# LeCAR-Lab/dial-mpc

Measured on NVIDIA H100. Metric: sample-steps/s (Nsample*Hsample/wall-s) per MPC reverse_once, Go2, higher is better.
Workload: dtype f32

## Files before the change

__graft_entry__.py:

```python
from __future__ import annotations

import os
import subprocess
import sys

ROOT = os.path.dirname(os.path.abspath(__file__))
CSRC = os.path.join(ROOT, "dial_mpc_b200", "csrc")
LIB = os.path.join(CSRC, "libdial_b200.so")
NVCC_FLAGS = ["-gencode", "arch=compute_90a,code=sm_90a", "-lineinfo", "-O3", "-std=c++17",
              "-use_fast_math", "-Xcompiler", "-fPIC"]
LINK_FLAGS = ["-gencode", "arch=compute_90a,code=sm_90a", "-shared", "-Xcompiler", "-fPIC", "-cudart", "static"]
VARIANTS = (1, 2, 3, 4, 0)
OBJDIR = os.path.join(CSRC, "build")


def _digest(srcs, extra=""):
    import hashlib
    h = hashlib.sha256()
    for s in srcs:
        h.update(open(s, "rb").read())
    h.update((" ".join(NVCC_FLAGS + LINK_FLAGS) + extra).encode())
    return h.hexdigest()


def _stale(target, digest):
    side = target + ".sha256"
    if not (os.path.exists(target) and os.path.exists(side)):
        return True
    return open(side).read().strip() != digest


def _stamp(target, digest):
    with open(target + ".sha256", "w") as f:
        f.write(digest)


def build_library(force: bool = False, extra=(), lib: str = LIB, objdir: str = OBJDIR) -> None:
    extra = list(extra)
    tag = " " + " ".join(extra)
    hdrs = [os.path.join(CSRC, f) for f in ("dial_device.cuh", "dial_host.h")] + [os.path.join(ROOT, "include", "dial_b200.h")]
    var_src = os.path.join(CSRC, "dial_rollout_variant.cu")
    abi_src = os.path.join(CSRC, "dial_kernels.cu")
    lib_digest = _digest(hdrs + [var_src, abi_src], tag)
    if not (force or _stale(lib, lib_digest)):
        return
    nvcc = os.environ.get("NVCC", "/usr/local/cuda/bin/nvcc")
    os.makedirs(objdir, exist_ok=True)
    jobs = []
    for v in VARIANTS:
        obj = os.path.join(objdir, f"rollout_v{v}.o")
        jobs.append((obj, _digest(hdrs + [var_src], f" variant={v}" + tag),
                     [nvcc] + NVCC_FLAGS + extra + [f"-DDIAL_VARIANT={v}", "-c", "-o", obj, var_src]))
    obj = os.path.join(objdir, "dial_kernels.o")
    jobs.append((obj, _digest(hdrs + [abi_src], tag), [nvcc] + NVCC_FLAGS + extra + ["-c", "-o", obj, abi_src]))
    running = [(o, d, subprocess.Popen(cmd)) for o, d, cmd in jobs if force or _stale(o, d)]
    for o, d, p in running:
        if p.wait() != 0:
            for _, _, q in running:
                q.wait()
            raise RuntimeError(f"nvcc failed for {o}")
        _stamp(o, d)
    subprocess.check_call([nvcc] + LINK_FLAGS + ["-o", lib] + [o for o, _, _ in jobs])
    _stamp(lib, lib_digest)


def build(force: bool = False) -> None:
    build_library(force)
    if ROOT not in sys.path:
        sys.path.insert(0, ROOT)
    import dial_mpc_b200
    from dial_mpc_b200 import _capi
    _capi.lib()
    ex = os.path.join(ROOT, "dial_mpc_b200", "examples", "custom_env")
    if ex not in sys.path:
        sys.path.insert(0, ex)
    import quadpod_env
    _ = quadpod_env.QuadpodEnv(quadpod_env.QuadpodEnvConfig()).library_path
    import pincher_env
    _ = pincher_env.PincherEnv(pincher_env.PincherEnvConfig()).library_path
    for mod in ("tests.emul.emul", "oracle.build_oracle"):
        path = os.path.join(ROOT, *mod.split(".")) + ".py"
        if os.path.exists(path):
            subprocess.check_call([sys.executable, "-c", f"import {mod} as m; m.build()"], cwd=ROOT)


def smoke() -> None:
    if ROOT not in sys.path:
        sys.path.insert(0, ROOT)
    import numpy as np
    import torch
    build()
    import dial_mpc_b200.envs as E
    from dial_mpc_b200 import random as drandom
    from dial_mpc_b200.core.dial_config import DialConfig
    from dial_mpc_b200.core.dial_core import MBDPI
    from oracle.envs_oracle import make_env
    from oracle.planner_oracle import PlannerOracle
    torch.cuda.set_device(0)
    cfg = DialConfig(env_name="unitree_go2_walk", Nsample=64, Hsample=8, Hnode=4, temp_sample=0.05)
    env = E.get_environment(cfg.env_name, config=E.UnitreeGo2EnvConfig(default_vx=0.8, ramp_up_time=1.0))
    mb = MBDPI(cfg, env)
    state = env.reset(drandom.PRNGKey(0))
    rng = np.random.default_rng(0)
    eps = rng.standard_normal((cfg.Nsample, cfg.Hnode + 1, mb.nu)).astype(np.float32)
    Y0 = torch.zeros(cfg.Hnode + 1, mb.nu, device=mb.device)
    _, Ybar, info = mb.reverse_once(state, drandom.PRNGKey(1), Y0, mb.sigma_control, eps=eps)
    torch.cuda.synchronize()
    o = make_env(cfg.env_name, dict(default_vx=0.8, ramp_up_time=1.0))
    po = PlannerOracle(o, cfg.Nsample, cfg.Hsample, cfg.Hnode, cfg.temp_sample, cfg.horizon_diffuse_factor,
                       cfg.traj_diffuse_factor)
    Yo, io = po.reverse_once(o.reset(), eps.astype(np.float64), np.zeros((cfg.Hnode + 1, mb.nu)), po.sigma_control)
    rews = info["rews"].cpu().numpy()
    err_r = np.abs(rews - io["rews"]).max()
    err_y = np.abs(Ybar.cpu().numpy() - Yo).max()
    print(f"smoke: max|rews - oracle| = {err_r:.3e}, max|Ybar - oracle| = {err_y:.3e}, launches = {mb.plan.launches}")
    assert np.isfinite(rews).all()
    assert err_r < 2e-3 and err_y < 5e-3, "CUDA reverse_once disagrees with the oracle"


if __name__ == "__main__":
    build()
    if len(sys.argv) > 1 and sys.argv[1] == "smoke":
        smoke()
```

dial_mpc_b200/_capi.py:

```python

from __future__ import annotations

import ctypes as C
import os
import re
from typing import Dict, Optional

import numpy as np

_HERE = os.path.dirname(os.path.abspath(__file__))
_ROOT = os.path.dirname(_HERE)
HEADER = os.path.join(_ROOT, "include", "dial_b200.h")
LIB_PATH = os.path.join(_HERE, "csrc", "libdial_b200.so")

_CT = {"int32_t": C.c_int32, "uint32_t": C.c_uint32, "float": C.c_float, "int64_t": C.c_int64}


def _parse_header(path: str):
    text = open(path).read()
    text = re.sub(r"/\*.*?\*/", "", text, flags=re.S)
    text = re.sub(r"//[^\n]*", "", text)
    defines: Dict[str, int] = {}
    for mm in re.finditer(r"#define\s+(\w+)\s+(\d+)\s*$", text, flags=re.M):
        defines[mm.group(1)] = int(mm.group(2))
# ... 105 lines not shown

def _set(field, value):
    arr = np.ctypeslib.as_array(field)
    value = np.asarray(value)
    if value.size == 0:
        return
    sl = tuple(slice(0, s) for s in value.shape)
    if any(s > d for s, d in zip(value.shape, arr.shape)):
        raise ValueError(f"value of shape {value.shape} exceeds capacity {arr.shape}")
    arr[sl] = value


def fill_model_desc(cm) -> dial_model_desc:
    d = dial_model_desc()
    for k in ("nq", "nv", "nu", "nbody", "njnt", "ngeom", "nsite", "npair", "ncon",
              "iterations", "ls_iterations", "cone"):
        setattr(d, k, int(getattr(cm, k)))
    d.eulerdamp = int(bool(cm.eulerdamp))
    for k in ("timestep", "tolerance", "ls_tolerance", "impratio", "meaninertia"):
        setattr(d, k, float(getattr(cm, k)))
    _set(d.gravity, cm.gravity)
    A = cm.arrays
    for k in ("body_parentid", "body_rootid", "body_depth", "body_jntadr", "body_dofadr", "body_dofnum",
              "body_pos", "body_quat", "body_ipos", "body_iquat", "body_mass", "body_inertia",
              "jnt_type", "jnt_qposadr", "jnt_dofadr", "jnt_limited", "jnt_pos", "jnt_axis", "jnt_range",
              "jnt_margin", "jnt_solref", "jnt_solimp",
              "dof_bodyid", "dof_jntid", "dof_parentid", "dof_armature", "dof_damping", "dof_invweight0",
              "qpos0", "geom_type", "geom_bodyid", "geom_pos", "geom_quat", "geom_size",
              "pair_kind", "pair_geom1", "pair_geom2", "pair_ncon", "pair_condim", "pair_friction", "pair_margin",
              "pair_gap", "pair_solref", "pair_solimp", "site_bodyid", "site_pos",
              "actuator_dofadr", "actuator_qposadr", "actuator_ctrllimited", "actuator_forcelimited",
              "actuator_gear", "actuator_gain", "actuator_bias", "actuator_ctrlrange", "actuator_forcerange"):
        _set(getattr(d, k), A[k])
    _set(d.body_invweight0, A["body_invweight0"][:, 0])
    _set(d.body_invweight0_rot, A["body_invweight0"][:, 1])
    return d


def _bind(path: str) -> C.CDLL:
    if not os.path.exists(path):
        raise RuntimeError(
            f"{path} is missing: build it with `python -c 'import __graft_entry__ as g; g.build()'`."
            " There is no CPU fallback for the DIAL-MPC sampling core.")
    lib = C.CDLL(path)
    lib.dial_abi_version.restype = C.c_int
    lib.dial_last_error.restype = C.c_char_p
    lib.dial_sizeof.restype = C.c_size_t
    lib.dial_sizeof.argtypes = [C.c_int]
    lib.dial_plan_create.restype = C.c_void_p
    lib.dial_plan_create.argtypes = [C.POINTER(dial_model_desc), C.POINTER(dial_plan_desc)]
    lib.dial_plan_destroy.argtypes = [C.c_void_p]
    lib.dial_plan_destroy.restype = None
    P, I, V = C.c_void_p, C.c_int, C.c_void_p
    lib.dial_rollout.argtypes = [V, C.POINTER(dial_state), P, I, I, P, P, P, P, V]
    lib.dial_env_step.argtypes = [V, C.POINTER(dial_state), P, P, P, P, P, P, V]
    lib.dial_env_step_kin.argtypes = [V, C.POINTER(dial_state), P, P, P, P, P, P, P, V]
    lib.dial_plan_set_command.argtypes = [V, C.c_int, C.POINTER(C.c_float), C.POINTER(C.c_float), V]
    F = C.POINTER(C.c_float)
    lib.dial_plan_set_stages.argtypes = [V, C.c_int, F, F, F, F, V]
    lib.dial_pipeline_init.argtypes = [V, P, P, P, P, V]
    U2 = C.POINTER(C.c_uint32)
    lib.dial_reverse_rollout.argtypes = [V, C.POINTER(dial_state), P, U2, P, P, P, V]
    lib.dial_reverse_update.argtypes = [V, P, U2, P, P, P, P, P, V]
    lib.dial_reverse_update_x.argtypes = [V, P, U2, P, P, P, P, P, P, V]
    lib.dial_reverse_update_fused.argtypes = [V, P, P, P, P, P, P, V]
    lib.dial_reverse_trajbar.argtypes = [V, P, I, P, P, P, V]
    lib.dial_exchange_create.argtypes = [V, I, I, P]
    lib.dial_exchange_connect.argtypes = [V, P]
    lib.dial_exchange_status.argtypes = [V, U2]
    lib.dial_reverse_trajectories.argtypes = [V, P, P, P, V]
    lib.dial_key_split.argtypes = [U2, U2, U2]
    lib.dial_key_split.restype = None
    lib.dial_fp32_peak.argtypes = [I, C.POINTER(C.c_float)]
    lib.dial_fp32_peak.restype = C.c_int
    lib.dial_launch_count.argtypes = [V]
    lib.dial_launch_count.restype = C.c_int64
    lib.dial_rollout_wpc.argtypes = [V, I]
    lib.dial_rollout_wpc.restype = C.c_int
    lib.dial_debug_counters.argtypes = [V, C.POINTER(C.c_float)]
    lib.dial_debug_counters.restype = C.c_int
    lib.dial_solver_variant.argtypes = [C.POINTER(dial_model_desc)]
    lib.dial_solver_variant.restype = C.c_int
    lib.dial_custom_reward_id.restype = C.c_char_p
    lib.dial_mpc_bind.argtypes = [V, C.POINTER(dial_mpc_buffers), P]
    lib.dial_mpc_bind.restype = C.c_int
    lib.dial_mpc_step.argtypes = [V, I, I, V]
    lib.dial_mpc_step.restype = C.c_int
    lib.dial_plan_get_task.argtypes = [V, C.POINTER(dial_task)]
    lib.dial_plan_get_task.restype = C.c_int
    for fn in ("dial_rollout", "dial_env_step", "dial_env_step_kin", "dial_plan_set_command", "dial_plan_set_stages", "dial_pipeline_init", "dial_reverse_rollout",
               "dial_reverse_update", "dial_reverse_update_x", "dial_reverse_update_fused", "dial_reverse_trajbar",
               "dial_reverse_trajectories", "dial_exchange_create", "dial_exchange_connect", "dial_exchange_status"):
        getattr(lib, fn).restype = C.c_int
    if lib.dial_abi_version() != DEFINES["DIAL_ABI_VERSION"]:
        raise RuntimeError(f"{os.path.basename(path)} ABI version does not match include/dial_b200.h")
    for i, t in enumerate((dial_model_desc, dial_plan_desc, dial_state, dial_mpc_buffers, dial_task)):
        if lib.dial_sizeof(i) != C.sizeof(t):
            raise RuntimeError(f"struct layout mismatch for {t.__name__}: C {lib.dial_sizeof(i)} vs ctypes {C.sizeof(t)}")
    return lib


_LIBS: Dict[str, C.CDLL] = {}


def lib(path: Optional[str] = None) -> C.CDLL:
    path = os.path.abspath(path or os.environ.get("DIAL_B200_LIB") or LIB_PATH)
    if path not in _LIBS:
        _LIBS[path] = _bind(path)
    return _LIBS[path]


def check(rc: int) -> None:
    if rc != 0:
        raise RuntimeError(f"dial_b200: {lib().dial_last_error().decode()} (rc={rc})")


EXPORTS = ["dial_abi_version", "dial_last_error", "dial_sizeof", "dial_plan_create", "dial_plan_destroy", "dial_rollout",
           "dial_env_step", "dial_env_step_kin", "dial_plan_set_command", "dial_plan_set_stages", "dial_pipeline_init", "dial_reverse_rollout", "dial_reverse_update", "dial_reverse_update_x",
           "dial_reverse_update_fused", "dial_exchange_create", "dial_exchange_connect", "dial_exchange_status",
           "dial_reverse_trajbar", "dial_reverse_trajectories", "dial_key_split", "dial_fp32_peak", "dial_launch_count", "dial_rollout_wpc", "dial_debug_counters",
           "dial_solver_variant", "dial_custom_reward_id", "dial_mpc_bind", "dial_mpc_step", "dial_plan_get_task"]
```

dial_mpc_b200/csrc/dial_device.cuh:

```cuda
#pragma once

#include <stdint.h>
#include <math.h>
#include "../../include/dial_b200.h"

#ifdef DIAL_HOST_EMUL
#include "warp_emul.h"
#define DEV inline
#define HD inline
#else
#define HD __host__ __device__ __forceinline__
#define DEV __device__ __forceinline__
DEV void syncwarp() { __syncwarp(); }
DEV float shfl(float v, int src) { return __shfl_sync(0xffffffffu, v, src); }
DEV float shfl_xor(float v, int m) { return __shfl_xor_sync(0xffffffffu, v, m); }
DEV int shfl_i(int v, int src) { return __shfl_sync(0xffffffffu, v, src); }
DEV void cta_sync() { __syncthreads(); }
DEV bool cta_sync_or(bool p) { return __syncthreads_or(p) != 0; }
DEV void fast_sincos(float x, float& s, float& c) { __sincosf(x, &s, &c); }
DEV float fast_cos(float x) { return __cosf(x); }
#endif

#if defined(DIAL_HOST_EMUL) && defined(DIAL_EMUL_TRACE)
extern "C" void emul_trace(int kind, int val);
// ... 30 lines not shown
  int32_t con_row0[DIAL_MAXC], con_dim[DIAL_MAXC], nrow_c;
  int32_t jd_stride;
  int8_t con_colidx[DIAL_MAXC][DIAL_MAXV];
  int32_t con_lastdof[DIAL_MAXC];
  int32_t dof_nchain[DIAL_MAXV], dof_ndesc[DIAL_MAXV], nlimited;
  int32_t chain_tab[DIAL_MAXV][DIAL_MAXCHAIN];
  int32_t star_nroot, star_nchain, star_maxlen;
  int32_t star_root[8], star_len[4], star_leaf[4], star_att[4];
  int32_t nedge;
  int32_t s_on, s_nrp, s_cs, s_rs, s_npos;
  int32_t s_pos[DIAL_MAXV];
  int32_t s_chain[DIAL_MAXV];
  int32_t s_depth[DIAL_MAXV];
  int32_t s_top[4];
  int32_t s_con_chain[DIAL_MAXC];
  int32_t o_Ms, o_Hs, o_Js, o_xs;
  int32_t sb_on, sb_nroot, sb_root[4], sb_top[4], sb_len[4], sb_att[4];
  int32_t o_xpos, o_xquat, o_xmat, o_xipos, o_cinert, o_cdof, o_cdofdot, o_cvel, o_cacc,
      o_cfrc, o_Mb, o_L, o_J, o_qpos, o_qvel, o_warm, o_ctrl, o_vec, o_frow, o_cpos,
      o_cframe, o_cdist, o_rcom, o_xch, o_crb, o_cfs, o_Md, o_Ld, o_Jd, o_Gd, o_frow2, o_cact, o_hcs, warp_floats;
  int32_t pad_[1];
};

struct alignas(16) DevPlan {
  dial_plan_desc c;
  int32_t pad_[3];
};

#define DIAL_TASK_AT(f) (offsetof(dial_plan_desc, f) - offsetof(dial_plan_desc, vel_cmd) == offsetof(dial_task, f))
static_assert(DIAL_TASK_AT(vel_cmd) && DIAL_TASK_AT(ang_cmd) && DIAL_TASK_AT(pos_tar) && DIAL_TASK_AT(gait_duty) &&
              DIAL_TASK_AT(gait_cadence) && DIAL_TASK_AT(gait_amplitude) && DIAL_TASK_AT(gait_phase) &&
              DIAL_TASK_AT(cmd_step) && DIAL_TASK_AT(cmd_vel) && DIAL_TASK_AT(cmd_ang) && DIAL_TASK_AT(n_stage) &&
              DIAL_TASK_AT(jump_dt) && DIAL_TASK_AT(pose_seq) && DIAL_TASK_AT(yaw_seq) &&
              DIAL_TASK_AT(contact_targets) && DIAL_TASK_AT(contact_radius) && DIAL_TASK_AT(n_user) &&
              DIAL_TASK_AT(user) &&
              offsetof(dial_plan_desc, user) + sizeof(float) * DIAL_MAXUSER - offsetof(dial_plan_desc, vel_cmd) == sizeof(dial_task),
              "dial_plan_desc's task block must have the layout of dial_task");
#undef DIAL_TASK_AT

HD const dial_task& plan_task(const dial_plan_desc& c) { return *reinterpret_cast<const dial_task*>(c.vel_cmd); }

struct RolloutArgs {
  int32_t nrows;
  int32_t H;
  int32_t mode;
  int32_t lockstep;
  int32_t sync_every;
  int32_t step0, stage0;
  int32_t rows_per_inst;
  int32_t us_row;
  int32_t task_rows;
  const dial_task* tasks;
  const float* qpos0;
  const float* qvel0;
  const float* warm0;
  const float* us;
  const float* eps;
  const float* Ybar;
  const float* noise;
  uint32_t key0, key1;
  float* rewss;
  float* rews;
  float* q;
  float* qd;
  float* xpos;
  float* qpos_out;
  float* qvel_out;
  float* warm_out;
  float* ctrl_out;
  float* kin_out;
  const int32_t* counters_in;
  int32_t* counters_out;
  const uint32_t* key_dev;
  const uint32_t* rng_dev;
  unsigned int* row_counter;
  float* dbg;
  int32_t xch_world, xch_rank;
  float* xch_mbox[DIAL_MAXRANK];
  uint32_t* xch_flags[DIAL_MAXRANK];
  const uint32_t* xch_seq;
  unsigned int* xch_done;
};

struct V3 { float x, y, z; };
struct Q4 { float w, x, y, z; };

DEV V3 v3(float x, float y, float z) { V3 r; r.x = x; r.y = y; r.z = z; return r; }
DEV V3 ld3(const float* p) { return v3(p[0], p[1], p[2]); }
DEV void st3(float* p, V3 a) { p[0] = a.x; p[1] = a.y; p[2] = a.z; }
DEV V3 operator+(V3 a, V3 b) { return v3(a.x + b.x, a.y + b.y, a.z + b.z); }
DEV V3 operator-(V3 a, V3 b) { return v3(a.x - b.x, a.y - b.y, a.z - b.z); }
DEV V3 operator*(V3 a, float s) { return v3(a.x * s, a.y * s, a.z * s); }
DEV float dot(V3 a, V3 b) { return a.x * b.x + a.y * b.y + a.z * b.z; }
DEV V3 cross(V3 a, V3 b) { return v3(a.y * b.z - a.z * b.y, a.z * b.x - a.x * b.z, a.x * b.y - a.y * b.x); }
DEV Q4 ldq(const float* p) { Q4 q; q.w = p[0]; q.x = p[1]; q.y = p[2]; q.z = p[3]; return q; }
DEV void stq(float* p, Q4 q) { p[0] = q.w; p[1] = q.x; p[2] = q.y; p[3] = q.z; }
DEV Q4 qmul(Q4 a, Q4 b) {
  Q4 r;
  r.w = a.w * b.w - a.x * b.x - a.y * b.y - a.z * b.z;
  r.x = a.w * b.x + a.x * b.w + a.y * b.z - a.z * b.y;
  r.y = a.w * b.y - a.x * b.z + a.y * b.w + a.z * b.x;
  r.z = a.w * b.z + a.x * b.y - a.y * b.x + a.z * b.w;
  return r;
}
DEV V3 qrot(Q4 q, V3 v) {
  V3 u = v3(q.x, q.y, q.z);
  float s = q.w;
  V3 r = u * (2.f * dot(u, v)) + v * (s * s - dot(u, u));
  return r + cross(u, v) * (2.f * s);
}
DEV Q4 qnormalize(Q4 q) {
  float n = sqrtf(q.w * q.w + q.x * q.x + q.y * q.y + q.z * q.z);
  float inv = 1.f / (n + 1e-6f * (n == 0.f ? 1.f : 0.f));
  Q4 r; r.w = q.w * inv; r.x = q.x * inv; r.y = q.y * inv; r.z = q.z * inv; return r;
}
DEV void qmat(Q4 q, float* m) {
  float w = q.w, x = q.x, y = q.y, z = q.z;
  m[0] = w * w + x * x - y * y - z * z; m[1] = 2.f * (x * y - w * z); m[2] = 2.f * (x * z + w * y);
  m[3] = 2.f * (x * y + w * z); m[4] = w * w - x * x + y * y - z * z; m[5] = 2.f * (y * z - w * x);
  m[6] = 2.f * (x * z - w * y); m[7] = 2.f * (y * z + w * x); m[8] = w * w - x * x - y * y + z * z;
}
DEV Q4 axisangle(V3 axis, float angle) {
  float s, c;
  fast_sincos(0.5f * angle, s, c);
  Q4 q; q.w = c; q.x = axis.x * s; q.y = axis.y * s; q.z = axis.z * s; return q;
}

struct F4 { float x, y, z, w; };
DEV F4 ld4(const float* p) {
#ifdef DIAL_HOST_EMUL
  F4 r; r.x = p[0]; r.y = p[1]; r.z = p[2]; r.w = p[3]; return r;
#else
  const float4 v = *reinterpret_cast<const float4*>(p);
  F4 r; r.x = v.x; r.y = v.y; r.z = v.z; r.w = v.w; return r;
#endif
}
DEV void st4(float* p, float a, float b, float c, float d) {
#ifdef DIAL_HOST_EMUL
  p[0] = a; p[1] = b; p[2] = c; p[3] = d;
#else
  *reinterpret_cast<float4*>(p) = make_float4(a, b, c, d);
#endif
}
DEV void ld2(const float* p, float& a, float& b) {
#ifdef DIAL_HOST_EMUL
  a = p[0]; b = p[1];
#else
  const float2 v = *reinterpret_cast<const float2*>(p);
  a = v.x; b = v.y;
#endif
}
DEV void st2(float* p, float a, float b) {
#ifdef DIAL_HOST_EMUL
  p[0] = a; p[1] = b;
#else
  *reinterpret_cast<float2*>(p) = make_float2(a, b);
#endif
}
#define CDS 8
#define CIS 12
DEV void ld6(const float* p, float* o) {
  F4 a = ld4(p);
  o[0] = a.x; o[1] = a.y; o[2] = a.z; o[3] = a.w;
  ld2(p + 4, o[4], o[5]);
}
DEV void st6(float* p, const float* v) {
// ... 433 lines not shown
  float l_sign, l_D, l_aref, l_Jaref;
  float e_D, e_aref, e_Jaref;
  float gauss, cost, prev_cost, gradnorm2;
  float qfc;
};

DEV void update_constraint(WarpCtx& w, Solver& S) {
  float fl = (S.l_Jaref < 0.f) ? -S.l_D * S.l_Jaref : 0.f;
  float fe = (S.e_Jaref < 0.f) ? -S.e_D * S.e_Jaref : 0.f;
  float qfc = mul_JT(w, fe) + S.l_sign * fl;
  S.grad = S.Ma - S.qfs - qfc;
  float g = (S.Ma - S.qfs) * (S.qacc - S.qas);
  float c = ((S.l_Jaref < 0.f) ? S.l_D * S.l_Jaref * S.l_Jaref : 0.f)
          + ((S.e_Jaref < 0.f) ? S.e_D * S.e_Jaref * S.e_Jaref : 0.f);
  float g2 = S.grad * S.grad;
  warp_sum3(g, c, g2);
  S.gauss = 0.5f * g;
  S.prev_cost = S.cost;
  S.cost = 0.5f * c + S.gauss;
  S.gradnorm2 = g2;
}

template <int MCU>
DEV void build_H(WarpCtx& w, const Solver& S, const float* Mrow, float* R) {
  const DevModel& M = *w.M;
  const int lane = w.lane;
  const float* Jc = SM(J);
  float* frow = SM(frow);
  syncwarp();
  frow[lane] = (S.e_Jaref < 0.f) ? S.e_D : 0.f;
  syncwarp();
#pragma unroll
  for (int c = 0; c < MCU; ++c) R[c] = Mrow[c];
  if (w.nch > 0) {
    R[0] += (S.l_Jaref < 0.f) ? S.l_D : 0.f;
    for (int c_ = 0; c_ < M.m.ncon; ++c_) {
      const int kc = M.con_lastdof[c_];
      if ((M.dof_ancmask[kc] >> lane) & 1u) {
        const int off = M.dof_nchain[kc] - w.nch;
        for (int e = 4 * c_; e < 4 * c_ + 4; ++e) {
          const float de = frow[e];
          if (de != 0.f) {
            const float* Je = Jc + e * MC + off;
            const float a = de * Je[0];
#pragma unroll
            for (int c = 0; c < MCU; ++c)
              if (c < w.nch) R[c] += a * Je[c];
          }
        }
      }
    }
  }
}


template <int NL, int NR>
struct StarDims {
  static constexpr int NRP = (NR + 3) & ~3, CS = (NL + 3) & ~3, RS = NRP + CS;
};

template <int N>
DEV void ldv(const float* p, float* out) {
  F4 a = ld4(p);
  out[0] = a.x; if (N > 1) out[1] = a.y; if (N > 2) out[2] = a.z; if (N > 3) out[3] = a.w;
  if (N > 4) {
    F4 b = ld4(p + 4);
    out[4] = b.x; if (N > 5) out[5] = b.y; if (N > 6) out[6] = b.z; if (N > 7) out[7] = b.w;
  }
}
template <int NL, int NR>
DEV void star_store_row(float* p, const float* Rr, const float* Rc) {
  using SD = StarDims<NL, NR>;
  float t[SD::RS];
#pragma unroll
  for (int i = 0; i < SD::RS; ++i) t[i] = 0.f;
#pragma unroll
  for (int a = 0; a < NR; ++a) t[a] = Rr[a];
#pragma unroll
  for (int q = 0; q < NL; ++q) t[SD::NRP + q] = Rc[q];
#pragma unroll
  for (int i = 0; i < SD::RS; i += 4) st4(p + i, t[i], t[i + 1], t[i + 2], t[i + 3]);
}

template <int NL, int NR, bool WITH_M, bool WITH_J>
DEV void star_mul_MJ(WarpCtx& w, const float* Mr, const float* Mc, float x, float& Mx, float& Jx) {
  using SD = StarDims<NL, NR>;
  const DevModel& M = *w.M;
  float* xs = SM(xs);
  const float* Ms = SM(Ms);
  syncwarp();
  if (w.s_chain >= -1) xs[w.s_pos] = x;
  syncwarp();
  float xr[SD::NRP], xc[SD::CS];
  ldv<NR>(xs, xr);
  ldv<NL>(xs + w.s_cb, xc);
  float y = 0.f;
  if (WITH_M) {
  float y0 = 0.f, y1 = 0.f, y2 = 0.f, y3 = 0.f;
#pragma unroll
  for (int a = 0; a < NR; ++a) { if (a & 1) y1 += Mr[a] * xr[a]; else y0 += Mr[a] * xr[a]; }
  if (w.s_chain >= 0) {
#pragma unroll
    for (int q = 0; q < NL; ++q) { if (q & 1) y3 += Mc[q] * xc[q]; else y2 += Mc[q] * xc[q]; }
  } else if (w.s_chain == -1) {
    const float* col = Ms + SD::NRP * SD::RS + w.s_col;
    const int nslot = M.star_nchain * SD::CS;
    for (int s0 = 0; s0 < nslot; s0 += 4) {
      F4 xv = ld4(xs + SD::NRP + s0);
      y0 += col[(s0 + 0) * SD::RS] * xv.x; y1 += col[(s0 + 1) * SD::RS] * xv.y;
      y2 += col[(s0 + 2) * SD::RS] * xv.z; y3 += col[(s0 + 3) * SD::RS] * xv.w;
    }
  }
  y = (y0 + y1) + (y2 + y3);
  }
  Mx = y;
  if (WITH_J) {
    float j = 0.f;
    if (w.lane < M.nedge) {
      const float* row = SM(Js) + w.lane * SD::RS;
      float jr[SD::NRP], jc[SD::CS], xe[SD::CS];
      ldv<NR>(row, jr);
      ldv<NL>(row + SD::NRP, jc);
      ldv<NL>(xs + w.e_cb, xe);
      float j0 = 0.f, j1 = 0.f, j2 = 0.f;
#pragma unroll
      for (int a = 0; a < NR; ++a) { if (a & 1) j1 += jr[a] * xr[a]; else j0 += jr[a] * xr[a]; }
#pragma unroll
      for (int q = 0; q < NL; ++q) j2 += jc[q] * xe[q];
      j = (j0 + j1) + j2;
    }
    Jx = j;
  }
}

template <int NL, int NR>
DEV float star_mul_JT(WarpCtx& w, float f) {
  using SD = StarDims<NL, NR>;
  const DevModel& M = *w.M;
  const float* Js = SM(Js);
  float* frow = SM(frow);
  syncwarp();
  frow[w.lane] = f;
  syncwarp();
  float y0 = 0.f, y1 = 0.f, y2 = 0.f, y3 = 0.f;
  const float* col = Js + w.s_col;
  for (int c = 0; c < M.m.ncon; ++c) {
    const F4 fv = ld4(frow + 4 * c);
    if ((w.s_conmask >> c) & 1u) {
      const float* jc = col + 4 * c * SD::RS;
      y0 += jc[0] * fv.x; y1 += jc[SD::RS] * fv.y; y2 += jc[2 * SD::RS] * fv.z; y3 += jc[3 * SD::RS] * fv.w;
    }
  }
  return (y0 + y1) + (y2 + y3);
}

template <int NL, int NR>
DEV void star_build_H(WarpCtx& w, const Solver& S, const float* Mr, const float* Mc, float* Rr, float* Rc) {
  using SD = StarDims<NL, NR>;
  const DevModel& M = *w.M;
  const float* Js = SM(Js);
  float* frow = SM(frow);
  syncwarp();
  frow[w.lane] = (S.e_Jaref < 0.f) ? S.e_D : 0.f;
  syncwarp();
#pragma unroll
  for (int a = 0; a < NR; ++a) Rr[a] = Mr[a];
#pragma unroll
  for (int q = 0; q < NL; ++q) Rc[q] = Mc[q];
  const float ld = (S.l_Jaref < 0.f) ? S.l_D : 0.f;
  if (w.s_chain >= 0) {
#pragma unroll
    for (int q = 0; q < NL; ++q) Rc[q] += (q == w.s_depth) ? ld : 0.f;
  } else if (w.s_chain == -1) {
#pragma unroll
    for (int a = 0; a < NR; ++a) Rr[a] += (a == w.s_depth) ? ld : 0.f;
  }
  for (int e = 0; e < M.nedge; ++e) {
    const float de = frow[e];
    if (de == 0.f) continue;
    const float* row = Js + e * SD::RS;
    const float je = ((w.s_conmask >> (e >> 2)) & 1u) ? row[w.s_col] : 0.f;
    const float al = de * je;
    float jr[SD::NRP], jc[SD::CS];
    ldv<NR>(row, jr);
    ldv<NL>(row + SD::NRP, jc);
#pragma unroll
    for (int a = 0; a < NR; ++a) Rr[a] += al * jr[a];
#pragma unroll
    for (int q = 0; q < NL; ++q) Rc[q] += al * jc[q];
  }
}

template <int NL, int NR>
DEV float star_solve2(WarpCtx& w, const float* Rr, const float* Rc, float g) {
  using SD = StarDims<NL, NR>;
  static_assert(NR + 1 <= 8, "root block + rhs must fit the 8 lanes of a group");
  const DevModel& M = *w.M;
  const int lane = w.lane;
  float* Hs = SM(Hs);
  float* xs = SM(xs);
  syncwarp();
  if (w.s_chain >= -1) {
    star_store_row<NL, NR>(Hs + w.s_pos * SD::RS, Rr, Rc);
    xs[w.s_pos] = g;
  }
  syncwarp();
  const int grp = lane >> 3, j = lane & 7, gbase = lane & ~7;
  const bool ischain = grp < M.star_nchain;
  const int len = ischain ? M.star_len[grp] : 0;
  const int cb = SD::NRP + grp * SD::CS;
  float A[NL][NL], wv[NL];
#pragma unroll
  for (int p = 0; p < NL; ++p) {
    const bool on = p < len;
    const float* row = Hs + (cb + p) * SD::RS;
    float rc[SD::CS];
    ldv<NL>(row + SD::NRP, rc);
#pragma unroll
    for (int p2 = p; p2 < NL; ++p2) A[p][p2] = (on && p2 < len) ? rc[p2] : (p2 == p ? 1.f : 0.f);
    float cv = 0.f;
    if (on && j < NR) cv = row[j];
    if (on && j == NR) cv = xs[cb + p];
    wv[p] = cv;
  }
  float rinv[NL];
#pragma unroll
  for (int p = 0; p < NL; ++p) {
    float d = A[p][p];
#pragma unroll
    for (int k = 0; k < p; ++k) d -= A[k][p] * A[k][p];
    const float inv = rsqrtf(fmaxf(d, DIAL_MINVAL));
    rinv[p] = inv;
#pragma unroll
    for (int p2 = p + 1; p2 < NL; ++p2) {
      float v = A[p][p2];
#pragma unroll
      for (int k = 0; k < p; ++k) v -= A[k][p] * A[k][p2];
      A[p][p2] = v * inv;
    }
    float v = wv[p];
#pragma unroll
    for (int k = 0; k < p; ++k) v -= A[k][p] * wv[k];
    wv[p] = v * inv;
  }
  float t[NR + 1];
#pragma unroll
  for (int j2 = 0; j2 <= NR; ++j2) {
    float acc = 0.f;
#pragma unroll
    for (int p = 0; p < NL; ++p) acc += wv[p] * shfl(wv[p], gbase + j2);
    t[j2] = acc;
  }
#pragma unroll
  for (int j2 = 0; j2 <= NR; ++j2) {
    t[j2] += shfl_xor(t[j2], 8);
    t[j2] += shfl_xor(t[j2], 16);
  }
  float srow[NR], rhs = 0.f;
  {
    const int jj = j < NR ? j : 0;
    float br[SD::NRP];
    ldv<NR>(Hs + jj * SD::RS, br);
#pragma unroll
    for (int a2 = 0; a2 < NR; ++a2) srow[a2] = br[a2] - t[a2];
    rhs = xs[jj] - t[NR];
  }
  float S_[NR][NR], xB[NR];
#pragma unroll
  for (int a = 0; a < NR; ++a) {
#pragma unroll
    for (int a2 = a; a2 < NR; ++a2) S_[a][a2] = shfl(srow[a2], gbase + a);
    xB[a] = shfl(rhs, gbase + a);
  }
  float sinv[NR];
#pragma unroll
  for (int a = 0; a < NR; ++a) {
    float d = S_[a][a];
#pragma unroll
    for (int k = 0; k < a; ++k) d -= S_[k][a] * S_[k][a];
    const float inv = rsqrtf(fmaxf(d, DIAL_MINVAL));
    sinv[a] = inv;
#pragma unroll
    for (int a2 = a + 1; a2 < NR; ++a2) {
      float v = S_[a][a2];
#pragma unroll
      for (int k = 0; k < a; ++k) v -= S_[k][a] * S_[k][a2];
      S_[a][a2] = v * inv;
    }
    float v = xB[a];
#pragma unroll
    for (int k = 0; k < a; ++k) v -= S_[k][a] * xB[k];
    xB[a] = v * inv;
  }
#pragma unroll
  for (int a = NR - 1; a >= 0; --a) {
    float v = xB[a];
#pragma unroll
    for (int a2 = a + 1; a2 < NR; ++a2) v -= S_[a][a2] * xB[a2];
    xB[a] = v * sinv[a];
  }
  float xb_j = 0.f;
#pragma unroll
  for (int a = 0; a < NR; ++a) xb_j = (j == a) ? xB[a] : xb_j;
  float xl[NL];
#pragma unroll
  for (int p = 0; p < NL; ++p) {
    float v = (j < NR) ? wv[p] * xb_j : 0.f;
    v += shfl_xor(v, 1); v += shfl_xor(v, 2); v += shfl_xor(v, 4);
    xl[p] = shfl(wv[p], gbase + NR) - v;
  }
#pragma unroll
  for (int p = NL - 1; p >= 0; --p) {
    float v = xl[p];
#pragma unroll
    for (int p2 = p + 1; p2 < NL; ++p2) v -= A[p][p2] * xl[p2];
    xl[p] = v * rinv[p];
  }
  syncwarp();
  if (j == 0 && ischain) {
#pragma unroll
    for (int p = 0; p < NL; ++p)
      if (p < len) xs[cb + p] = xl[p];
  }
  if (lane == 0) {
#pragma unroll
    for (int a = 0; a < NR; ++a) xs[a] = xB[a];
  }
  syncwarp();
  return w.s_chain >= -1 ? xs[w.s_pos] : 0.f;
}

template <int NL, int NR>
DEV void star_update_constraint(WarpCtx& w, Solver& S) {
  float fl = (S.l_Jaref < 0.f) ? -S.l_D * S.l_Jaref : 0.f;
  float fe = (S.e_Jaref < 0.f) ? -S.e_D * S.e_Jaref : 0.f;
  float qfc = star_mul_JT<NL, NR>(w, fe) + S.l_sign * fl;
  S.grad = S.Ma - S.qfs - qfc;
  float g = (S.Ma - S.qfs) * (S.qacc - S.qas);
  float c = ((S.l_Jaref < 0.f) ? S.l_D * S.l_Jaref * S.l_Jaref : 0.f)
          + ((S.e_Jaref < 0.f) ? S.e_D * S.e_Jaref * S.e_Jaref : 0.f);
  float g2 = S.grad * S.grad;
  warp_sum3(g, c, g2);
  S.gauss = 0.5f * g;
  S.prev_cost = S.cost;
  S.cost = 0.5f * c + S.gauss;
  S.gradnorm2 = g2;
}

struct LSPoint { float alpha, cost, d0, d1; };

#ifdef DIAL_ROBUST_LS
#define DIAL_LS_SWAP_LO(lo, nx) (((lo).d0 < (nx).d0) && ((nx).d0 < 0.f))
#define DIAL_LS_SWAP_HI(hi, nx) (((hi).d0 > (nx).d0) && ((nx).d0 > 0.f))
#else
#define DIAL_LS_SWAP_LO(lo, nx) (((lo).d0 > 0.f) || ((lo).d0 < (nx).d0))
#define DIAL_LS_SWAP_HI(hi, nx) (((hi).d0 < 0.f) || ((hi).d0 > (nx).d0))
#endif

DEV void warp_allsum6(int lane, float* v) {
  const bool b16 = (lane & 16) != 0, b8 = (lane & 8) != 0;
  float u0 = b16 ? v[3] : v[0], u1 = b16 ? v[4] : v[1], u2 = b16 ? v[5] : v[2];
  const float s0 = b16 ? v[0] : v[3], s1 = b16 ? v[1] : v[4], s2 = b16 ? v[2] : v[5];
  u0 += shfl_xor(s0, 16); u1 += shfl_xor(s1, 16); u2 += shfl_xor(s2, 16);
  float t = b8 ? u1 : u0;
  const float st = b8 ? u0 : u1;
  t += shfl_xor(st, 8); u2 += shfl_xor(u2, 8);
  t += shfl_xor(t, 4); u2 += shfl_xor(u2, 4);
  t += shfl_xor(t, 2); u2 += shfl_xor(u2, 2);
  t += shfl_xor(t, 1); u2 += shfl_xor(u2, 1);
  v[0] = shfl(t, 0); v[1] = shfl(t, 8); v[3] = shfl(t, 16); v[4] = shfl(t, 24);
  v[2] = shfl(u2, 0); v[5] = shfl(u2, 16);
}

struct LSRow { float lq0, lq1, lq2, eq0, eq1, eq2; };

template <int NA, bool COST>
DEV void ls_points(int lane, const Solver& S, const LSRow& K, float l_jv, float e_jv, const float* qg, const float* al, LSPoint* out) {
  float s[3 * NA];
#pragma unroll
  for (int i = 0; i < 3 * NA; ++i) s[i] = 0.f;
#pragma unroll
  for (int i = 0; i < NA; ++i) {
    if (S.l_Jaref + al[i] * l_jv < 0.f) { if (COST) s[3 * i] += K.lq0; s[3 * i + 1] += K.lq1; s[3 * i + 2] += K.lq2; }
    if (S.e_Jaref + al[i] * e_jv < 0.f) { if (COST) s[3 * i] += K.eq0; s[3 * i + 1] += K.eq1; s[3 * i + 2] += K.eq2; }
  }
  if constexpr ((NA == 3 && !COST) || (NA == 2 && COST)) {
    float v[6];
    if constexpr (NA == 3) { v[0] = s[1]; v[1] = s[2]; v[2] = s[4]; v[3] = s[5]; v[4] = s[7]; v[5] = s[8]; }
    else { v[0] = s[0]; v[1] = s[1]; v[2] = s[2]; v[3] = s[3]; v[4] = s[4]; v[5] = s[5]; }
    warp_allsum6(lane, v);
    if constexpr (NA == 3) { s[1] = v[0]; s[2] = v[1]; s[4] = v[2]; s[5] = v[3]; s[7] = v[4]; s[8] = v[5]; }
    else { s[0] = v[0]; s[1] = v[1]; s[2] = v[2]; s[3] = v[3]; s[4] = v[4]; s[5] = v[5]; }
  } else {
#pragma unroll
    for (int o = 16; o > 0; o >>= 1) {
#pragma unroll
      for (int i = 0; i < 3 * NA; ++i)
        if (COST || (i % 3) != 0) s[i] += shfl_xor(s[i], o);
    }
  }
#pragma unroll
  for (int i = 0; i < NA; ++i) {
    float t0 = qg[0] + s[3 * i], t1 = qg[1] + s[3 * i + 1], t2 = qg[2] + s[3 * i + 2];
    float a = al[i];
    out[i].alpha = a;
    out[i].cost = COST ? a * a * t2 + a * t1 + t0 : 0.f;
    out[i].d0 = 2.f * a * t2 + t1;
    out[i].d1 = 2.f * t2 + (t2 == 0.f ? DIAL_MINVAL : 0.f);
  }
}

DEV void linesearch_core(WarpCtx& w, Solver& S, float mv, float e_jv) {
  const DevModel& M = *w.M;
  const int nv = M.m.nv;
  const float scale = M.m.meaninertia * (float)(nv > 1 ? nv : 1);
  float l_jv = S.l_sign * S.search;
  float ss = S.search * S.search, sMa = S.search * (S.Ma - S.qfs), sMv = S.search * mv;
  warp_sum3(ss, sMa, sMv);
  float gtol = M.m.tolerance * M.m.ls_tolerance * sqrtf(ss) * scale;
  float qg[3] = {S.gauss, sMa, 0.5f * sMv};
  LSRow K;
  K.lq0 = 0.5f * S.l_Jaref * S.l_Jaref * S.l_D; K.lq1 = l_jv * S.l_Jaref * S.l_D; K.lq2 = 0.5f * l_jv * l_jv * S.l_D;
  K.eq0 = 0.5f * S.e_Jaref * S.e_Jaref * S.e_D; K.eq1 = e_jv * S.e_Jaref * S.e_D; K.eq2 = 0.5f * e_jv * e_jv * S.e_D;
  LSPoint p0, lo, hi;
  float a1[1] = {0.f};
  ls_points<1, true>(w.lane, S, K, l_jv, e_jv, qg, a1, &p0);
  a1[0] = p0.alpha - p0.d0 / p0.d1;
  ls_points<1, false>(w.lane, S, K, l_jv, e_jv, qg, a1, &lo);
  if (lo.d0 < p0.d0) { hi = p0; } else { hi = lo; lo = p0; }
  bool swap = true;
  for (int it = 0; it < M.m.ls_iterations; ++it) {
    bool done = !swap;
    done |= (lo.d0 < 0.f) && (lo.d0 > -gtol);
    done |= (hi.d0 > 0.f) && (hi.d0 < gtol);
    if (done) break;
    LSPoint pt[3];
    float a3[3] = {lo.alpha - lo.d0 / lo.d1, hi.alpha - hi.d0 / hi.d1, 0.5f * (lo.alpha + hi.alpha)};
    ls_points<3, false>(w.lane, S, K, l_jv, e_jv, qg, a3, pt);
    const LSPoint lo_next = pt[0], hi_next = pt[1], mid = pt[2];
    bool swap_lo_next = DIAL_LS_SWAP_LO(lo, lo_next);
    if (swap_lo_next) lo = lo_next;
    bool swap_lo_mid = (mid.d0 < 0.f) && (lo.d0 < mid.d0);
    if (swap_lo_mid) lo = mid;
    bool swap_hi_next = DIAL_LS_SWAP_HI(hi, hi_next);
    if (swap_hi_next) hi = hi_next;
    bool swap_hi_mid = (mid.d0 > 0.f) && (hi.d0 > mid.d0);
    if (swap_hi_mid) hi = mid;
    swap = swap_lo_next || swap_lo_mid || swap_hi_next || swap_hi_mid;
  }
  {
    LSPoint fin[2];
    float a2[2] = {lo.alpha, hi.alpha};
    ls_points<2, true>(w.lane, S, K, l_jv, e_jv, qg, a2, fin);
    lo.cost = fin[0].cost; hi.cost = fin[1].cost;
  }
  bool improved = (lo.cost < p0.cost) || (hi.cost < p0.cost);
  float alpha = (lo.cost < hi.cost) ? lo.alpha : hi.alpha;
  if (!improved) alpha = 0.f;
  S.qacc += alpha * S.search;
  S.Ma += alpha * mv;
  S.l_Jaref += alpha * l_jv;
  S.e_Jaref += alpha * e_jv;
}

template <int MCU>
DEV void linesearch(WarpCtx& w, Solver& S, const float* Mrow) {
  float mv = mul_M<MCU>(w, Mrow, S.search);
  float e_jv = mul_J(w, S.search);
  linesearch_core(w, S, mv, e_jv);
}

struct ConeLane {
  float x[6], D[6], aref[6], fri[5];
  float mu, Dm;
  int dim, r0;
  bool inst;
};

DEV void dense_mul_J(WarpCtx& w, const ConeLane& C, float xd, float* out) {
  const DevModel& M = *w.M;
  const int nv = M.m.nv, lane = w.lane;
  const float* Jd = SM(Jd);
  const int* cact = reinterpret_cast<const int*>(SM(cact));
#pragma unroll
  for (int i = 0; i < 6; ++i) out[i] = 0.f;
  const float xv = lane < nv ? xd : 0.f;
  const int col = lane < nv ? lane : 0, js = M.jd_stride;
  for (int c = 0; c < M.m.ncon; ++c) {
    if (!cact[c]) continue;
    const int r0 = M.con_row0[c], dim = M.con_dim[c];
    const int idx = M.con_colidx[c][col];
    float p[6];
#pragma unroll
    for (int i = 0; i < 6; ++i) p[i] = (i < dim && idx >= 0) ? Jd[(r0 + i) * js + idx] * xv : 0.f;
#pragma unroll
    for (int o = 16; o > 0; o >>= 1) {
#pragma unroll
      for (int i = 0; i < 6; ++i)
        if (i < dim) p[i] += shfl_xor(p[i], o);
    }
    if (lane == c) {
#pragma unroll
      for (int i = 0; i < 6; ++i) out[i] = p[i];
    }
  }
  (void)C;
}

DEV float dense_mul_JT(WarpCtx& w, const ConeLane& C, const float* f) {
  const DevModel& M = *w.M;
  const int nv = M.m.nv, lane = w.lane;
  const float* Jd = SM(Jd);
  float* fr = SM(frow2);
  const int* cact = reinterpret_cast<const int*>(SM(cact));
// ... 509 lines not shown
      S.cost = INFINITY;
      S.prev_cost = 0.f;
      mode = 1;
    } else if (!done) {
      S.search = -x;
      dense_linesearch(w, S, C);
      ++it;
    }
    if (!done) {
      dense_update_constraint(w, S, C);
      done = it >= m.iterations;
      if (m.iterations != 1 || it > 0) {
        float improvement = (S.prev_cost - S.cost) / scale;
        float gradient = sqrtf(S.gradnorm2) / scale;
        if (m.iterations != 1) done = done || (improvement < m.tolerance) || (gradient < m.tolerance);
      }
      if (!(fabsf(S.cost) <= 3.0e38f)) done = true;
    }
    const bool any = w.itersync ? cta_sync_or(!done) : !done;
    if (!any) {
      if (!m.eulerdamp) { qacc_int = S.qacc; break; }
      mode = 2;
#pragma unroll
      for (int j = 0; j < NVD; ++j) Hrow[j] = (isdof && j <= d) ? Md[d * nv + j] : 0.f;
#pragma unroll
      for (int j = 0; j < NVD; ++j)
        if (j == d) Hrow[j] += isdof ? m.timestep * m.dof_damping[d] : 1.f;
      g = S.qfs + S.qfc;
      continue;
    }
    if (done) continue;
    dense_build_H<NVD>(w, S, C, Hrow);
    g = S.grad;
  }
#ifndef DIAL_HOST_EMUL
  if (w.dbg && lane == 0) { atomicAdd(w.dbg, 1.f); atomicAdd(w.dbg + 1, (float)it); }
#endif
  DIAL_TRACE(lane, 0, it);
  return S.qacc;
}

DEV V3 mat_z(const float* X, const float* q) {
  float Rg[9];
  qmat(ldq(q), Rg);
  return v3(X[0] * Rg[2] + X[1] * Rg[5] + X[2] * Rg[8], X[3] * Rg[2] + X[4] * Rg[5] + X[5] * Rg[8],
            X[6] * Rg[2] + X[7] * Rg[5] + X[8] * Rg[8]);
}
DEV V3 mat_apply(const float* X, const float* p) {
  return v3(X[0] * p[0] + X[1] * p[1] + X[2] * p[2], X[3] * p[0] + X[4] * p[1] + X[5] * p[2],
            X[6] * p[0] + X[7] * p[1] + X[8] * p[2]);
}
DEV V3 vnormalize(V3 a, float& n) {
  n = sqrtf(dot(a, a));
  return a * (1.f / (n + 1e-6f * (n == 0.f ? 1.f : 0.f)));
}
DEV V3 closest_segment_point(V3 a, V3 b, V3 pt) {
  V3 ab = b - a;
  float t = dot(pt - a, ab) / (dot(ab, ab) + 1e-6f);
  return a + ab * fminf(fmaxf(t, 0.f), 1.f);
}
DEV void closest_segment_to_segment(V3 a0, V3 a1, V3 b0, V3 b1, V3& pa, V3& pb) {
  float len_a, len_b;
  V3 dir_a = vnormalize(a1 - a0, len_a), dir_b = vnormalize(b1 - b0, len_b);
  float ha = 0.5f * len_a, hb = 0.5f * len_b;
  V3 a_mid = a0 + dir_a * ha, b_mid = b0 + dir_b * hb;
  V3 trans = a_mid - b_mid;
  float dd = dot(dir_a, dir_b), dat = dot(dir_a, trans), dbt = dot(dir_b, trans);
  float denom = 1.f - dd * dd;
  float ta = (-dat + dd * dbt) / (denom + 1e-6f);
  float tb = dbt + ta * dd;
  ta = fminf(fmaxf(ta, -ha), ha);
  tb = fminf(fmaxf(tb, -hb), hb);
  V3 best_a = a_mid + dir_a * ta, best_b = b_mid + dir_b * tb;
  V3 new_a = closest_segment_point(a0, a1, best_b), new_b = closest_segment_point(b0, b1, best_a);
  V3 e1 = new_a - best_b, e2 = new_b - best_a;
  if (dot(e1, e1) < dot(e2, e2)) { pa = new_a; pb = best_b; } else { pa = best_a; pb = new_b; }
}
DEV V3 frame_tangent(V3 n) {
  V3 alt = (n.y > -0.5f && n.y < 0.5f) ? v3(0, 1, 0) : v3(0, 0, 1);
  float bn;
  return vnormalize(alt - n * dot(n, alt), bn);
}

DEV void collide(WarpCtx& w) {
  const DevModel& M = *w.M;
  const dial_model_desc& m = M.m;
  const int lane = w.lane;
  if (lane >= m.ncon) return;
  const float* xpos = SM(xpos);
  const float* xmat = SM(xmat);
  const int k = M.con_pair[lane];
  const int g1 = m.pair_geom1[k], g2 = m.pair_geom2[k];
  const int b1 = m.geom_bodyid[g1], b2 = m.geom_bodyid[g2];
  const float* X1 = xmat + 9 * b1;
  const float* X2 = xmat + 9 * b2;
  const V3 gp1 = mat_apply(X1, m.geom_pos[g1]) + ld3(xpos + 3 * b1);
  const V3 gp2 = mat_apply(X2, m.geom_pos[g2]) + ld3(xpos + 3 * b2);
  const int kind = m.pair_kind[k];
  V3 n, t1, p;
  float dist;
  if (kind == PAIR_PLANE_SPHERE || kind == PAIR_PLANE_CAPSULE) {
    n = mat_z(X1, m.geom_quat[g1]);
    const float radius = m.geom_size[g2][0];
    V3 center = gp2;
    if (kind == PAIR_PLANE_CAPSULE) {
      V3 ax = mat_z(X2, m.geom_quat[g2]);
      float bn;
      V3 bd = vnormalize(ax - n * dot(n, ax), bn);
      V3 alt = (n.y > -0.5f && n.y < 0.5f) ? v3(0, 1, 0) : v3(0, 0, 1);
      t1 = bn < 0.5f ? alt : bd;
      center = gp2 + ax * ((M.con_sub[lane] == 0 ? 1.f : -1.f) * m.geom_size[g2][1]);
    } else {
      t1 = frame_tangent(n);
    }
    dist = dot(center - gp1, n) - radius;
    p = center - n * (radius + 0.5f * dist);
  } else {
    V3 q1 = gp1, q2 = gp2;
    if (kind == PAIR_SPHERE_CAPSULE) {
      V3 seg = mat_z(X2, m.geom_quat[g2]) * m.geom_size[g2][1];
      q2 = closest_segment_point(gp2 - seg, gp2 + seg, gp1);
    } else if (kind == PAIR_CAPSULE_CAPSULE) {
      V3 s1 = mat_z(X1, m.geom_quat[g1]) * m.geom_size[g1][1];
      V3 s2 = mat_z(X2, m.geom_quat[g2]) * m.geom_size[g2][1];
      closest_segment_to_segment(gp1 - s1, gp1 + s1, gp2 - s2, gp2 + s2, q1, q2);
    }
    float dn;
    n = vnormalize(q2 - q1, dn);
    if (dn == 0.f) n = v3(1, 0, 0);
    const float r1 = m.geom_size[g1][0], r2 = m.geom_size[g2][0];
    dist = dn - (r1 + r2);
    p = q1 + n * (r1 + 0.5f * dist);
    float nn;
    n = vnormalize(n, nn);
    t1 = frame_tangent(n);
  }
  SM(cdist)[lane] = dist;
  st3(SM(cpos) + 3 * lane, p);
  st3(SM(cframe) + 9 * lane, n);
  st3(SM(cframe) + 9 * lane + 3, t1);
  st3(SM(cframe) + 9 * lane + 6, cross(n, t1));
}

template <int NL, int NR>
DEV void physics_step(WarpCtx& w, bool integrate) {
  constexpr int MCU = (NL == 3 && NR == 6) ? 9 : DIAL_MAXCHAIN;
  const DevModel& M = *w.M;
  const dial_model_desc& m = M.m;
  const int lane = w.lane, nb = m.nbody, nv = m.nv;
  float* xpos = SM(xpos); float* xquat = SM(xquat); float* xmat = SM(xmat); float* xipos = SM(xipos);
  float* cinert = SM(cinert); float* cdof = SM(cdof); float* cdofdot = SM(cdofdot);
  float* cvel = SM(cvel); float* cacc = SM(cacc); float* cfrc = SM(cfrc);
  float* J = SM(J);
  float* qpos = SM(qpos); float* qvel = SM(qvel); float* warm = SM(warm); float* ctrl = SM(ctrl);
  float* cpos = SM(cpos); float* cframe = SM(cframe); float* cdist = SM(cdist); float* rcom = SM(rcom);

  const int b = lane;
  const bool isbody = b > 0 && b < nb;
  const int depth = isbody ? m.body_depth[b] : -1;
  const int jid = isbody ? m.body_jntadr[b] : -1;
  const int jtype = jid >= 0 ? m.jnt_type[jid] : -1;
  V3 anchor = v3(0, 0, 0), axis = v3(0, 0, 1), xip = v3(0, 0, 0);
  float ximat[9];
#pragma unroll
  for (int i = 0; i < 9; ++i) ximat[i] = 0.f;
  Q4 qL; qL.w = 1.f; qL.x = qL.y = qL.z = 0.f;
  V3 pL = v3(0, 0, 0), aL = v3(0, 0, 0), axL = v3(0, 0, 1);
  if (isbody) {
    const Q4 bq = ldq(m.body_quat[b]);
    const V3 bp = ld3(m.body_pos[b]);
    qL = bq; pL = bp;
    if (jtype == JNT_HINGE || jtype == JNT_SLIDE) {
      const int qa = m.jnt_qposadr[jid];
      const V3 jp = ld3(m.jnt_pos[jid]), ja = ld3(m.jnt_axis[jid]);
      aL = bp + qrot(bq, jp);
      axL = qrot(bq, ja);
      const float dq = qpos[qa] - m.qpos0[qa];
      if (jtype == JNT_HINGE) {
        qL = qmul(bq, axisangle(ja, dq));
        pL = aL - qrot(qL, jp);
      } else {
        pL = bp + axL * dq;
      }
    }
  }
  V3 pos = v3(0, 0, 0);
  Q4 quat; quat.w = 1.f; quat.x = quat.y = quat.z = 0.f;
  for (int lv = 1; lv <= M.maxdepth; ++lv) {
    if (depth == lv) {
      if (jtype == JNT_FREE) {
        const int qa = m.jnt_qposadr[jid];
        pos = ld3(qpos + qa);
        quat = qnormalize(ldq(qpos + qa + 3));
        stq(qpos + qa + 3, quat);
        anchor = pos;
        axis = v3(0, 0, 1);
      } else {
        const int p = m.body_parentid[b];
        const Q4 pq = ldq(xquat + 4 * p);
        const V3 pp = ld3(xpos + 3 * p);
        quat = qmul(pq, qL);
        pos = pp + qrot(pq, pL);
        anchor = pp + qrot(pq, aL);
        axis = qrot(pq, axL);
      }
      quat = qnormalize(quat);
      st3(xpos + 3 * b, pos);
      stq(xquat + 4 * b, quat);
    }
    syncwarp();
  }
  if (isbody) {
    float R[9];
    qmat(quat, R);
#pragma unroll
    for (int i = 0; i < 9; ++i) xmat[9 * b + i] = R[i];
    xip = pos + qrot(quat, ld3(m.body_ipos[b]));
    st3(xipos + 3 * b, xip);
    qmat(qmul(quat, ldq(m.body_iquat[b])), ximat);
  }

  const int myroot = isbody ? M.body_rootidx[b] : -1;
  V3 com = v3(0, 0, 0);
  for (int r = 0; r < M.nroot; ++r) {
    float mass = (myroot == r) ? m.body_mass[b] : 0.f;
    float sx = mass * xip.x, sy = mass * xip.y, sz = mass * xip.z;
    warp_sum3(sx, sy, sz);
    V3 c = v3(sx, sy, sz) * M.root_invmass[r];
    if (lane == 0) st3(rcom + 3 * r, c);
    if (myroot == r) com = c;
  }

  if (isbody) {
    V3 off = xip - com;
    float mass = m.body_mass[b];
    const float* di = m.body_inertia[b];
    float I[6];
    I[0] = ximat[0] * ximat[0] * di[0] + ximat[1] * ximat[1] * di[1] + ximat[2] * ximat[2] * di[2];
    I[1] = ximat[3] * ximat[3] * di[0] + ximat[4] * ximat[4] * di[1] + ximat[5] * ximat[5] * di[2];
    I[2] = ximat[6] * ximat[6] * di[0] + ximat[7] * ximat[7] * di[1] + ximat[8] * ximat[8] * di[2];
    I[3] = ximat[0] * ximat[3] * di[0] + ximat[1] * ximat[4] * di[1] + ximat[2] * ximat[5] * di[2];
    I[4] = ximat[0] * ximat[6] * di[0] + ximat[1] * ximat[7] * di[1] + ximat[2] * ximat[8] * di[2];
    I[5] = ximat[3] * ximat[6] * di[0] + ximat[4] * ximat[7] * di[1] + ximat[5] * ximat[8] * di[2];
    float o2 = dot(off, off);
    float* ci = cinert + CIS * b;
    st4(ci, I[0] + mass * (o2 - off.x * off.x), I[1] + mass * (o2 - off.y * off.y), I[2] + mass * (o2 - off.z * off.z),
        I[3] - mass * off.x * off.y);
    st4(ci + 4, I[4] - mass * off.x * off.z, I[5] - mass * off.y * off.z, mass * off.x, mass * off.y);
    st2(ci + 8, mass * off.z, mass);
    if (jid >= 0) {
      int d = m.jnt_dofadr[jid];
      V3 offset = com - anchor;
      if (jtype == JNT_FREE) {
        for (int i = 0; i < 3; ++i) {
          float* c0 = cdof + CDS * (d + i);
          st4(c0, 0.f, 0.f, 0.f, i == 0 ? 1.f : 0.f);
          st2(c0 + 4, i == 1 ? 1.f : 0.f, i == 2 ? 1.f : 0.f);
          V3 ax = v3(xmat[9 * b + i], xmat[9 * b + 3 + i], xmat[9 * b + 6 + i]);
          V3 cx = cross(ax, offset);
          float* c1 = cdof + CDS * (d + 3 + i);
          st4(c1, ax.x, ax.y, ax.z, cx.x);
          st2(c1 + 4, cx.y, cx.z);
        }
      } else if (jtype == JNT_HINGE) {
        V3 cx = cross(axis, offset);
        st4(cdof + CDS * d, axis.x, axis.y, axis.z, cx.x);
        st2(cdof + CDS * d + 4, cx.y, cx.z);
      } else {
        st4(cdof + CDS * d, 0.f, 0.f, 0.f, axis.x);
        st2(cdof + CDS * d + 4, axis.y, axis.z);
      }
    }
  }
  syncwarp();

  float mycv[6] = {0.f, 0.f, 0.f, 0.f, 0.f, 0.f}, myca[6] = {0.f, 0.f, 0.f, 0.f, 0.f, 0.f};
  for (int lv = 1; lv <= M.maxdepth; ++lv) {
    if (depth == lv) {
      int p = m.body_parentid[b];
      float cv[6], ca[6];
#pragma unroll
      for (int i = 0; i < 6; ++i) { cv[i] = cvel[6 * p + i]; ca[i] = cacc[6 * p + i]; }
      if (jtype == JNT_FREE) {
        int d = m.jnt_dofadr[jid];
        for (int k = 0; k < 3; ++k) {
          float qd = qvel[d + k], cd[6];
          ld6(cdof + CDS * (d + k), cd);
#pragma unroll
          for (int i = 0; i < 6; ++i) cv[i] += cd[i] * qd;
          st4(cdofdot + CDS * (d + k), 0.f, 0.f, 0.f, 0.f);
          st2(cdofdot + CDS * (d + k) + 4, 0.f, 0.f);
        }
        float cvt[6];
#pragma unroll
        for (int i = 0; i < 6; ++i) cvt[i] = cv[i];
        for (int k = 3; k < 6; ++k) {
          float dd[6], cd[6];
          ld6(cdof + CDS * (d + k), cd);
          mcross(cvt, cd, dd);
          float qd = qvel[d + k];
          st6(cdofdot + CDS * (d + k), dd);
#pragma unroll
          for (int i = 0; i < 6; ++i) {
            cv[i] += cd[i] * qd;
            ca[i] += dd[i] * qd;
          }
        }
      } else if (jid >= 0) {
        int d = m.jnt_dofadr[jid];
        float dd[6], cd[6];
        ld6(cdof + CDS * d, cd);
        mcross(cv, cd, dd);
        float qd = qvel[d];
        st6(cdofdot + CDS * d, dd);
#pragma unroll
        for (int i = 0; i < 6; ++i) {
          cv[i] += cd[i] * qd;
          ca[i] += dd[i] * qd;
        }
      }
#pragma unroll
      for (int i = 0; i < 6; ++i) {
        cvel[6 * b + i] = cv[i];
        cacc[6 * b + i] = ca[i];
        mycv[i] = cv[i]; myca[i] = ca[i];
      }
    }
    syncwarp();
  }
  if (isbody) {
    float f1[6], f2[6], f3[6], cib[10];
    ld10(cinert + CIS * b, cib);
    inert_mul(cib, myca, f1);
    inert_mul(cib, mycv, f2);
    mcross_force(mycv, f2, f3);
#pragma unroll
    for (int i = 0; i < 6; ++i) cfrc[6 * b + i] = f1[i] + f3[i];
  }
  syncwarp();

  {
    float* crb = SM(crb);
    float* cfs = SM(cfs);
    const int comp = lane & 15, half = lane >> 4;
    const float* src = comp < 10 ? cinert + comp : cfrc + (comp - 10);
    const int stride = comp < 10 ? CIS : 6;
    float* dst = comp < 10 ? crb + comp : cfs + (comp - 10);
    if (NL > 0 && M.sb_on) {
      for (int l = half; l < M.star_nchain; l += 2) {
        const int top = M.sb_top[l];
        float acc = 0.f;
        for (int k = M.sb_len[l] - 1; k >= 0; --k) { acc += src[(top + k) * stride]; dst[(top + k) * stride] = acc; }
      }
      syncwarp();
      if (half == 0) {
        float below = 0.f;
        for (int r = 0; r < M.sb_nroot; ++r) {
          float acc = src[M.sb_root[r] * stride] + below;
          for (int l = 0; l < M.star_nchain; ++l)
            if (M.sb_att[l] == r) acc += dst[M.sb_top[l] * stride];
          dst[M.sb_root[r] * stride] = acc;
          below = acc;
        }
      }
    } else {
      for (int b0 = 1; b0 < nb; b0 += 2) {
        const int bb = b0 + half;
        if (bb < nb) {
          float acc = 0.f;
          const int last = bb + M.body_ndesc[bb];
          for (int jb = bb; jb <= last; ++jb) acc += src[jb * stride];
          dst[bb * stride] = acc;
        }
      }
    }
  }
  syncwarp();

  collide(w);
  syncwarp();

  Solver S;
  S.qfs = 0.f; S.qas = 0.f;
  S.l_sign = 0.f; S.l_D = 0.f; S.l_aref = 0.f; S.l_Jaref = 0.f;
  S.e_D = 0.f; S.e_aref = 0.f; S.e_Jaref = 0.f;
  S.qacc = S.Ma = S.grad = S.search = 0.f;
  S.gauss = S.cost = S.prev_cost = S.gradnorm2 = 0.f;
  S.qfc = 0.f;
  const int d = lane;
  const bool isdof = d < nv;
  float myqvel = isdof ? qvel[d] : 0.f;
  float mycdof[6] = {0.f, 0.f, 0.f, 0.f, 0.f, 0.f};
  constexpr bool STAR = NL > 0;
  constexpr int SNR = STAR ? NR : 1, SNL = STAR ? NL : 1;
  float Mrow[STAR ? 1 : MC], R[STAR ? 1 : MC];
  float Mr[SNR], Mc[SNL], Rr[SNR], Rc[SNL];
#pragma unroll
  for (int a = 0; a < SNR; ++a) { Mr[a] = 0.f; Rr[a] = 0.f; }
#pragma unroll
  for (int q = 0; q < SNL; ++q) { Mc[q] = 0.f; Rc[q] = 0.f; }
  if constexpr (!STAR) {
#pragma unroll
    for (int c = 0; c < MCU; ++c) { Mrow[c] = 0.f; R[c] = 0.f; }
  }
  if (isdof) {
    int bi = m.dof_bodyid[d];
    float f[6];
    {
      float crbb[10];
      ld10(SM(crb) + CIS * bi, crbb);
      ld6(cdof + CDS * d, mycdof);
      inert_mul(crbb, mycdof, f);
    }
    if constexpr (STAR) {
      using SD = StarDims<NL, NR>;
      const float arm = m.dof_armature[d];
      if (w.s_chain >= 0) {
        const int att = M.star_att[w.s_chain];
#pragma unroll
        for (int q = 0; q < NL; ++q)
          if (q <= w.s_depth) { float cd[6]; ld6(cdof + CDS * (w.s_top + q), cd); Mc[q] = dot6(f, cd) + (q == w.s_depth ? arm : 0.f); }
#pragma unroll
        for (int a = 0; a < NR; ++a)
          if (a >= att) { float cd[6]; ld6(cdof + CDS * M.star_root[a], cd); Mr[a] = dot6(f, cd); }
      } else {
#pragma unroll
        for (int a = 0; a < NR; ++a)
          if (a >= w.s_depth) { float cd[6]; ld6(cdof + CDS * M.star_root[a], cd); Mr[a] = dot6(f, cd) + (a == w.s_depth ? arm : 0.f); }
      }
      star_store_row<NL, NR>(SM(Ms) + w.s_pos * SD::RS, Mr, Mc);
    } else {
#pragma unroll
      for (int c = 0; c < MCU; ++c)
        if (c < w.nch) { float cd[6]; ld6(cdof + CDS * w.chain[c], cd); Mrow[c] = dot6(f, cd); }
      Mrow[0] += m.dof_armature[d];
      if constexpr (NL >= 0) {
        float* Mb = SM(Mb);
#pragma unroll
        for (int c = 0; c < MCU; ++c)
          if (c < w.nch) Mb[d * MC + c] = Mrow[c];
      }
    }
    float bias = dot6(mycdof, SM(cfs) + 6 * bi);
    float act = 0.f;
    int a = M.dof_actuator[d];
    if (a >= 0) {
      float c = ctrl[a];
      if (m.actuator_ctrllimited[a]) c = fminf(fmaxf(c, m.actuator_ctrlrange[a][0]), m.actuator_ctrlrange[a][1]);
      float force = m.actuator_gain[a] * c + m.actuator_bias[a][0]
                  + m.actuator_bias[a][1] * qpos[m.actuator_qposadr[a]] + m.actuator_bias[a][2] * myqvel;
      if (m.actuator_forcelimited[a]) force = fminf(fmaxf(force, m.actuator_forcerange[a][0]), m.actuator_forcerange[a][1]);
      act = force * m.actuator_gear[a];
    }
    S.qfs = -m.dof_damping[d] * myqvel - bias + act;
  }
  if constexpr (NL >= 0) {
    if (M.s_on && M.o_crb == M.o_Hs) {
      syncwarp();
      float* z = SM(crb);
      for (int i = lane; i < (CIS + 6) * nb; i += 32) z[i] = 0.f;
      syncwarp();
    }
  }
  if constexpr (STAR) {
    using SD = StarDims<NL, NR>;
    float* Ms = SM(Ms);
    syncwarp();
    if (w.s_chain >= 0) {
#pragma unroll
      for (int q = 0; q < NL; ++q)
        if (q > w.s_depth) { Mc[q] = Ms[(w.s_cb + q) * SD::RS + SD::NRP + w.s_depth]; Ms[w.s_pos * SD::RS + SD::NRP + q] = Mc[q]; }
    } else if (w.s_chain == -1) {
#pragma unroll
      for (int a = 0; a < NR; ++a)
        if (a < w.s_depth) { Mr[a] = Ms[a * SD::RS + w.s_depth]; Ms[w.s_pos * SD::RS + a] = Mr[a]; }
    }
  }

  float qacc, qacc_int;
  if constexpr (NL < 0) {
    if (w.midsync) cta_sync();
    else syncwarp();
    qacc = dense_constraint_solve<NR>(w, S, Mrow, myqvel, qacc_int);
  } else if constexpr (STAR) {
  using SD = StarDims<NL, NR>;
  float* Js = SM(Js);
  if (isdof) {
    V3 ca_ = v3(mycdof[0], mycdof[1], mycdof[2]), cl_ = v3(mycdof[3], mycdof[4], mycdof[5]);
    V3 rc = ld3(rcom + 3 * M.body_rootidx[m.dof_bodyid[d]]);
    for (int c = 0; c < m.ncon; ++c) {
      if (!((w.s_conmask >> c) & 1u)) continue;
      const int k = M.con_pair[c];
      float e0 = 0.f, e1 = 0.f, e2 = 0.f, e3 = 0.f;
      const bool moves = (M.body_dofmask[m.geom_bodyid[m.pair_geom2[k]]] >> d) & 1u;
      if (moves && cdist[c] - (m.pair_margin[k] - m.pair_gap[k]) < 0.f) {
        V3 p = ld3(cpos + 3 * c);
        V3 jp = cl_ + cross(ca_, p - rc);
        float jn = dot(ld3(cframe + 9 * c), jp), j1 = dot(ld3(cframe + 9 * c + 3), jp), j2 = dot(ld3(cframe + 9 * c + 6), jp);
        float mu0 = m.pair_friction[k][0], mu1 = m.pair_friction[k][1];
        e0 = jn + mu0 * j1; e1 = jn - mu0 * j1; e2 = jn + mu1 * j2; e3 = jn - mu1 * j2;
      }
      float* col = Js + 4 * c * SD::RS + w.s_col;
      col[0] = e0; col[SD::RS] = e1; col[2 * SD::RS] = e2; col[3 * SD::RS] = e3;
    }
    int lj = M.dof_limited[d];
    if (lj >= 0) {
      float qv = qpos[m.jnt_qposadr[lj]];
      float dmin = qv - m.jnt_range[lj][0], dmax = m.jnt_range[lj][1] - qv;
      float pos = fminf(dmin, dmax) - m.jnt_margin[lj];
      if (pos < 0.f) {
        float sign = dmin < dmax ? 1.f : -1.f;
        float k_, b_, imp;
        kbi(m.timestep, m.jnt_solref[lj], m.jnt_solimp[lj], pos, k_, b_, imp);
        float Rr_ = fmaxf(m.dof_invweight0[d] * (1.f - imp) / imp, DIAL_MINVAL);
        S.l_sign = sign;
        S.l_D = 1.f / Rr_;
        S.l_aref = -b_ * (sign * myqvel) - k_ * imp * pos;
      }
    }
  }
  float ejv, dummy;
  star_mul_MJ<NL, NR, false, true>(w, Mr, Mc, myqvel, dummy, ejv);
  if (lane < M.nedge) {
    int c = lane >> 2;
    int k = M.con_pair[c];
    float pos = cdist[c] - (m.pair_margin[k] - m.pair_gap[k]);
    if (pos < 0.f) {
      int b1 = m.geom_bodyid[m.pair_geom1[k]], b2 = m.geom_bodyid[m.pair_geom2[k]];
      float mu = m.pair_friction[k][0];
      float t = m.body_invweight0[b1] + m.body_invweight0[b2];
      float iw = (t + mu * mu * t) * 2.f * mu * mu / m.impratio;
      float k_, b_, imp;
      kbi(m.timestep, m.pair_solref[k], m.pair_solimp[k], pos, k_, b_, imp);
      float Rr_ = fmaxf(iw * (1.f - imp) / imp, DIAL_MINVAL);
      S.e_D = 1.f / Rr_;
      S.e_aref = -b_ * ejv - k_ * imp * pos;
    }
  }
  if (w.midsync) cta_sync();
  const float scale = m.meaninertia * (float)(nv > 1 ? nv : 1);
  const float mywarm = isdof ? warm[d] : 0.f;
  float g = S.qfs;
#pragma unroll
  for (int a = 0; a < NR; ++a) Rr[a] = Mr[a];
#pragma unroll
  for (int q = 0; q < NL; ++q) Rc[q] = Mc[q];
  int it = 0;
  bool done;
  {
    float x = star_solve2<NL, NR>(w, Rr, Rc, g);
    S.qas = x;
    if (M.nedge == 0 && M.nlimited == 0) { S.qacc = x; done = true; }
    else {
      float Maw, eJw, eJs;
      star_mul_MJ<NL, NR, true, true>(w, Mr, Mc, mywarm, Maw, eJw);
      star_mul_MJ<NL, NR, false, true>(w, Mr, Mc, S.qas, dummy, eJs);
      eJw -= S.e_aref; eJs -= S.e_aref;
      float lJw = S.l_sign * mywarm - S.l_aref;
      float gw = (Maw - S.qfs) * (mywarm - S.qas);
      float cw = ((lJw < 0.f) ? S.l_D * lJw * lJw : 0.f) + ((eJw < 0.f) ? S.e_D * eJw * eJw : 0.f);
      float Mas = S.qfs;
      float lJs = S.l_sign * S.qas - S.l_aref;
      float cs = ((lJs < 0.f) ? S.l_D * lJs * lJs : 0.f) + ((eJs < 0.f) ? S.e_D * eJs * eJs : 0.f);
      warp_sum3(gw, cw, cs);
      const bool usewarm = (0.5f * cw + 0.5f * gw) < (0.5f * cs);
      S.qacc = usewarm ? mywarm : S.qas;
      S.Ma = usewarm ? Maw : Mas;
      S.e_Jaref = usewarm ? eJw : eJs;
      S.l_Jaref = usewarm ? lJw : lJs;
      S.cost = INFINITY;
      S.prev_cost = 0.f;
      star_update_constraint<NL, NR>(w, S);
      done = false;
      if (m.iterations != 1) {
        float improvement = (S.prev_cost - S.cost) / scale;
        float gradient = sqrtf(S.gradnorm2) / scale;
        done = (improvement < m.tolerance) || (gradient < m.tolerance);
      }
    }
  }
  while (!done) {
    star_build_H<NL, NR>(w, S, Mr, Mc, Rr, Rc);
    float x = star_solve2<NL, NR>(w, Rr, Rc, S.grad);
    S.search = -x;
    float mv, e_jv;
    star_mul_MJ<NL, NR, true, true>(w, Mr, Mc, S.search, mv, e_jv);
    linesearch_core(w, S, mv, e_jv);
    ++it;
    star_update_constraint<NL, NR>(w, S);
    done = it >= m.iterations;
    float improvement = (S.prev_cost - S.cost) / scale;
    float gradient = sqrtf(S.gradnorm2) / scale;
    if (m.iterations != 1) done = done || (improvement < m.tolerance) || (gradient < m.tolerance);
  }
  qacc = S.qacc;
  qacc_int = qacc;
  } else {
  if (isdof) {
    V3 ca_ = v3(mycdof[0], mycdof[1], mycdof[2]), cl_ = v3(mycdof[3], mycdof[4], mycdof[5]);
    int rootb = M.body_rootidx[m.dof_bodyid[d]];
    V3 rc = ld3(rcom + 3 * rootb);
    for (int c = 0; c < m.ncon; ++c) {
      const int kc = M.con_lastdof[c];
      if (!((M.dof_ancmask[kc] >> d) & 1u)) continue;
      const int k = M.con_pair[c];
      const int p_ = M.dof_nchain[kc] - w.nch;
      float e0 = 0.f, e1 = 0.f, e2 = 0.f, e3 = 0.f;
      if (cdist[c] - (m.pair_margin[k] - m.pair_gap[k]) < 0.f) {
        V3 p = ld3(cpos + 3 * c);
        V3 jp = cl_ + cross(ca_, p - rc);
        float jn = dot(ld3(cframe + 9 * c), jp), j1 = dot(ld3(cframe + 9 * c + 3), jp), j2 = dot(ld3(cframe + 9 * c + 6), jp);
        float mu0 = m.pair_friction[k][0], mu1 = m.pair_friction[k][1];
        e0 = jn + mu0 * j1; e1 = jn - mu0 * j1; e2 = jn + mu1 * j2; e3 = jn - mu1 * j2;
      }
      J[(4 * c + 0) * MC + p_] = e0; J[(4 * c + 1) * MC + p_] = e1;
      J[(4 * c + 2) * MC + p_] = e2; J[(4 * c + 3) * MC + p_] = e3;
    }
    int lj = M.dof_limited[d];
    if (lj >= 0) {
      float qv = qpos[m.jnt_qposadr[lj]];
      float dmin = qv - m.jnt_range[lj][0], dmax = m.jnt_range[lj][1] - qv;
      float pos = fminf(dmin, dmax) - m.jnt_margin[lj];
      if (pos < 0.f) {
        float sign = dmin < dmax ? 1.f : -1.f;
        float k_, b_, imp;
        kbi(m.timestep, m.jnt_solref[lj], m.jnt_solimp[lj], pos, k_, b_, imp);
        float Rr = fmaxf(m.dof_invweight0[d] * (1.f - imp) / imp, DIAL_MINVAL);
        S.l_sign = sign;
        S.l_D = 1.f / Rr;
        S.l_aref = -b_ * (sign * myqvel) - k_ * imp * pos;
      }
    }
  }
  float ejv = mul_J(w, myqvel);
  if (lane < M.nedge) {
    int c = lane >> 2;
    int k = M.con_pair[c];
    float pos = cdist[c] - (m.pair_margin[k] - m.pair_gap[k]);
    if (pos < 0.f) {
      int b1 = m.geom_bodyid[m.pair_geom1[k]], b2 = m.geom_bodyid[m.pair_geom2[k]];
      float mu = m.pair_friction[k][0];
      float t = m.body_invweight0[b1] + m.body_invweight0[b2];
      float iw = (t + mu * mu * t) * 2.f * mu * mu / m.impratio;
      float k_, b_, imp;
      kbi(m.timestep, m.pair_solref[k], m.pair_solimp[k], pos, k_, b_, imp);
      float Rr = fmaxf(iw * (1.f - imp) / imp, DIAL_MINVAL);
      S.e_D = 1.f / Rr;
      S.e_aref = -b_ * ejv - k_ * imp * pos;
    }
  }

  if (w.midsync) cta_sync();
  const float scale = m.meaninertia * (float)(nv > 1 ? nv : 1);
  const float mywarm = isdof ? warm[d] : 0.f;
  float g = S.qfs;
#pragma unroll
  for (int c = 0; c < MCU; ++c) R[c] = Mrow[c];
  int phase = 0, it = 0;
  while (true) {
    float x = tree_solve<NL, NR, MCU>(w, R, g);
    if (phase == 0) {
      S.qas = x;
      if (M.nedge == 0 && M.nlimited == 0) { S.qacc = x; break; }
      float Maw = mul_M<MCU>(w, Mrow, mywarm);
      float eJw = mul_J(w, mywarm) - S.e_aref;
      float lJw = S.l_sign * mywarm - S.l_aref;
      float gw = (Maw - S.qfs) * (mywarm - S.qas);
      float cw = ((lJw < 0.f) ? S.l_D * lJw * lJw : 0.f) + ((eJw < 0.f) ? S.e_D * eJw * eJw : 0.f);
      float Mas = S.qfs;
      float eJs = mul_J(w, S.qas) - S.e_aref;
      float lJs = S.l_sign * S.qas - S.l_aref;
      float cs = ((lJs < 0.f) ? S.l_D * lJs * lJs : 0.f) + ((eJs < 0.f) ? S.e_D * eJs * eJs : 0.f);
      warp_sum3(gw, cw, cs);
      const bool usewarm = (0.5f * cw + 0.5f * gw) < (0.5f * cs);
      S.qacc = usewarm ? mywarm : S.qas;
      S.Ma = usewarm ? Maw : Mas;
// ... 2 lines not shown
      S.cost = INFINITY;
      S.prev_cost = 0.f;
    } else {
      S.search = -x;
      linesearch<MCU>(w, S, Mrow);
      ++it;
    }
    update_constraint(w, S);
    bool done = (phase == 1) && (it >= m.iterations);
    if (m.iterations != 1 || phase == 1) {
      float improvement = (S.prev_cost - S.cost) / scale;
      float gradient = sqrtf(S.gradnorm2) / scale;
      if (m.iterations != 1) done = done || (improvement < m.tolerance) || (gradient < m.tolerance);
    }
    if (done) break;
    phase = 1;
    build_H<MCU>(w, S, Mrow, R);
    g = S.grad;
  }
  qacc = S.qacc;
  qacc_int = qacc;

  }

  syncwarp();
  if (isdof) {
    warm[d] = qacc;
    if (integrate) qvel[d] = myqvel + m.timestep * qacc_int;
  }
  syncwarp();
  if (integrate && isbody && jid >= 0) {
    int qa = m.jnt_qposadr[jid], dd = m.jnt_dofadr[jid];
    if (jtype == JNT_FREE) {
      for (int i = 0; i < 3; ++i) qpos[qa + i] += m.timestep * qvel[dd + i];
      V3 wv = ld3(qvel + dd + 3);
      float nrm = sqrtf(dot(wv, wv));
      V3 ax = wv * (1.f / (nrm + 1e-6f * (nrm == 0.f ? 1.f : 0.f)));
      Q4 qn = qnormalize(qmul(ldq(qpos + qa + 3), axisangle(ax, m.timestep * nrm)));
      stq(qpos + qa + 3, qn);
    } else {
      qpos[qa] += m.timestep * qvel[dd];
    }
  }
  syncwarp();
}

DEV float foot_step(float duty, float cadence, float amplitude, float phase, float time) {
  const float PI = 3.14159265358979f, TWO_PI = 6.28318530717959f;
  float t = time * TWO_PI * cadence + PI;
  float a = t + PI - TWO_PI * phase;
  float angle = a - floorf(a / TWO_PI) * TWO_PI - PI;
  if (duty < 1.f) angle *= 0.5f / (1.f - duty);
  float cl = fminf(fmaxf(angle, -0.5f * PI), 0.5f * PI);
  float value = duty < 1.f ? fast_cos(cl) : 0.f;
  float fin = fabsf(value) >= 1e-6f ? fabsf(value) : 0.f;
  return amplitude * fin;
}

DEV float quat_yaw(Q4 q) {
  return atan2f(-2.f * q.x * q.y + 2.f * q.w * q.z, q.x * q.x + q.w * q.w - q.z * q.z - q.y * q.y);
}

struct BaseKin { V3 pos, vb, ab; Q4 rot; };

DEV BaseKin base_kin(WarpCtx& w, int bid) {
  const DevModel& M = *w.M;
  BaseKin r;
  r.pos = ld3(SM(xpos) + 3 * bid);
  r.rot = ldq(SM(xquat) + 4 * bid);
  V3 ang = ld3(SM(cvel) + 6 * bid), lin = ld3(SM(cvel) + 6 * bid + 3);
  V3 off = r.pos - ld3(SM(rcom) + 3 * M.body_rootidx[bid]);
  V3 vel = lin - cross(off, ang);
  Q4 qc; qc.w = r.rot.w; qc.x = -r.rot.x; qc.y = -r.rot.y; qc.z = -r.rot.z;
  r.vb = qrot(qc, vel);
  r.ab = qrot(qc, ang * (3.14159265358979f / 180.f));
  return r;
}

#ifdef DIAL_CUSTOM_REWARD_FILE
#include "../../include/dial_custom_reward.h"
#include DIAL_CUSTOM_REWARD_FILE
#endif

DEV void reward_partials(WarpCtx& w, const dial_task& T, int step, int stage, float& p0, float& p1) {
  const DevModel& M = *w.M;
  const dial_plan_desc& c = w.P->c;
  const dial_model_desc& m = M.m;
  const float stepf = (float)step;
  const int f = w.lane;
  p0 = 0.f; p1 = 0.f;
  if (c.env_id == DIAL_ENV_GO2_WALK || c.env_id == DIAL_ENV_H1_WALK || c.env_id == DIAL_ENV_H1_LOCO) {
    if (f < c.nfeet) {
      float zt = foot_step(T.gait_duty, T.gait_cadence, T.gait_amplitude, T.gait_phase[f], stepf * c.dt);
      float z;
      if (c.env_id == DIAL_ENV_GO2_WALK) {
        int sid = c.feet_site[f], sb = m.site_bodyid[sid];
        const float* X = SM(xmat) + 9 * sb;
        z = SM(xpos)[3 * sb + 2] + X[6] * m.site_pos[sid][0] + X[7] * m.site_pos[sid][1] + X[8] * m.site_pos[sid][2];
        float e = (zt - z) / 0.05f;
        p0 = -e * e;
      } else if (c.env_id == DIAL_ENV_H1_WALK) {
        z = fminf(SM(cdist)[2 * f], SM(cdist)[2 * f + 1]);
        p0 = -(zt - z) * (zt - z);
      } else {
        z = fminf(fminf(SM(cdist)[4 * f], SM(cdist)[4 * f + 1]), fminf(SM(cdist)[4 * f + 2], SM(cdist)[4 * f + 3]));
        p0 = -(zt - z) * (zt - z);
      }
    }
  } else if (c.env_id == DIAL_ENV_GO2_SEQJUMP) {
    if (f < 4) {
      const int i = f;
      float dist = SM(cdist)[i];
      bool penal = dist <= 0.001f;
      float px = SM(cpos)[3 * i], py = SM(cpos)[3 * i + 1];
      for (int j = 0; j < T.n_stage; ++j) {
        float dx = px - T.contact_targets[j][i][0], dyy = py - T.contact_targets[j][i][1];
        bool cond = dx * dx + dyy * dyy <= T.contact_radius[j][i] * T.contact_radius[j][i];
        if (cond && j == stage) p0 += fminf(fmaxf(1.f - dist, 0.f), 1.f);
        penal = penal && !cond;
      }
      p1 = penal ? 1.f : 0.f;
    }
  } else {
    return;
  }
  p0 += shfl_xor(p0, 1); p1 += shfl_xor(p1, 1);
  p0 += shfl_xor(p0, 2); p1 += shfl_xor(p1, 2);
}

DEV float reward_lane0(WarpCtx& w, const dial_task& T, int step, int& stage, float part0, float part1) {
  const DevModel& M = *w.M;
  const dial_plan_desc& c = w.P->c;
  const dial_model_desc& m = M.m;
  const float stepf = (float)step;
  float rew = 0.f;
#ifdef DIAL_CUSTOM_REWARD_FILE
  if (c.env_id == DIAL_ENV_CUSTOM) {
    dial_reward_ctx x;
    x.step = step; x.dt = c.dt;
    x.nq = m.nq; x.nv = m.nv; x.nu = m.nu; x.nbody = m.nbody; x.ncon = m.ncon; x.nsite = m.nsite; x.n_user = T.n_user;
    x.qpos = SM(qpos); x.qvel = SM(qvel); x.ctrl = SM(ctrl);
    x.xpos = SM(xpos); x.xquat = SM(xquat); x.xmat = SM(xmat); x.cvel = SM(cvel);
    x.subtree_com = SM(rcom); x.body_rootidx = M.body_rootidx;
    x.contact_dist = SM(cdist); x.contact_pos = SM(cpos);
    x.site_bodyid = m.site_bodyid; x.site_pos = &m.site_pos[0][0];
    x.user = T.user;
    return dial_custom_reward(&x);
  }
#endif
  Q4 rot0 = ldq(SM(xquat) + 4);
  V3 up = qrot(rot0, v3(0, 0, 1));
  float r_upright = -(up.x * up.x + up.y * up.y + (up.z - 1.f) * (up.z - 1.f));
  BaseKin bk = base_kin(w, c.torso_body);
  if (c.env_id == DIAL_ENV_ALLEGRO) {
    const int ob = c.torso_body;
    V3 wv = ld3(SM(cvel) + 6 * ob) * (3.14159265358979f / 180.f);
    V3 dw = wv - ld3(T.ang_cmd);
    V3 dp = ld3(SM(xpos) + 3 * ob) - ld3(T.pos_tar);
    float rj = 0.f;
    for (int a = 0; a < m.nu; ++a) { float e = SM(qpos)[7 + a] - c.joint_offset[a]; rj -= e * e; }
    return -dot(dw, dw) - 5.f * dot(dp, dp) + 0.1f * rj;
  }
  if (c.env_id == DIAL_ENV_GO2_WALK || c.env_id == DIAL_ENV_H1_WALK || c.env_id == DIAL_ENV_H1_LOCO) {
    float ramp = stepf * c.dt / c.ramp_up_time;
    const float* vel_cmd = step == T.cmd_step ? T.cmd_vel : T.vel_cmd;
    const float* ang_cmd = step == T.cmd_step ? T.cmd_ang : T.ang_cmd;
    float vtx = fminf(vel_cmd[0] * ramp, vel_cmd[0]), vty = fminf(vel_cmd[1] * ramp, vel_cmd[1]);
    float atz = fminf(ang_cmd[2] * ramp, ang_cmd[2]);
    const float r_gaits = part0;
    float yaw_tar = 0.f + atz * c.dt * stepf;
    float dyaw = quat_yaw(bk.rot) - yaw_tar;
    float wy = dyaw - 6.28318530717959f * rintf(dyaw * 0.159154943091895f);
    float r_yaw = -wy * wy;
    float r_vel = -((bk.vb.x - vtx) * (bk.vb.x - vtx) + (bk.vb.y - vty) * (bk.vb.y - vty));
    float r_ang = -(bk.ab.z - atz) * (bk.ab.z - atz);
    float r_h = -(bk.pos.z - T.pos_tar[2]) * (bk.pos.z - T.pos_tar[2]);
    if (c.env_id == DIAL_ENV_GO2_WALK) {
      rew = 0.1f * r_gaits + 0.5f * r_upright + 0.3f * r_yaw + r_vel + r_ang + r_h;
    } else if (c.env_id == DIAL_ENV_H1_LOCO) {
      float atx = fminf(ang_cmd[0] * ramp, ang_cmd[0]), aty = fminf(ang_cmd[1] * ramp, ang_cmd[1]);
      float r_ang3 = -((bk.ab.x - atx) * (bk.ab.x - atx) + (bk.ab.y - aty) * (bk.ab.y - aty) + (bk.ab.z - atz) * (bk.ab.z - atz));
      float r_level = 0.f;
      for (int f = 0; f < c.nfeet; ++f) {
        const float* X = SM(xmat) + 9 * m.site_bodyid[c.feet_site[f]];
        r_level -= X[2] * X[2] + X[5] * X[5] + (X[8] - 1.f) * (X[8] - 1.f);
      }
      float r_energy = 0.f;
      for (int a = 0; a < m.nu; ++a) { float e = SM(ctrl)[a] / c.joint_torque_range[a][1] * SM(qvel)[6 + a] / 160.f; r_energy -= e * e; }
      rew = 10.f * r_gaits + 0.5f * r_upright + 0.5f * r_yaw + r_vel + r_ang3 + 0.5f * r_h + 0.02f * r_level + 0.01f * r_energy;
    } else {
      float r_energy = 0.f;
      for (int a = 0; a < m.nu; ++a) { float e = SM(ctrl)[a] / c.joint_torque_range[a][1]; r_energy -= e * e; }
      rew = 5.f * r_gaits + 0.5f * r_upright + 0.1f * r_yaw + r_vel + r_ang + 0.5f * r_h + 0.01f * r_energy;
    }
  } else {
    V3 dp = bk.pos - ld3(T.pose_seq[stage]);
    float r_pos = -dot(dp, dp);
    float dy = quat_yaw(bk.rot) - T.yaw_seq[stage];
    float r_yaw = -dy * dy;
    const float r_contact = part0, pen = part1;
    rew = r_pos + r_upright + 0.3f * r_yaw + 0.1f * r_contact - 0.1f * pen + 10.f;
    int ns = (int)floorf((float)(step + 1) * c.dt / T.jump_dt);
    stage = ns < T.n_stage - 1 ? ns : T.n_stage - 1;
  }
  return rew;
}

template <int NL, int NR>
DEV void rollout_warp(const DevModel* Mp, const DevPlan* Pp, float* slab, const RolloutArgs& A,
                      int row, int lane) {
  WarpCtx w;
  w.M = Mp; w.P = Pp; w.s = slab; w.lane = lane;
  w.midsync = A.lockstep >= 2;
  w.itersync = A.lockstep >= 3;
  w.dbg = A.dbg;
  const DevModel& M = *Mp;
  const dial_model_desc& m = M.m;
  const dial_plan_desc& c = Pp->c;
  const int nq = m.nq, nv = m.nv, nu = m.nu, nb = m.nbody;
  const int inst = A.rows_per_inst > 0 ? row / A.rows_per_inst : 0;
  const int lrow = row - inst * A.rows_per_inst;
  w.nch = 0; w.ndesc = 0; w.mylevel = -1; w.parent = -1;
#pragma unroll
  for (int i = 0; i < DIAL_MAXCHAIN; ++i) w.chain[i] = 0;
  if (lane < nv) {
    w.nch = M.dof_nchain[lane];
    w.ndesc = M.dof_ndesc[lane];
    w.mylevel = M.dof_level[lane];
    w.parent = m.dof_parentid[lane];
#pragma unroll
    for (int i = 0; i < DIAL_MAXCHAIN; ++i)
      if (i < w.nch) w.chain[i] = M.chain_tab[lane][i];
  }
  w.s_pos = 0; w.s_col = 0; w.s_cb = 0; w.s_chain = -2; w.s_depth = 0; w.s_top = 0; w.s_conmask = 0u; w.e_cb = 0;
  if constexpr (NL > 0) {
    using SD = StarDims<NL, NR>;
    w.s_cb = SD::NRP; w.e_cb = SD::NRP;
    if (lane < nv) {
      w.s_pos = M.s_pos[lane]; w.s_chain = M.s_chain[lane]; w.s_depth = M.s_depth[lane];
      if (w.s_chain >= 0) { w.s_cb = SD::NRP + w.s_chain * SD::CS; w.s_col = SD::NRP + w.s_depth; w.s_top = M.s_top[w.s_chain]; }
      else w.s_col = w.s_depth;
      for (int c = 0; c < m.ncon; ++c)
        if (w.s_chain < 0 || M.s_con_chain[c] == w.s_chain) w.s_conmask |= 1u << c;
    }
    if (lane < M.nedge) { const int cc = M.s_con_chain[lane >> 2]; if (cc >= 0) w.e_cb = SD::NRP + cc * SD::CS; }
    const int nz = 2 * M.s_npos * SD::RS + M.nedge * SD::RS + M.s_npos + 8;
    for (int i = lane; i < nz; i += 32) SM(Ms)[i] = 0.f;
    for (int i = lane; i < 32; i += 32) SM(frow)[i] = 0.f;
  }
  for (int i = lane; i < nq; i += 32) SM(qpos)[i] = A.qpos0[(size_t)inst * nq + i];
  for (int i = lane; i < nv; i += 32) { SM(qvel)[i] = A.qvel0[(size_t)inst * nv + i]; SM(warm)[i] = A.warm0[(size_t)inst * nv + i]; }
  if (lane == 0) {
    SM(xpos)[0] = SM(xpos)[1] = SM(xpos)[2] = 0.f;
    SM(xquat)[0] = 1.f; SM(xquat)[1] = SM(xquat)[2] = SM(xquat)[3] = 0.f;
    for (int i = 0; i < 9; ++i) SM(xmat)[i] = (i % 4 == 0) ? 1.f : 0.f;
    for (int i = 0; i < 3; ++i) SM(xipos)[i] = 0.f;
    for (int i = 0; i < 10; ++i) SM(cinert)[i] = 0.f;
    for (int i = 0; i < 6; ++i) { SM(cvel)[i] = 0.f; SM(cfrc)[i] = 0.f; }
    SM(cacc)[0] = SM(cacc)[1] = SM(cacc)[2] = 0.f;
    SM(cacc)[3] = -m.gravity[0]; SM(cacc)[4] = -m.gravity[1]; SM(cacc)[5] = -m.gravity[2];
  }
  syncwarp();

  const int Hn1 = c.Hnode + 1;
  float Y[DIAL_MAXNODE];
#pragma unroll
  for (int k = 0; k < DIAL_MAXNODE; ++k) Y[k] = 0.f;
  if (A.mode == 1 && lane < nu) {
    const bool is_mean = lrow == c.Nsample;
    const uint32_t gidx = (uint32_t)(c.shard_offset + lrow);
    const uint32_t ntot = (uint32_t)c.Ntotal * (uint32_t)Hn1 * (uint32_t)nu;
    uint32_t key0 = A.key_dev ? A.key_dev[2 * inst] : A.key0, key1 = A.key_dev ? A.key_dev[2 * inst + 1] : A.key1;
    if (A.rng_dev) split_key(A.rng_dev[2 * inst], A.rng_dev[2 * inst + 1], key0, key1);
#pragma unroll
    for (int k = 0; k < DIAL_MAXNODE; ++k) {
      if (k < Hn1) {
        float yb = A.Ybar[(inst * Hn1 + k) * nu + lane];
        float y = yb;
        if (!is_mean && k > 0) {
          uint32_t idx = (gidx * (uint32_t)Hn1 + (uint32_t)k) * (uint32_t)nu + (uint32_t)lane;
          float e = A.eps ? A.eps[idx] : jax_normal_legacy(key0, key1, idx, ntot);
          y = e * A.noise[k] + yb;
        }
        Y[k] = fminf(fmaxf(y, -1.f), 1.f);
      }
    }
  }

  int step = A.counters_in ? A.counters_in[2 * inst] : A.step0, stage = A.counters_in ? A.counters_in[2 * inst + 1] : A.stage0;
  float rsum = 0.f;
  const bool fwd_only = A.mode == 2;
  const int H = fwd_only ? 1 : A.H;
  const int nfr = fwd_only ? 1 : c.n_frames;
  for (int t = 0; t < H; ++t) {
    if (A.lockstep && (A.sync_every <= 1 || t % A.sync_every == 0)) cta_sync();
    if (lane < nu && fwd_only) SM(ctrl)[lane] = 0.f;
    if (lane < nu && !fwd_only) {
      float u;
      if (A.mode == 0) {
        u = A.us[(size_t)row * (A.us_row ? A.us_row : A.H * nu) + t * nu + lane];
      } else {
        u = 0.f;
#pragma unroll
        for (int k = 0; k < DIAL_MAXNODE; ++k)
          if (k < Hn1) u += c.M_n2u[t][k] * Y[k];
      }
      float an = (u * c.action_scale + 1.f) * 0.5f;
      float jt = c.joint_range[lane][0] + c.joint_offset[lane] + an * (c.joint_range[lane][1] - c.joint_range[lane][0]);
      jt = fminf(fmaxf(jt, c.physical_joint_range[lane][0]), c.physical_joint_range[lane][1]);
      float ctrl = jt;
      if (c.leg_control_torque) {
        float tau = c.kp[lane] * (jt - SM(qpos)[7 + lane]) - c.kd[lane] * SM(qvel)[6 + lane];
        ctrl = fminf(fmaxf(tau, c.joint_torque_range[lane][0]), c.joint_torque_range[lane][1]);
      }
      SM(ctrl)[lane] = ctrl;
    }
    syncwarp();
    for (int f = 0; f < nfr; ++f) physics_step<NL, NR>(w, !fwd_only);
    if (fwd_only) break;
    float rew = 0.f, part0, part1;
    const dial_task& T = A.tasks ? A.tasks[A.task_rows > 0 ? row / A.task_rows : 0] : plan_task(c);
    reward_partials(w, T, step, stage, part0, part1);
    if (lane == 0) rew = reward_lane0(w, T, step, stage, part0, part1);
    stage = shfl_i(stage, 0);
    step += 1;
    rsum += rew;
    size_t rt = (size_t)row * A.H + t;
    if (A.rewss && lane == 0) A.rewss[rt] = rew;
    if (A.q) for (int i = lane; i < nq; i += 32) A.q[rt * nq + i] = SM(qpos)[i];
    if (A.qd) for (int i = lane; i < nv; i += 32) A.qd[rt * nv + i] = SM(qvel)[i];
    if (A.xpos) for (int i = lane; i < 3 * (nb - 1); i += 32) A.xpos[rt * 3 * (nb - 1) + i] = SM(xpos)[3 + i];
  }
  if (A.rews && lane == 0 && !fwd_only) A.rews[row] = rsum / (float)A.H;
#ifndef DIAL_NO_XCH
  if (A.xch_world > 1 && lane == 0 && !fwd_only && A.mode == 1) {
    const float val = rsum / (float)A.H;
    const uint32_t buf = (*A.xch_seq) & 1u;
    const size_t base = (size_t)buf * (size_t)(c.Ntotal + 1);
    const bool sample = row < c.Nsample;
    const size_t slot = base + (size_t)(sample ? c.shard_offset + row : c.Ntotal);
    for (int p = 0; p < A.xch_world; ++p)
      if (sample || p == A.xch_rank) A.xch_mbox[p][slot] = val;
  }
#endif
  const int erow = shfl_i(row, 0), einst = A.rows_per_inst > 0 ? erow / A.rows_per_inst : 0;
  if (erow == einst * A.rows_per_inst) {
    const int inst = einst;
    if (A.qpos_out) for (int i = lane; i < nq; i += 32) A.qpos_out[(size_t)inst * nq + i] = SM(qpos)[i];
    if (A.qvel_out) for (int i = lane; i < nv; i += 32) A.qvel_out[(size_t)inst * nv + i] = SM(qvel)[i];
    if (A.warm_out) for (int i = lane; i < nv; i += 32) A.warm_out[(size_t)inst * nv + i] = SM(warm)[i];
    if (A.ctrl_out) for (int i = lane; i < nu; i += 32) A.ctrl_out[(size_t)inst * nu + i] = SM(ctrl)[i];
    if (A.kin_out && lane == 0) {
      const BaseKin bk = base_kin(w, c.torso_body);
      float* ko = A.kin_out + 13 * inst;
      ko[0] = bk.pos.x; ko[1] = bk.pos.y; ko[2] = bk.pos.z;
      ko[3] = bk.rot.w; ko[4] = bk.rot.x; ko[5] = bk.rot.y; ko[6] = bk.rot.z;
      ko[7] = bk.vb.x; ko[8] = bk.vb.y; ko[9] = bk.vb.z;
      ko[10] = bk.ab.x; ko[11] = bk.ab.y; ko[12] = bk.ab.z;
    }
    if (A.counters_out && lane == 0) { A.counters_out[2 * inst] = step; A.counters_out[2 * inst + 1] = stage; }
  }
}
```

dial_mpc_b200/csrc/dial_kernels.cu:

```cuda
#include <cuda_runtime.h>
#include <stdio.h>
#include <stdlib.h>
#include <string>
#include <vector>
#include <new>
#include "dial_host.h"
#define DIAL_STR2(x) #x
#define DIAL_STR(x) DIAL_STR2(x)

static thread_local std::string g_err;
static int fail(const std::string& s) { g_err = s; return -1; }
#define CUDA_OK(x) do { cudaError_t e_ = (x); if (e_ != cudaSuccess) return fail(std::string(#x) + ": " + cudaGetErrorString(e_)); } while (0)

#ifdef DIAL_ONLY_VARIANT
#define DIAL_HAS_VARIANT(v) ((v) == DIAL_ONLY_VARIANT)
#define DIAL_VARIANT DIAL_ONLY_VARIANT
#include "dial_rollout_variant.cu"
#else
#define DIAL_HAS_VARIANT(v) 1
#endif
#define DIAL_DECL_LAUNCH(v) cudaError_t dial_launch_rollout_v##v(const DevModel*, const DevPlan*, const RolloutArgs&, int, int, size_t, cudaStream_t);
#if DIAL_HAS_VARIANT(0)
DIAL_DECL_LAUNCH(0)
#endif
#if DIAL_HAS_VARIANT(1)
DIAL_DECL_LAUNCH(1)
#endif
#if DIAL_HAS_VARIANT(2)
DIAL_DECL_LAUNCH(2)
#endif
#if DIAL_HAS_VARIANT(3)
DIAL_DECL_LAUNCH(3)
#endif
#if DIAL_HAS_VARIANT(4)
DIAL_DECL_LAUNCH(4)
#endif

template <typename T, int K>
__device__ __forceinline__ void block_reduce(T (&v)[K], T* mx, T* red) {
  const int lane = threadIdx.x & 31, wid = threadIdx.x >> 5, nw = blockDim.x >> 5;
#pragma unroll
  for (int o = 16; o > 0; o >>= 1) {
#pragma unroll
    for (int k = 0; k < K; ++k) v[k] += __shfl_xor_sync(0xffffffffu, v[k], o);
    if (mx) *mx = fmax(*mx, __shfl_xor_sync(0xffffffffu, *mx, o));
  }
  __syncthreads();
  if (lane == 0) {
#pragma unroll
    for (int k = 0; k < K; ++k) red[k * 32 + wid] = v[k];
    if (mx) red[K * 32 + wid] = *mx;
  }
  __syncthreads();
#pragma unroll
  for (int k = 0; k < K; ++k) v[k] = lane < nw ? red[k * 32 + lane] : T(0);
  if (mx) *mx = lane < nw ? red[K * 32 + lane] : T(-INFINITY);
#pragma unroll
  for (int o = 16; o > 0; o >>= 1) {
#pragma unroll
    for (int k = 0; k < K; ++k) v[k] += __shfl_xor_sync(0xffffffffu, v[k], o);
    if (mx) *mx = fmax(*mx, __shfl_xor_sync(0xffffffffu, *mx, o));
  }
}

struct SoftmaxParams {
  float shift, inv, mx;
  bool none;
};
__device__ __noinline__ SoftmaxParams reward_softmax_params_fp64(const float* __restrict__ rews, int n, float temp,
                                                                 float rbar, float mean, float cnt, float* red_f) {
  double* red = reinterpret_cast<double*>(red_f);
  SoftmaxParams s;
  s.none = false;
  const double c = isfinite(mean) ? (double)rbar + (double)mean : 0.0;
  double s1[1] = {0.0}, s2[1] = {0.0}, rmax = -INFINITY;
  for (int i = threadIdx.x; i < n; i += blockDim.x) {
    const float r = __ldcg(rews + i);
    if (isfinite(r)) { const double d = (double)r - c; s1[0] += d; s2[0] += d * d; rmax = fmax(rmax, (double)r); }
  }
  block_reduce<double, 1>(s1, &rmax, red);
  block_reduce<double, 1>(s2, nullptr, red);
  const double m = s1[0] / (double)cnt, var64 = s2[0] / (double)cnt - m * m;
  s.shift = (float)rmax;
  s.mx = 0.f;
  s.inv = var64 > 0.0 ? (float)fmin(1.0 / (sqrt(var64) * (double)temp), 3.4028234663852886e38) : 0.f;
  return s;
}
__device__ __forceinline__ SoftmaxParams reward_softmax_params(const float* __restrict__ rews, int n, float temp,
                                                               float* red) {
  float rbar = __ldcg(rews + n - 1);
  const bool rbar_finite = isfinite(rbar);
  if (!rbar_finite) rbar = 0.f;
  float st[3] = {0.f, 0.f, 0.f}, dmax = -INFINITY;
  for (int i = threadIdx.x; i < n; i += blockDim.x) {
    const float r = __ldcg(rews + i);
    if (isfinite(r)) { const float d = r - rbar; st[0] += 1.f; st[1] += d; st[2] += d * d; dmax = fmaxf(dmax, d); }
  }
  block_reduce<float, 3>(st, &dmax, red);
  SoftmaxParams s;
  const float cnt = st[0];
  s.none = cnt == 0.f;
  const float mean = st[1] / fmaxf(cnt, 1.f);
  const float var = st[2] / fmaxf(cnt, 1.f) - mean * mean;
  const float sd = sqrtf(fmaxf(var, 0.f));
  if (s.none || (rbar_finite && isfinite(st[2]) && fabsf(mean) <= 8.f * sd)) {
    s.shift = rbar;
    s.inv = (sd > 0.f) ? 1.f / sd / temp : 0.f;
    s.mx = dmax * s.inv;
    return s;
  }
  return reward_softmax_params_fp64(rews, n, temp, rbar, mean, cnt, red);
}

struct XchWait {
  const float* mbox;
  const uint32_t* flags;
  uint32_t* seq;
  uint32_t* err;
// ... 246 lines not shown

__global__ void mpc_shift_kernel(const float* __restrict__ Msh, const float* __restrict__ Yin,
                                 float* __restrict__ Yout, int n1, int nu) {
  const int i = threadIdx.x;
  Yin += (size_t)blockIdx.x * n1 * nu; Yout += (size_t)blockIdx.x * n1 * nu;
  if (i < n1 * nu) {
    const int k = i / nu, a = i - k * nu;
    float s = 0.f;
    for (int j = 0; j < n1; ++j) s += Msh[k * n1 + j] * Yin[j * nu + a];
    Yout[i] = s;
  }
}

#define TB_CHUNKS 32
struct TrajArgs {
  const float* traj[3];
  float* out[3];
  int ncol[3], coloff[3];
  int coltot, nrows, H;
  const float* weights;
  int w_offset, mean_row, mean_weight_index, include_mean;
  float* partial;
};

template <bool BATCH>
__global__ void __launch_bounds__(256, 8) trajbar_partial_kernel(const TrajArgs T) {
  const int chunk = blockIdx.y, arr = BATCH ? blockIdx.z % 3 : blockIdx.z, inst = BATCH ? blockIdx.z / 3 : 0;
  const int ncol = arr == 0 ? T.ncol[0] : (arr == 1 ? T.ncol[1] : T.ncol[2]), len = T.H * ncol;
  const int coloff = arr == 0 ? T.coloff[0] : (arr == 1 ? T.coloff[1] : T.coloff[2]);
  const int j = blockIdx.x * 256 + threadIdx.x;
  if (blockIdx.x * 256 >= len) return;
  const float* __restrict__ traj = (arr == 0 ? T.traj[0] : (arr == 1 ? T.traj[1] : T.traj[2])) + (size_t)inst * T.nrows * len;
  const float* wts = BATCH ? T.weights + (size_t)inst * (T.mean_weight_index + 1) : T.weights;
  const int per = (T.nrows + TB_CHUNKS - 1) / TB_CHUNKS;
  const int r0 = chunk * per, r1 = min(T.nrows, r0 + per);
  const int jj = j < len ? j : len - 1;
  float a = 0.f;
  for (int r = r0; r < r1; r += 8) {
    float wv[8], xv[8];
#pragma unroll
    for (int k = 0; k < 8; ++k) {
      const int rr = r + k;
      float wgt = 0.f;
      if (rr < r1) {
        if (rr == T.mean_row) wgt = T.include_mean ? wts[T.mean_weight_index] : 0.f;
        else wgt = wts[T.w_offset + rr];
      }
      wv[k] = wgt;
    }
#pragma unroll
    for (int k = 0; k < 8; ++k)
      xv[k] = (wv[k] != 0.f) ? traj[(size_t)(r + k) * len + jj] : 0.f;
#pragma unroll
    for (int k = 0; k < 8; ++k) a += wv[k] * xv[k];
  }
  if (j < len) {
    const int t = j / ncol, c = j - t * ncol;
    T.partial[(((size_t)inst * TB_CHUNKS + chunk) * T.H + t) * T.coltot + coloff + c] = a;
  }
}

template <bool BATCH>
__global__ void __launch_bounds__(128, 8) trajbar_final_kernel(const TrajArgs T) {
  const int t = blockIdx.x, inst = BATCH ? blockIdx.y : 0;
  const float* partial = T.partial + (size_t)inst * TB_CHUNKS * T.H * T.coltot;
  for (int col = threadIdx.x; col < T.coltot; col += blockDim.x) {
    float s = 0.f;
#pragma unroll 8
    for (int ch = 0; ch < TB_CHUNKS; ++ch) s += partial[((size_t)ch * T.H + t) * T.coltot + col];
    float* out; int ncol, off;
    if (col >= T.coloff[2]) { out = T.out[2]; ncol = T.ncol[2]; off = T.coloff[2]; }
    else if (col >= T.coloff[1]) { out = T.out[1]; ncol = T.ncol[1]; off = T.coloff[1]; }
    else { out = T.out[0]; ncol = T.ncol[0]; off = T.coloff[0]; }
    if (out) out[((size_t)inst * T.H + t) * ncol + (col - off)] = s;
  }
}

struct dial_plan {
  DevModel hM;
  DevPlan hP;
  DevModel* dM = nullptr;
  DevPlan* dP = nullptr;
  int variant = 0;
  int n_inst = 1;
  int num_sms = 132;
  size_t smem_bytes = 0;
  float *traj_q[2] = {nullptr, nullptr}, *traj_qd[2] = {nullptr, nullptr}, *traj_x[2] = {nullptr, nullptr};
  int cur = 0;
  float* weights = nullptr;
  float* weights2 = nullptr;
  cudaStream_t side = nullptr;
  cudaEvent_t ev_main[2] = {nullptr, nullptr}, ev_side[2] = {nullptr, nullptr};
  float* partial = nullptr;
  float* tb_partial = nullptr;
  unsigned int* counter = nullptr;
  unsigned int* row_counter = nullptr;
  float* zeros = nullptr;
  int ybar_grid = 0;
  int upd_grid = 0;
  int64_t launches = 0;
  float* dbg = nullptr;
  dial_mpc_buffers mpc{};
  bool mpc_bound = false;
  float* mpc_Msh = nullptr;
  float* mpc_Y1 = nullptr;
  uint32_t* mpc_key = nullptr;
  struct MpcGraph { int n_diffuse, env_step, seen; cudaGraphExec_t exec; int64_t launches; };
  std::vector<MpcGraph> mpc_graphs;
  struct Exchange {
    bool on = false;
    int rank = 0, world = 1, nbar = 0;
    uint32_t* base[DIAL_MAXRANK] = {nullptr};
    size_t words = 0, o_mbox = 0, o_bars = 0, o_flags = 0, o_bflags = 0, o_local = 0;
    float* bars_partial = nullptr;
    float* mbox(int p) const { return reinterpret_cast<float*>(base[p] + o_mbox); }
    float* bars(int p) const { return reinterpret_cast<float*>(base[p] + o_bars); }
    uint32_t* flags(int p) const { return base[p] + o_flags; }
    uint32_t* bflags(int p) const { return base[p] + o_bflags; }
    uint32_t* seq() const { return base[rank] + o_local; }
    unsigned int* done() const { return base[rank] + o_local + 1; }
    uint32_t* err() const { return base[rank] + o_local + 2; }
    uint32_t* bseq() const { return base[rank] + o_local + 3; }
  } xch;
};

static void fill_xch(const dial_plan* p, RolloutArgs& A) {
  if (!p->xch.on) return;
  A.xch_world = p->xch.world; A.xch_rank = p->xch.rank;
  for (int r = 0; r < p->xch.world; ++r) { A.xch_mbox[r] = p->xch.mbox(r); A.xch_flags[r] = p->xch.flags(r); }
  A.xch_seq = p->xch.seq(); A.xch_done = p->xch.done();
}
static XchWait xch_wait_args(const dial_plan* p, float* rews_copy) {
  XchWait X; memset(&X, 0, sizeof(X));
  if (p->xch.on) {
    X.mbox = p->xch.mbox(p->xch.rank); X.flags = p->xch.flags(p->xch.rank); X.seq = p->xch.seq(); X.err = p->xch.err();
    X.rews_copy = rews_copy; X.world = p->xch.world;
  }
  return X;
}

extern "C" int dial_abi_version(void) { return DIAL_ABI_VERSION; }
extern "C" const char* dial_last_error(void) { return g_err.c_str(); }
extern "C" size_t dial_sizeof(int which) {
  return which == 0 ? sizeof(dial_model_desc) : which == 1 ? sizeof(dial_plan_desc) : which == 2 ? sizeof(dial_state)
       : which == 3 ? sizeof(dial_mpc_buffers) : which == 4 ? sizeof(dial_task) : 0;
}

static cudaError_t launch_rollout(dial_plan* p, const RolloutArgs& A, int wpc, cudaStream_t st) {
  const size_t smem = sizeof(DevModel) + sizeof(DevPlan) + (size_t)wpc * p->hM.warp_floats * sizeof(float);
  int grid = (A.nrows + wpc - 1) / wpc;
  if (A.row_counter) {
    const int resident = p->num_sms * (wpc > 8 ? 1 : 16 / wpc);
    grid = grid < resident ? grid : resident;
    cudaError_t e = cudaMemsetAsync(A.row_counter, 0, sizeof(unsigned int), st);
    if (e != cudaSuccess) return e;
  }
  p->launches++;
  switch (p->variant) {
#if DIAL_HAS_VARIANT(1)
    case 1: return dial_launch_rollout_v1(p->dM, p->dP, A, grid, wpc, smem, st);
#endif
#if DIAL_HAS_VARIANT(2)
    case 2: return dial_launch_rollout_v2(p->dM, p->dP, A, grid, wpc, smem, st);
#endif
#if DIAL_HAS_VARIANT(3)
    case 3: return dial_launch_rollout_v3(p->dM, p->dP, A, grid, wpc, smem, st);
#endif
#if DIAL_HAS_VARIANT(4)
    case 4: return dial_launch_rollout_v4(p->dM, p->dP, A, grid, wpc, smem, st);
#endif
#if DIAL_HAS_VARIANT(0)
    case 0: return dial_launch_rollout_v0(p->dM, p->dP, A, grid, wpc, smem, st);
#endif
    default: return cudaErrorInvalidDeviceFunction;
  }
}

static int default_wpc(const dial_plan* p, int nrows) {
  const int per_sm = (nrows + p->num_sms - 1) / p->num_sms;
  const size_t fixed = sizeof(DevModel) + sizeof(DevPlan), slab = (size_t)p->hM.warp_floats * sizeof(float);
  int maxw = DIAL_MAXTHREADS / 32;
  while (maxw > 1 && fixed + maxw * slab > 227 * 1024) --maxw;
  if (per_sm <= maxw) return per_sm;
  const int waves = (per_sm + maxw - 1) / maxw;
  return (per_sm + waves - 1) / waves;
}

static cudaError_t launch_rollout_any(dial_plan* p, const RolloutArgs& A0, cudaStream_t st) {
  RolloutArgs A = A0;
  const char* f = getenv("DIAL_WPC");
  int wpc = f ? atoi(f) : 0;
  if (wpc == 0) wpc = default_wpc(p, A.nrows);
  if (wpc < 1 || wpc > DIAL_MAXTHREADS / 32) return cudaErrorInvalidValue;
  A.lockstep = (wpc >= 2 && !getenv("DIAL_NO_LOCKSTEP")) ? 1 : 0;
  if (p->hM.dense && !A.lockstep && A.nrows > wpc * p->num_sms && !getenv("DIAL_NO_DYNAMIC_ROWS")) A.row_counter = p->row_counter;
  const bool mid = getenv("DIAL_MIDSYNC") ? true : (getenv("DIAL_NO_MIDSYNC") ? false : (p->hM.dense || !p->hM.s_on));
  if (A.lockstep && mid) A.lockstep = 2;
  { const char* se = getenv("DIAL_SYNC_EVERY"); A.sync_every = se ? atoi(se) : 1; if (A.sync_every < 1) A.sync_every = 1; }
  const char* dl = getenv("DIAL_DENSE_LOCKSTEP");
  if (A.lockstep == 2 && p->hM.dense && !(dl && atoi(dl) == 2)) A.lockstep = 3;
  return launch_rollout(p, A, wpc, st);
}

extern "C" dial_plan* dial_plan_create(const dial_model_desc* model, const dial_plan_desc* cfg) {
  if (!model || !cfg) { g_err = "null descriptor"; return nullptr; }
  dial_plan* p = new (std::nothrow) dial_plan();
  if (!p) { g_err = "out of memory"; return nullptr; }
  std::string err;
  if (!derive_model(*model, p->hM, err)) { g_err = err; delete p; return nullptr; }
  {
    int dev = 0, sms = 0;
    if (cudaGetDevice(&dev) == cudaSuccess && cudaDeviceGetAttribute(&sms, cudaDevAttrMultiProcessorCount, dev) == cudaSuccess && sms > 0)
      p->num_sms = sms;
  }
  p->variant = (getenv("DIAL_FORCE_GENERIC_TREE") && !p->hM.dense) ? 0 : star_variant(p->hM);
  if (p->variant < 0) { g_err = "this build instantiates the dense (elliptic) solver path for nv = " DIAL_STR(DIAL_DENSE_NV) " only (custom builds: dial_mpc_b200.custom compiles it for the model's nv)"; delete p; return nullptr; }
  memset(&p->hP, 0, sizeof(DevPlan));
  p->hP.c = *cfg;
  p->hP.c.cmd_step = -1;
  const dial_plan_desc& c = *cfg;
  if (c.Hsample + 1 > DIAL_MAXH || c.Hnode + 1 > DIAL_MAXNODE || c.Hnode < 1 || c.Nsample < 1 || c.Ntotal < c.Nsample ||
      c.n_frames < 1 || (c.Hnode + 1) * model->nu > YBAR_THREADS || c.n_stage > DIAL_MAXSTAGE) {
    g_err = "invalid plan configuration (Hsample/Hnode/Nsample/n_frames out of range)";
    delete p;
    return nullptr;
  }
  if (c.env_id < DIAL_ENV_GO2_WALK || c.env_id > DIAL_ENV_CUSTOM) { g_err = "unknown env_id"; delete p; return nullptr; }
#ifndef DIAL_CUSTOM_REWARD_FILE
  if (c.env_id == DIAL_ENV_CUSTOM) {
    g_err = "env_id DIAL_ENV_CUSTOM needs a library built with a reward source (dial_mpc_b200.custom.build_library); this is the stock build";
    delete p; return nullptr;
  }
#endif
#ifdef DIAL_ONLY_VARIANT
  if (p->variant != DIAL_ONLY_VARIANT) {
    g_err = "this custom build holds solver variant " + std::to_string(DIAL_ONLY_VARIANT) + " only, the model needs " + std::to_string(p->variant);
    delete p; return nullptr;
  }
#endif
  if (c.n_user < 0 || c.n_user > DIAL_MAXUSER) { g_err = "n_user out of range"; delete p; return nullptr; }
  if (c.n_inst < 0) { g_err = "n_inst must be >= 0 (0 or 1: a single instance)"; delete p; return nullptr; }
  if (c.n_inst > 1) {
    if (c.Ntotal != c.Nsample) { g_err = "a batched plan (n_inst > 1) cannot be sharded (Ntotal must equal Nsample)"; delete p; return nullptr; }
    if (c.Nsample + 1 > (1 << 17)) { g_err = "a batched plan (n_inst > 1) needs Nsample + 1 <= 131072 (the fused update)"; delete p; return nullptr; }
    if (c.n_inst > 65535 / 3 || (int64_t)c.n_inst * (c.Nsample + 1) > 0x7fffffff) {
      g_err = "n_inst too large: at most 21845 instances and 2^31 - 1 rows per rollout launch"; delete p; return nullptr;
    }
  }
  p->n_inst = c.n_inst > 1 ? c.n_inst : 1;
  auto bad = [&](cudaError_t e, const char* what) {
    g_err = std::string(what) + ": " + cudaGetErrorString(e);
    dial_plan_destroy(p);
    return (dial_plan*)nullptr;
  };
  cudaError_t e;
  if ((e = cudaMalloc(&p->dM, sizeof(DevModel))) != cudaSuccess) return bad(e, "cudaMalloc(model)");
  if ((e = cudaMalloc(&p->dP, sizeof(DevPlan))) != cudaSuccess) return bad(e, "cudaMalloc(plan)");
  if ((e = cudaMemcpy(p->dM, &p->hM, sizeof(DevModel), cudaMemcpyHostToDevice)) != cudaSuccess) return bad(e, "cudaMemcpy(model)");
  if ((e = cudaMemcpy(p->dP, &p->hP, sizeof(DevPlan), cudaMemcpyHostToDevice)) != cudaSuccess) return bad(e, "cudaMemcpy(plan)");
  const size_t B = (size_t)p->n_inst, rows = B * ((size_t)c.Nsample + 1), H = (size_t)c.Hsample + 1;
  const dial_model_desc& m = *model;
  for (int b = 0; b < 2; ++b) {
    if ((e = cudaMalloc(&p->traj_q[b], rows * H * m.nq * sizeof(float))) != cudaSuccess) return bad(e, "cudaMalloc(traj_q)");
    if ((e = cudaMalloc(&p->traj_qd[b], rows * H * m.nv * sizeof(float))) != cudaSuccess) return bad(e, "cudaMalloc(traj_qd)");
    if ((e = cudaMalloc(&p->traj_x[b], rows * H * 3 * (m.nbody - 1) * sizeof(float))) != cudaSuccess) return bad(e, "cudaMalloc(traj_x)");
  }
  if ((e = cudaMalloc(&p->weights, B * ((size_t)c.Ntotal + 1) * sizeof(float))) != cudaSuccess) return bad(e, "cudaMalloc(weights)");
  if ((e = cudaMalloc(&p->weights2, B * ((size_t)c.Ntotal + 1) * sizeof(float))) != cudaSuccess) return bad(e, "cudaMalloc(weights2)");
  if ((e = cudaStreamCreateWithFlags(&p->side, cudaStreamNonBlocking)) != cudaSuccess) return bad(e, "cudaStreamCreate(side)");
  for (int i = 0; i < 2; ++i) {
    if ((e = cudaEventCreateWithFlags(&p->ev_main[i], cudaEventDisableTiming)) != cudaSuccess) return bad(e, "cudaEventCreate");
    if ((e = cudaEventCreateWithFlags(&p->ev_side[i], cudaEventDisableTiming)) != cudaSuccess) return bad(e, "cudaEventCreate");
  }
  const int ne = (c.Hnode + 1) * m.nu, slots = YBAR_THREADS / ne;
  int g = (c.Ntotal + 1 + slots - 1) / slots;
  p->ybar_grid = g < 1 ? 1 : (g > 2 * p->num_sms ? 2 * p->num_sms : g);
  {
    int gu = (c.Ntotal + 1 + slots * 8 - 1) / (slots * 8);
    p->upd_grid = gu < 1 ? 1 : (gu > p->ybar_grid ? p->ybar_grid : gu);
  }
  if ((e = cudaMalloc(&p->partial, B * p->ybar_grid * (ne + 1) * sizeof(float))) != cudaSuccess) return bad(e, "cudaMalloc(partial)");
  if ((e = cudaMalloc(&p->tb_partial, B * TB_CHUNKS * H * (m.nq + m.nv + 3 * (m.nbody - 1)) * sizeof(float))) != cudaSuccess) return bad(e, "cudaMalloc(tb_partial)");
  if ((e = cudaMalloc(&p->counter, B * sizeof(unsigned int))) != cudaSuccess) return bad(e, "cudaMalloc(counter)");
  if ((e = cudaMemset(p->counter, 0, B * sizeof(unsigned int))) != cudaSuccess) return bad(e, "cudaMemset(counter)");
  if ((e = cudaMalloc(&p->row_counter, sizeof(unsigned int))) != cudaSuccess) return bad(e, "cudaMalloc(row_counter)");
  if (getenv("DIAL_DEBUG_COUNTERS")) {
    if ((e = cudaMalloc(&p->dbg, 8 * sizeof(float))) != cudaSuccess) return bad(e, "cudaMalloc(dbg)");
    cudaMemset(p->dbg, 0, 8 * sizeof(float));
  }
  if ((e = cudaMalloc(&p->zeros, DIAL_MAXV * sizeof(float))) != cudaSuccess) return bad(e, "cudaMalloc(zeros)");
  if ((e = cudaMemset(p->zeros, 0, DIAL_MAXV * sizeof(float))) != cudaSuccess) return bad(e, "cudaMemset(zeros)");
  return p;
}

extern "C" void dial_plan_destroy(dial_plan* p) {
  if (!p) return;
  cudaFree(p->dM); cudaFree(p->dP);
  for (int b = 0; b < 2; ++b) { cudaFree(p->traj_q[b]); cudaFree(p->traj_qd[b]); cudaFree(p->traj_x[b]); }
  for (auto& g : p->mpc_graphs) if (g.exec) cudaGraphExecDestroy(g.exec);
  for (int r = 0; r < DIAL_MAXRANK; ++r) {
    if (!p->xch.base[r]) continue;
    if (r == p->xch.rank) cudaFree(p->xch.base[r]); else cudaIpcCloseMemHandle(p->xch.base[r]);
  }
  cudaFree(p->xch.bars_partial);
  cudaFree(p->mpc_Msh); cudaFree(p->mpc_Y1); cudaFree(p->mpc_key);
  for (int i = 0; i < 2; ++i) { if (p->ev_main[i]) cudaEventDestroy(p->ev_main[i]); if (p->ev_side[i]) cudaEventDestroy(p->ev_side[i]); }
  if (p->side) cudaStreamDestroy(p->side);
  cudaFree(p->weights2);
  cudaFree(p->weights); cudaFree(p->partial); cudaFree(p->tb_partial); cudaFree(p->counter); cudaFree(p->row_counter); cudaFree(p->zeros); cudaFree(p->dbg);
  delete p;
}

static void fill_state(RolloutArgs& A, const dial_state* s) {
  A.qpos0 = s->qpos; A.qvel0 = s->qvel; A.warm0 = s->qacc_warmstart; A.step0 = s->step; A.stage0 = s->stage;
}

extern "C" int dial_rollout(dial_plan* p, const dial_state* s, const float* us, int B, int H, float* rewss,
                            float* q, float* qd, float* xpos, void* stream) {
  if (!p || !s || !us || !rewss) return fail("dial_rollout: null argument");
  if (B < 1 || H < 1) return fail("dial_rollout: B and H must be positive");
  RolloutArgs A; memset(&A, 0, sizeof(A));
  fill_state(A, s);
  A.nrows = B; A.H = H; A.mode = 0; A.us = us; A.rewss = rewss; A.q = q; A.qd = qd; A.xpos = xpos;
  CUDA_OK(launch_rollout_any(p, A, (cudaStream_t)stream));
  return 0;
}

extern "C" int dial_plan_set_command(dial_plan* p, int cmd_step, const float* vel, const float* ang, void* stream) {
  if (!p) return fail("dial_plan_set_command: null plan");
  if (cmd_step >= 0 && (!vel || !ang)) return fail("dial_plan_set_command: null command");
  dial_plan_desc& c = p->hP.c;
  c.cmd_step = cmd_step;
// ... 322 lines not shown
      weights_kernel<<<1, 1024, 0, st>>>(B.rews, c.Ntotal + 1, c.temp_sample, w, X);
      p->launches++;
      CUDA_OK(cudaGetLastError());
      ybar_kernel<<<p->ybar_grid, YBAR_THREADS, 0, st>>>(w, nullptr, 0u, 0u, Y[cur], noise, c.Ntotal, n1, nu,
                                                         p->partial, p->counter, Y[cur ^ 1], p->mpc_key);
      p->launches++;
      CUDA_OK(cudaGetLastError());
    }
    cur ^= 1;
    if (bars) {
      CUDA_OK(cudaEventRecord(p->ev_main[i & 1], st));
      CUDA_OK(cudaStreamWaitEvent(p->side, p->ev_main[i & 1], 0));
      int rc = enqueue_trajbar(p, w, p->xch.on ? p->xch.rank : 0, B.qbar, B.qdbar, B.xbar, p->side);
      if (rc) return rc;
      CUDA_OK(cudaEventRecord(p->ev_side[i & 1], p->side));
    }
  }
  if (cur != 0) CUDA_OK(cudaMemcpyAsync(Y[0], Y[1], (size_t)ni * n1 * nu * sizeof(float), cudaMemcpyDeviceToDevice, st));
  if (bars && n_diffuse > 0) {
    if (n_diffuse >= 2) CUDA_OK(cudaStreamWaitEvent(st, p->ev_side[(n_diffuse - 2) & 1], 0));
    CUDA_OK(cudaStreamWaitEvent(st, p->ev_side[(n_diffuse - 1) & 1], 0));
  }
  if (n_diffuse > 0 && wts[(n_diffuse - 1) & 1] != p->weights)
    CUDA_OK(cudaMemcpyAsync(p->weights, p->weights2, nw * sizeof(float), cudaMemcpyDeviceToDevice, st));
  return 0;
}

extern "C" int dial_mpc_step(dial_plan* p, int n_diffuse, int env_step, void* stream) {
  if (!p) return fail("dial_mpc_step: null plan");
  if (!p->mpc_bound) return fail("dial_mpc_step: call dial_mpc_bind first");
  if (n_diffuse < 0 || n_diffuse > 64) return fail("dial_mpc_step: n_diffuse out of range");
  if (env_step < 0 || env_step > 2) return fail("dial_mpc_step: env_step must be 0 (plan only), 1 (env step + shift) or 2 (shift only)");
  if (p->n_inst > 1 && getenv("DIAL_NO_FUSED_UPDATE")) return fail("dial_mpc_step: batched plans need the fused update (unset DIAL_NO_FUSED_UPDATE)");
  cudaStream_t st = (cudaStream_t)stream;
  dial_plan::MpcGraph* g = nullptr;
  for (auto& e : p->mpc_graphs) if (e.n_diffuse == n_diffuse && e.env_step == env_step) g = &e;
  if (!g) {
    p->mpc_graphs.push_back({n_diffuse, env_step, 1, nullptr, 0});
    return mpc_enqueue(p, n_diffuse, env_step, st);
  }
  if (!g->exec) {
    if (getenv("DIAL_NO_GRAPH")) return mpc_enqueue(p, n_diffuse, env_step, st);
    cudaStream_t cs;
    CUDA_OK(cudaStreamCreateWithFlags(&cs, cudaStreamNonBlocking));
    const int64_t l0 = p->launches;
    cudaError_t e = cudaStreamBeginCapture(cs, cudaStreamCaptureModeThreadLocal);
    if (e != cudaSuccess) { cudaStreamDestroy(cs); CUDA_OK(e); }
    int rc = mpc_enqueue(p, n_diffuse, env_step, cs);
    cudaGraph_t graph = nullptr;
    e = cudaStreamEndCapture(cs, &graph);
    cudaStreamDestroy(cs);
    g->launches = p->launches - l0;
    p->launches = l0;
    if (rc) { if (graph) cudaGraphDestroy(graph); return rc; }
    CUDA_OK(e);
    e = cudaGraphInstantiate(&g->exec, graph, 0);
    cudaGraphDestroy(graph);
    CUDA_OK(e);
  }
  CUDA_OK(cudaGraphLaunch(g->exec, st));
  p->launches += g->launches;
  return 0;
}

extern "C" void dial_key_split(const uint32_t key[2], uint32_t out0[2], uint32_t out1[2]) {
  uint32_t a0 = 0, b0 = 2, a1 = 1, b1 = 3;
  threefry2x32(key[0], key[1], a0, b0);
  threefry2x32(key[0], key[1], a1, b1);
  out0[0] = a0; out0[1] = a1; out1[0] = b0; out1[1] = b1;
}

extern "C" int dial_solver_variant(const dial_model_desc* model) {
  if (!model) return fail("null descriptor");
  DevModel* D = new (std::nothrow) DevModel();
  if (!D) return fail("out of memory");
  std::string err;
  int v = -1;
  if (!derive_model(*model, *D, err)) g_err = err;
  else if ((v = star_variant(*D)) < 0) g_err = "this build instantiates the dense (elliptic) solver path for nv = " DIAL_STR(DIAL_DENSE_NV) " only (custom builds: dial_mpc_b200.custom compiles it for the model's nv)";
  delete D;
  return v;
}

extern "C" const char* dial_custom_reward_id(void) {
#if defined(DIAL_CUSTOM_REWARD_FILE) && defined(DIAL_CUSTOM_REWARD_ID)
  return DIAL_STR(DIAL_CUSTOM_REWARD_ID);
#elif defined(DIAL_CUSTOM_REWARD_FILE)
  return "custom";
#else
  return "";
#endif
}

__global__ void __launch_bounds__(1024) fp32_peak_kernel(float* out, int iters, float a, float b) {
  float x[8];
#pragma unroll
  for (int i = 0; i < 8; ++i) x[i] = (float)(threadIdx.x + i) * 1e-3f;
  for (int it = 0; it < iters; ++it) {
#pragma unroll
    for (int r = 0; r < 16; ++r) {
#pragma unroll
      for (int i = 0; i < 8; ++i) x[i] = fmaf(x[i], a, b);
    }
  }
  float s = 0.f;
#pragma unroll
  for (int i = 0; i < 8; ++i) s += x[i];
  if (s == 123.456f) out[0] = s;
}

extern "C" int dial_fp32_peak(int iters, float* tflops_out) {
  if (!tflops_out || iters < 1) return fail("dial_fp32_peak: bad argument");
  int dev = 0, sms = 0;
  CUDA_OK(cudaGetDevice(&dev));
  CUDA_OK(cudaDeviceGetAttribute(&sms, cudaDevAttrMultiProcessorCount, dev));
  float* d = nullptr;
  CUDA_OK(cudaMalloc(&d, sizeof(float)));
  cudaEvent_t e0, e1;
  CUDA_OK(cudaEventCreate(&e0));
  CUDA_OK(cudaEventCreate(&e1));
  const int grid = sms * 2;
  fp32_peak_kernel<<<grid, 1024>>>(d, 64, 0.999f, 1e-3f);
  float best = 0.f;
  for (int rep = 0; rep < 3; ++rep) {
    cudaEventRecord(e0);
    fp32_peak_kernel<<<grid, 1024>>>(d, iters, 0.999f, 1e-3f);
    cudaEventRecord(e1);
    cudaError_t e = cudaEventSynchronize(e1);
    if (e != cudaSuccess) { cudaFree(d); return fail(std::string("fp32 peak kernel: ") + cudaGetErrorString(e)); }
    float ms = 0.f;
    cudaEventElapsedTime(&ms, e0, e1);
    const double flop = 2.0 * 8 * 16 * (double)iters * 1024.0 * grid;
    const float tf = (float)(flop / (ms * 1e-3) / 1e12);
    best = tf > best ? tf : best;
  }
  cudaEventDestroy(e0); cudaEventDestroy(e1); cudaFree(d);
  *tflops_out = best;
  return 0;
}

extern "C" int64_t dial_launch_count(const dial_plan* p) { return p ? p->launches : 0; }
extern "C" int dial_rollout_wpc(const dial_plan* p, int nrows) { return (p && nrows > 0) ? default_wpc(p, nrows) : 0; }

extern "C" int dial_debug_counters(dial_plan* p, float out[8]) {
  if (!p || !p->dbg) return fail("debug counters are off (set DIAL_DEBUG_COUNTERS=1 before dial_plan_create)");
  CUDA_OK(cudaMemcpy(out, p->dbg, 8 * sizeof(float), cudaMemcpyDeviceToHost));
  CUDA_OK(cudaMemset(p->dbg, 0, 8 * sizeof(float)));
  return 0;
}
```

dial_mpc_b200/csrc/dial_rollout_variant.cu:

```cuda
#include <cuda_runtime.h>
#include "dial_host.h"

#ifndef DIAL_VARIANT
#error "compile with -DDIAL_VARIANT=<0..4>"
#endif
#if DIAL_VARIANT == 1
#define DIAL_V_NL 3
#define DIAL_V_NR 6
#elif DIAL_VARIANT == 2
#define DIAL_V_NL 5
#define DIAL_V_NR 7
#elif DIAL_VARIANT == 3
#define DIAL_V_NL -1
#define DIAL_V_NR DIAL_DENSE_NV
#elif DIAL_VARIANT == 4
#define DIAL_V_NL 5
#define DIAL_V_NR 6
#else
#define DIAL_V_NL 0
#define DIAL_V_NR 0
#endif

__device__ __forceinline__ uint32_t smem_u32(const void* p) { return (uint32_t)__cvta_generic_to_shared(p); }
__device__ __forceinline__ void mbar_init(uint64_t* bar, int count) {
  asm volatile("mbarrier.init.shared::cta.b64 [%0], %1;" ::"r"(smem_u32(bar)), "r"(count));
  asm volatile("fence.mbarrier_init.release.cluster;" ::: "memory");
}
__device__ __forceinline__ void mbar_expect_tx(uint64_t* bar, uint32_t bytes) {
  asm volatile("mbarrier.arrive.expect_tx.shared::cta.b64 _, [%0], %1;" ::"r"(smem_u32(bar)), "r"(bytes) : "memory");
}
__device__ __forceinline__ void tma_bulk_g2s(void* dst, const void* src, uint32_t bytes, uint64_t* bar) {
  asm volatile("cp.async.bulk.shared::cluster.global.mbarrier::complete_tx::bytes [%0], [%1], %2, [%3];"
               ::"r"(smem_u32(dst)), "l"(src), "r"(bytes), "r"(smem_u32(bar)) : "memory");
}
__device__ __forceinline__ void mbar_wait(uint64_t* bar, uint32_t parity) {
  asm volatile(
      "{\n .reg .pred p;\n WAIT_%=:\n"
      " mbarrier.try_wait.parity.shared::cta.b64 p, [%0], %1;\n"
      " @p bra DONE_%=;\n bra WAIT_%=;\n DONE_%=:\n}\n" ::"r"(smem_u32(bar)), "r"(parity) : "memory");
}

static_assert(sizeof(DevModel) % 16 == 0, "DevModel must be a multiple of 16 bytes for cp.async.bulk");
static_assert(sizeof(DevPlan) % 16 == 0, "DevPlan must be a multiple of 16 bytes for cp.async.bulk");

template <int NL, int NR>
__global__ void __launch_bounds__(DIAL_MAXTHREADS, 1) rollout_kernel(const DevModel* __restrict__ gM,
                                                         const DevPlan* __restrict__ gP,
                                                         const RolloutArgs A) {
  extern __shared__ __align__(128) unsigned char smem[];
  __shared__ __align__(8) uint64_t bar;
  DevModel* sM = reinterpret_cast<DevModel*>(smem);
  DevPlan* sP = reinterpret_cast<DevPlan*>(smem + sizeof(DevModel));
  float* slabs = reinterpret_cast<float*>(smem + sizeof(DevModel) + sizeof(DevPlan));
  if (threadIdx.x == 0) {
    mbar_init(&bar, 1);
    mbar_expect_tx(&bar, (uint32_t)(sizeof(DevModel) + sizeof(DevPlan)));
    tma_bulk_g2s(sM, gM, (uint32_t)sizeof(DevModel), &bar);
    tma_bulk_g2s(sP, gP, (uint32_t)sizeof(DevPlan), &bar);
  }
  __syncthreads();
  mbar_wait(&bar, 0);
  const int warp = threadIdx.x >> 5, lane = threadIdx.x & 31, wpc = blockDim.x >> 5;
  float* slab = slabs + (size_t)warp * sM->warp_floats;
  if constexpr (NL < 0) {
    if (A.row_counter) {
      for (;;) {
        int row = 0;
        if (lane == 0) row = (int)atomicAdd(A.row_counter, 1u);
        row = __shfl_sync(0xffffffffu, row, 0);
        if (row >= A.nrows) return;
        rollout_warp<NL, NR>(sM, sP, slab, A, row, lane);
        __syncwarp();
      }
    }
  }
  int row = blockIdx.x * wpc + warp;
  bool active = true;
  if (row >= A.nrows) {
    active = A.lockstep != 0;
    row = A.nrows - 1;
  }
  if (active) rollout_warp<NL, NR>(sM, sP, slab, A, row, lane);
#ifndef DIAL_NO_XCH
  if (A.xch_world > 1) {
    __syncthreads();
    if (threadIdx.x == 0) {
      __threadfence_system();
      const unsigned int old = atomicAdd(A.xch_done, 1u);
      if (old == gridDim.x - 1) {
        __threadfence_system();
        const uint32_t seq = *A.xch_seq, buf = seq & 1u;
        for (int p = 0; p < A.xch_world; ++p)
          *reinterpret_cast<volatile uint32_t*>(A.xch_flags[p] + buf * DIAL_MAXRANK + A.xch_rank) = seq + 1u;
        *A.xch_done = 0u;
        __threadfence_system();
      }
    }
  }
#endif
}

#define DIAL_CAT2(a, b) a##b
#define DIAL_CAT(a, b) DIAL_CAT2(a, b)

cudaError_t DIAL_CAT(dial_launch_rollout_v, DIAL_VARIANT)(const DevModel* dM, const DevPlan* dP, const RolloutArgs& A,
                                                          int grid, int wpc, size_t smem, cudaStream_t st) {
  static size_t configured[64] = {0};
  int dev = 0;
  cudaError_t e = cudaGetDevice(&dev);
  if (e != cudaSuccess) return e;
  if (dev < 0 || dev >= 64 || smem > configured[dev]) {
    e = cudaFuncSetAttribute(rollout_kernel<DIAL_V_NL, DIAL_V_NR>, cudaFuncAttributeMaxDynamicSharedMemorySize, (int)smem);
    if (e != cudaSuccess) return e;
    if (dev >= 0 && dev < 64) configured[dev] = smem;
  }
  rollout_kernel<DIAL_V_NL, DIAL_V_NR><<<grid, wpc * 32, smem, st>>>(dM, dP, A);
  return cudaGetLastError();
}
```

include/dial_b200.h:

```cpp
#ifndef DIAL_B200_H_
#define DIAL_B200_H_

#include <stddef.h>
#include <stdint.h>

#ifdef __cplusplus
extern "C" {
#endif

#define DIAL_ABI_VERSION 11

#define DIAL_MAXB 24
#define DIAL_MAXV 28
#define DIAL_MAXQ 29
#define DIAL_MAXU 20
#define DIAL_MAXG 8
#define DIAL_MAXP 16
#define DIAL_MAXC 20
#define DIAL_MAXS 8
#define DIAL_MAXNODE 8
#define DIAL_MAXH 64
#define DIAL_MAXSTAGE 12
#define DIAL_MAXUSER 64
#define DIAL_MAXRANK 8
#define DIAL_IPC_HANDLE_BYTES 64

enum {
  DIAL_ENV_GO2_WALK = 0,
  DIAL_ENV_GO2_SEQJUMP = 1,
  DIAL_ENV_H1_WALK = 2,
  DIAL_ENV_ALLEGRO = 3,
  DIAL_ENV_H1_LOCO = 4,
  DIAL_ENV_CUSTOM = 5,
};

typedef struct dial_model_desc {
  int32_t nq, nv, nu, nbody, njnt, ngeom, nsite, npair, ncon;
  int32_t iterations, ls_iterations, eulerdamp, cone;
  float timestep, gravity[3], tolerance, ls_tolerance, impratio, meaninertia;
  int32_t body_parentid[DIAL_MAXB], body_rootid[DIAL_MAXB], body_depth[DIAL_MAXB];
  int32_t body_jntadr[DIAL_MAXB], body_dofadr[DIAL_MAXB], body_dofnum[DIAL_MAXB];
  float body_pos[DIAL_MAXB][3], body_quat[DIAL_MAXB][4];
  float body_ipos[DIAL_MAXB][3], body_iquat[DIAL_MAXB][4];
  float body_mass[DIAL_MAXB], body_inertia[DIAL_MAXB][3], body_invweight0[DIAL_MAXB];
  float body_invweight0_rot[DIAL_MAXB];
  int32_t jnt_type[DIAL_MAXB], jnt_qposadr[DIAL_MAXB], jnt_dofadr[DIAL_MAXB], jnt_limited[DIAL_MAXB];
  float jnt_pos[DIAL_MAXB][3], jnt_axis[DIAL_MAXB][3], jnt_range[DIAL_MAXB][2], jnt_margin[DIAL_MAXB];
  float jnt_solref[DIAL_MAXB][2], jnt_solimp[DIAL_MAXB][5];
  int32_t dof_bodyid[DIAL_MAXV], dof_jntid[DIAL_MAXV], dof_parentid[DIAL_MAXV];
  float dof_armature[DIAL_MAXV], dof_damping[DIAL_MAXV], dof_invweight0[DIAL_MAXV];
  float qpos0[DIAL_MAXQ];
  int32_t geom_type[DIAL_MAXG], geom_bodyid[DIAL_MAXG];
  float geom_pos[DIAL_MAXG][3], geom_quat[DIAL_MAXG][4], geom_size[DIAL_MAXG][3];
  int32_t pair_kind[DIAL_MAXP], pair_geom1[DIAL_MAXP], pair_geom2[DIAL_MAXP], pair_ncon[DIAL_MAXP];
  int32_t pair_condim[DIAL_MAXP];
  float pair_friction[DIAL_MAXP][5], pair_margin[DIAL_MAXP], pair_gap[DIAL_MAXP];
  float pair_solref[DIAL_MAXP][2], pair_solimp[DIAL_MAXP][5];
  int32_t site_bodyid[DIAL_MAXS];
  float site_pos[DIAL_MAXS][3];
  int32_t actuator_dofadr[DIAL_MAXU], actuator_qposadr[DIAL_MAXU];
  int32_t actuator_ctrllimited[DIAL_MAXU], actuator_forcelimited[DIAL_MAXU];
  float actuator_gear[DIAL_MAXU], actuator_gain[DIAL_MAXU], actuator_bias[DIAL_MAXU][3];
  float actuator_ctrlrange[DIAL_MAXU][2], actuator_forcerange[DIAL_MAXU][2];
} dial_model_desc;

typedef struct dial_plan_desc {
  int32_t env_id;
  int32_t Nsample;
  int32_t Ntotal;
  int32_t shard_offset;
  int32_t Hsample, Hnode;
  int32_t n_frames;
  int32_t leg_control_torque;
  float temp_sample;
  float dt, action_scale;
  float kp[DIAL_MAXU], kd[DIAL_MAXU];
  float joint_range[DIAL_MAXU][2];
  float physical_joint_range[DIAL_MAXU][2];
  float joint_torque_range[DIAL_MAXU][2];
  float joint_offset[DIAL_MAXU];
  float M_n2u[DIAL_MAXH][DIAL_MAXNODE];
  int32_t torso_body;
  int32_t nfeet;
  int32_t feet_site[4];
  float ramp_up_time;
  float vel_cmd[3], ang_cmd[3], pos_tar[3];
  float gait_duty, gait_cadence, gait_amplitude, gait_phase[4];
  int32_t cmd_step;
  float cmd_vel[3], cmd_ang[3];
  int32_t n_stage;
  float jump_dt;
  float pose_seq[DIAL_MAXSTAGE][3], yaw_seq[DIAL_MAXSTAGE];
  float contact_targets[DIAL_MAXSTAGE][4][3], contact_radius[DIAL_MAXSTAGE][4];
// ... 26 lines not shown
typedef struct dial_plan dial_plan;

int dial_abi_version(void);
const char* dial_last_error(void);
size_t dial_sizeof(int which);

dial_plan* dial_plan_create(const dial_model_desc* model, const dial_plan_desc* cfg);
void dial_plan_destroy(dial_plan* plan);

int dial_rollout(dial_plan* plan, const dial_state* s, const float* us, int B, int H,
                 float* rewss, float* q, float* qd, float* xpos, void* stream);

int dial_env_step(dial_plan* plan, const dial_state* s, const float* action,
                  float* qpos_out, float* qvel_out, float* warm_out, float* reward,
                  float* ctrl_out, void* stream);

int dial_plan_set_command(dial_plan* plan, int cmd_step, const float vel[3], const float ang[3], void* stream);

int dial_plan_set_stages(dial_plan* plan, int n_stage, const float* pose_seq, const float* yaw_seq,
                         const float* contact_targets, const float* contact_radius, void* stream);

int dial_plan_get_task(const dial_plan* plan, dial_task* out);

int dial_env_step_kin(dial_plan* plan, const dial_state* s, const float* action,
                      float* qpos_out, float* qvel_out, float* warm_out, float* reward,
                      float* ctrl_out, float* kin_out, void* stream);

int dial_pipeline_init(dial_plan* plan, const float* qpos, const float* qvel,
                       float* qpos_out, float* warm_out, void* stream);

int dial_reverse_rollout(dial_plan* plan, const dial_state* s, const float* eps,
                         const uint32_t key[2], const float* Ybar ,
                         const float* noise_scale , float* rews_local,
                         void* stream);

int dial_reverse_update(dial_plan* plan, const float* eps, const uint32_t key[2],
                        const float* Ybar, const float* noise_scale, const float* rews_all,
                        float* Ybar_out, float* weights, void* stream);

int dial_reverse_update_x(dial_plan* plan, const float* eps, const uint32_t key[2],
                          const float* Ybar, const float* noise_scale, const float* rews_all,
                          float* Ybar_out, float* weights, float* rews_gathered, void* stream);

int dial_reverse_update_fused(dial_plan* plan, const float* rews, uint32_t* rng, const float* Ybar,
                              const float* noise_scale, float* Ybar_out, float* weights, void* stream);

int dial_reverse_trajbar(dial_plan* plan, const float* weights, int rank,
                         float* qbar, float* qdbar, float* xbar, void* stream);

int dial_reverse_trajectories(dial_plan* plan, float* q, float* qd, float* xpos, void* stream);

int dial_exchange_create(dial_plan* plan, int rank, int world, unsigned char handle_out[DIAL_IPC_HANDLE_BYTES]);
int dial_exchange_connect(dial_plan* plan, const unsigned char* handles);
int dial_exchange_status(dial_plan* plan, uint32_t out[6]);

typedef struct dial_mpc_buffers {
  float* qpos;
  float* qvel;
  float* qacc_warmstart;
  int32_t* counters;
  uint32_t* rng;
  float* Y;
  float* ctrl;
  float* reward;
  float* rews;
  float* rews_all;
  float* qbar;
  float* qdbar;
  float* xbar;
  const float* noise;
  const dial_task* tasks;
} dial_mpc_buffers;

int dial_mpc_bind(dial_plan* plan, const dial_mpc_buffers* buffers, const float* M_shift);

int dial_mpc_step(dial_plan* plan, int n_diffuse, int env_step, void* stream);

void dial_key_split(const uint32_t key[2], uint32_t out0[2], uint32_t out1[2]);

int dial_debug_counters(dial_plan* plan, float out[8]);

int dial_solver_variant(const dial_model_desc* model);

const char* dial_custom_reward_id(void);

int dial_fp32_peak(int iters, float* tflops_out);

int64_t dial_launch_count(const dial_plan* plan);
int dial_rollout_wpc(const dial_plan* plan, int nrows);

#ifdef __cplusplus
}
#endif
#endif
```

Baseline: 67.41 million.

## Compile a shape-specialised Go2 rollout kernel with model dimensions as constants

Adds a ShapeFixed traits class whose model dimensions (bodies, dofs, chains, contact count, pair kind, solver iteration counts) come from compile-time defines derived from the Go2 model. The rollout, physics step, collision and solver routines are templated on it, and the plan selects the specialised kernel at runtime when the loaded model matches. The aim is to let the compiler unroll loops and fold branches that currently depend on runtime model fields. It adds an extra build object and a runtime structural match check, and falls back to the generic kernel when the model does not match.

```diff
diff --git a/__graft_entry__.py b/__graft_entry__.py
--- a/__graft_entry__.py
+++ b/__graft_entry__.py
@@ -35,13 +35,22 @@
         f.write(digest)
 
 
+def _shape_defines():
+    if ROOT not in sys.path:
+        sys.path.insert(0, ROOT)
+    from dial_mpc_b200.modelc.shape import SHAPES, env_structure_defines
+    return [(name, env_structure_defines(env)) for name, env in SHAPES]
+
+
 def build_library(force: bool = False, extra=(), lib: str = LIB, objdir: str = OBJDIR) -> None:
     extra = list(extra)
     tag = " " + " ".join(extra)
     hdrs = [os.path.join(CSRC, f) for f in ("dial_device.cuh", "dial_host.h")] + [os.path.join(ROOT, "include", "dial_b200.h")]
     var_src = os.path.join(CSRC, "dial_rollout_variant.cu")
     abi_src = os.path.join(CSRC, "dial_kernels.cu")
-    lib_digest = _digest(hdrs + [var_src, abi_src], tag)
+    shapes = _shape_defines()
+    shape_tag = "".join(f" {name}:" + ",".join(d) for name, d in shapes)
+    lib_digest = _digest(hdrs + [var_src, abi_src], tag + shape_tag)
     if not (force or _stale(lib, lib_digest)):
         return
     nvcc = os.environ.get("NVCC", "/usr/local/cuda/bin/nvcc")
@@ -51,6 +60,11 @@
         obj = os.path.join(objdir, f"rollout_v{v}.o")
         jobs.append((obj, _digest(hdrs + [var_src], f" variant={v}" + tag),
                      [nvcc] + NVCC_FLAGS + extra + [f"-DDIAL_VARIANT={v}", "-c", "-o", obj, var_src]))
+    for name, defs in shapes:
+        obj = os.path.join(objdir, f"rollout_{name}.o")
+        flags = ["-DDIAL_VARIANT=1", f"-DDIAL_SHAPE_NAME={name}"] + [f"-D{d}" for d in defs]
+        jobs.append((obj, _digest(hdrs + [var_src], " " + " ".join(flags) + tag),
+                     [nvcc] + NVCC_FLAGS + extra + flags + ["-c", "-o", obj, var_src]))
     obj = os.path.join(objdir, "dial_kernels.o")
     jobs.append((obj, _digest(hdrs + [abi_src], tag), [nvcc] + NVCC_FLAGS + extra + ["-c", "-o", obj, abi_src]))
     running = [(o, d, subprocess.Popen(cmd)) for o, d, cmd in jobs if force or _stale(o, d)]
diff --git a/dial_mpc_b200/_capi.py b/dial_mpc_b200/_capi.py
--- a/dial_mpc_b200/_capi.py
+++ b/dial_mpc_b200/_capi.py
@@ -211,6 +211,8 @@
     lib.dial_solver_variant.argtypes = [C.POINTER(dial_model_desc)]
     lib.dial_solver_variant.restype = C.c_int
     lib.dial_custom_reward_id.restype = C.c_char_p
+    lib.dial_plan_rollout_kernel.argtypes = [V]
+    lib.dial_plan_rollout_kernel.restype = C.c_char_p
     lib.dial_mpc_bind.argtypes = [V, C.POINTER(dial_mpc_buffers), P]
     lib.dial_mpc_bind.restype = C.c_int
     lib.dial_mpc_step.argtypes = [V, I, I, V]
@@ -248,4 +250,5 @@
            "dial_env_step", "dial_env_step_kin", "dial_plan_set_command", "dial_plan_set_stages", "dial_pipeline_init", "dial_reverse_rollout", "dial_reverse_update", "dial_reverse_update_x",
            "dial_reverse_update_fused", "dial_exchange_create", "dial_exchange_connect", "dial_exchange_status",
            "dial_reverse_trajbar", "dial_reverse_trajectories", "dial_key_split", "dial_fp32_peak", "dial_launch_count", "dial_rollout_wpc", "dial_debug_counters",
-           "dial_solver_variant", "dial_custom_reward_id", "dial_mpc_bind", "dial_mpc_step", "dial_plan_get_task"]
+           "dial_solver_variant", "dial_custom_reward_id", "dial_mpc_bind", "dial_mpc_step", "dial_plan_get_task",
+           "dial_plan_rollout_kernel"]
diff --git a/dial_mpc_b200/csrc/dial_device.cuh b/dial_mpc_b200/csrc/dial_device.cuh
--- a/dial_mpc_b200/csrc/dial_device.cuh
+++ b/dial_mpc_b200/csrc/dial_device.cuh
@@ -136,6 +136,65 @@
   unsigned int* xch_done;
 };
 
+struct ShapeRT {
+  static HD int nbody(const DevModel& M) { return M.m.nbody; }
+  static HD int nq(const DevModel& M) { return M.m.nq; }
+  static HD int nv(const DevModel& M) { return M.m.nv; }
+  static HD int nu(const DevModel& M) { return M.m.nu; }
+  static HD int maxdepth(const DevModel& M) { return M.maxdepth; }
+  static HD int nroot(const DevModel& M) { return M.nroot; }
+  static HD int ncon(const DevModel& M) { return M.m.ncon; }
+  static HD int nedge(const DevModel& M) { return M.nedge; }
+  static HD int nchain(const DevModel& M) { return M.star_nchain; }
+  static HD int sb_on(const DevModel& M) { return M.sb_on; }
+  static HD int sb_nroot(const DevModel& M) { return M.sb_nroot; }
+  static HD int sb_len(const DevModel& M, int l) { return M.sb_len[l]; }
+  static HD int pair_kind(const DevModel& M, int k) { return M.m.pair_kind[k]; }
+  static HD int iterations(const DevModel& M) { return M.m.iterations; }
+  static HD int ls_iterations(const DevModel& M) { return M.m.ls_iterations; }
+  static HD int n_frames(const dial_plan_desc& c) { return c.n_frames; }
+  static HD int env_id(const dial_plan_desc& c) { return c.env_id; }
+  static HD int nfeet(const dial_plan_desc& c) { return c.nfeet; }
+};
+
+#ifdef DIAL_SHAPE_NBODY
+namespace {
+struct ShapeFixed : ShapeRT {
+  static HD constexpr int nbody(const DevModel&) { return DIAL_SHAPE_NBODY; }
+  static HD constexpr int nq(const DevModel&) { return DIAL_SHAPE_NQ; }
+  static HD constexpr int nv(const DevModel&) { return DIAL_SHAPE_NV; }
+  static HD constexpr int nu(const DevModel&) { return DIAL_SHAPE_NU; }
+  static HD constexpr int maxdepth(const DevModel&) { return DIAL_SHAPE_MAXDEPTH; }
+  static HD constexpr int nroot(const DevModel&) { return DIAL_SHAPE_NROOT; }
+  static HD constexpr int nchain(const DevModel&) { return DIAL_SHAPE_NCHAIN; }
+  static HD constexpr int sb_on(const DevModel&) { return 1; }
+  static HD constexpr int sb_nroot(const DevModel&) { return DIAL_SHAPE_SB_NROOT; }
+  static HD constexpr int sb_len(const DevModel&, int) { return DIAL_SHAPE_CHAINLEN; }
+  static HD constexpr int pair_kind(const DevModel&, int) { return DIAL_SHAPE_PAIR_KIND; }
+  static HD constexpr int iterations(const DevModel&) { return DIAL_SHAPE_ITERATIONS; }
+  static HD constexpr int ls_iterations(const DevModel&) { return DIAL_SHAPE_LS_ITERATIONS; }
+};
+}
+#endif
+
+template <class SH>
+static inline bool shape_matches(const DevModel& M, const dial_plan_desc& c) {
+  using R = ShapeRT;
+  if (!M.s_on || !R::sb_on(M) || SH::sb_on(M) != R::sb_on(M)) return false;
+  if (SH::nbody(M) != R::nbody(M) || SH::nq(M) != R::nq(M) || SH::nv(M) != R::nv(M) || SH::nu(M) != R::nu(M) ||
+      SH::maxdepth(M) != R::maxdepth(M) || SH::nroot(M) != R::nroot(M) || SH::ncon(M) != R::ncon(M) ||
+      SH::nedge(M) != R::nedge(M) || SH::nchain(M) != R::nchain(M) || SH::sb_nroot(M) != R::sb_nroot(M) ||
+      SH::iterations(M) != R::iterations(M) || SH::ls_iterations(M) != R::ls_iterations(M) ||
+      SH::n_frames(c) != R::n_frames(c) || SH::env_id(c) != R::env_id(c) || SH::nfeet(c) != R::nfeet(c))
+    return false;
+  for (int l = 0; l < R::nchain(M); ++l) if (SH::sb_len(M, l) != R::sb_len(M, l)) return false;
+  for (int k = 0; k < R::ncon(M); ++k) {
+    const int p = M.con_pair[k];
+    if (SH::pair_kind(M, p) != R::pair_kind(M, p)) return false;
+  }
+  return true;
+}
+
 struct V3 { float x, y, z; };
 struct Q4 { float w, x, y, z; };
 
@@ -735,7 +794,7 @@
   for (int i = 0; i < SD::RS; i += 4) st4(p + i, t[i], t[i + 1], t[i + 2], t[i + 3]);
 }
 
-template <int NL, int NR, bool WITH_M, bool WITH_J>
+template <int NL, int NR, bool WITH_M, bool WITH_J, class SH = ShapeRT>
 DEV void star_mul_MJ(WarpCtx& w, const float* Mr, const float* Mc, float x, float& Mx, float& Jx) {
   using SD = StarDims<NL, NR>;
   const DevModel& M = *w.M;
@@ -757,7 +816,7 @@
     for (int q = 0; q < NL; ++q) { if (q & 1) y3 += Mc[q] * xc[q]; else y2 += Mc[q] * xc[q]; }
   } else if (w.s_chain == -1) {
     const float* col = Ms + SD::NRP * SD::RS + w.s_col;
-    const int nslot = M.star_nchain * SD::CS;
+    const int nslot = SH::nchain(M) * SD::CS;
     for (int s0 = 0; s0 < nslot; s0 += 4) {
       F4 xv = ld4(xs + SD::NRP + s0);
       y0 += col[(s0 + 0) * SD::RS] * xv.x; y1 += col[(s0 + 1) * SD::RS] * xv.y;
@@ -769,7 +828,7 @@
   Mx = y;
   if (WITH_J) {
     float j = 0.f;
-    if (w.lane < M.nedge) {
+    if (w.lane < SH::nedge(M)) {
       const float* row = SM(Js) + w.lane * SD::RS;
       float jr[SD::NRP], jc[SD::CS], xe[SD::CS];
       ldv<NR>(row, jr);
@@ -786,7 +845,7 @@
   }
 }
 
-template <int NL, int NR>
+template <int NL, int NR, class SH = ShapeRT>
 DEV float star_mul_JT(WarpCtx& w, float f) {
   using SD = StarDims<NL, NR>;
   const DevModel& M = *w.M;
@@ -797,7 +856,7 @@
   syncwarp();
   float y0 = 0.f, y1 = 0.f, y2 = 0.f, y3 = 0.f;
   const float* col = Js + w.s_col;
-  for (int c = 0; c < M.m.ncon; ++c) {
+  for (int c = 0; c < SH::ncon(M); ++c) {
     const F4 fv = ld4(frow + 4 * c);
     if ((w.s_conmask >> c) & 1u) {
       const float* jc = col + 4 * c * SD::RS;
@@ -807,7 +866,7 @@
   return (y0 + y1) + (y2 + y3);
 }
 
-template <int NL, int NR>
+template <int NL, int NR, class SH = ShapeRT>
 DEV void star_build_H(WarpCtx& w, const Solver& S, const float* Mr, const float* Mc, float* Rr, float* Rc) {
   using SD = StarDims<NL, NR>;
   const DevModel& M = *w.M;
@@ -828,7 +887,7 @@
 #pragma unroll
     for (int a = 0; a < NR; ++a) Rr[a] += (a == w.s_depth) ? ld : 0.f;
   }
-  for (int e = 0; e < M.nedge; ++e) {
+  for (int e = 0; e < SH::nedge(M); ++e) {
     const float de = frow[e];
     if (de == 0.f) continue;
     const float* row = Js + e * SD::RS;
@@ -844,7 +903,7 @@
   }
 }
 
-template <int NL, int NR>
+template <int NL, int NR, class SH = ShapeRT>
 DEV float star_solve2(WarpCtx& w, const float* Rr, const float* Rc, float g) {
   using SD = StarDims<NL, NR>;
   static_assert(NR + 1 <= 8, "root block + rhs must fit the 8 lanes of a group");
@@ -859,7 +918,7 @@
   }
   syncwarp();
   const int grp = lane >> 3, j = lane & 7, gbase = lane & ~7;
-  const bool ischain = grp < M.star_nchain;
+  const bool ischain = grp < SH::nchain(M);
   const int len = ischain ? M.star_len[grp] : 0;
   const int cb = SD::NRP + grp * SD::CS;
   float A[NL][NL], wv[NL];
@@ -983,11 +1042,11 @@
   return w.s_chain >= -1 ? xs[w.s_pos] : 0.f;
 }
 
-template <int NL, int NR>
+template <int NL, int NR, class SH = ShapeRT>
 DEV void star_update_constraint(WarpCtx& w, Solver& S) {
   float fl = (S.l_Jaref < 0.f) ? -S.l_D * S.l_Jaref : 0.f;
   float fe = (S.e_Jaref < 0.f) ? -S.e_D * S.e_Jaref : 0.f;
-  float qfc = star_mul_JT<NL, NR>(w, fe) + S.l_sign * fl;
+  float qfc = star_mul_JT<NL, NR, SH>(w, fe) + S.l_sign * fl;
   S.grad = S.Ma - S.qfs - qfc;
   float g = (S.Ma - S.qfs) * (S.qacc - S.qas);
   float c = ((S.l_Jaref < 0.f) ? S.l_D * S.l_Jaref * S.l_Jaref : 0.f)
@@ -1063,9 +1122,10 @@
   }
 }
 
+template <class SH = ShapeRT>
 DEV void linesearch_core(WarpCtx& w, Solver& S, float mv, float e_jv) {
   const DevModel& M = *w.M;
-  const int nv = M.m.nv;
+  const int nv = SH::nv(M);
   const float scale = M.m.meaninertia * (float)(nv > 1 ? nv : 1);
   float l_jv = S.l_sign * S.search;
   float ss = S.search * S.search, sMa = S.search * (S.Ma - S.qfs), sMv = S.search * mv;
@@ -1082,7 +1142,8 @@
   ls_points<1, false>(w.lane, S, K, l_jv, e_jv, qg, a1, &lo);
   if (lo.d0 < p0.d0) { hi = p0; } else { hi = lo; lo = p0; }
   bool swap = true;
-  for (int it = 0; it < M.m.ls_iterations; ++it) {
+#pragma unroll 1
+  for (int it = 0; it < SH::ls_iterations(M); ++it) {
     bool done = !swap;
     done |= (lo.d0 < 0.f) && (lo.d0 > -gtol);
     done |= (hi.d0 > 0.f) && (hi.d0 < gtol);
@@ -1758,11 +1819,12 @@
   return vnormalize(alt - n * dot(n, alt), bn);
 }
 
+template <class SH = ShapeRT>
 DEV void collide(WarpCtx& w) {
   const DevModel& M = *w.M;
   const dial_model_desc& m = M.m;
   const int lane = w.lane;
-  if (lane >= m.ncon) return;
+  if (lane >= SH::ncon(M)) return;
   const float* xpos = SM(xpos);
   const float* xmat = SM(xmat);
   const int k = M.con_pair[lane];
@@ -1772,7 +1834,7 @@
   const float* X2 = xmat + 9 * b2;
   const V3 gp1 = mat_apply(X1, m.geom_pos[g1]) + ld3(xpos + 3 * b1);
   const V3 gp2 = mat_apply(X2, m.geom_pos[g2]) + ld3(xpos + 3 * b2);
-  const int kind = m.pair_kind[k];
+  const int kind = SH::pair_kind(M, k);
   V3 n, t1, p;
   float dist;
   if (kind == PAIR_PLANE_SPHERE || kind == PAIR_PLANE_CAPSULE) {
@@ -1818,12 +1880,12 @@
   st3(SM(cframe) + 9 * lane + 6, cross(n, t1));
 }
 
-template <int NL, int NR>
+template <int NL, int NR, class SH = ShapeRT>
 DEV void physics_step(WarpCtx& w, bool integrate) {
   constexpr int MCU = (NL == 3 && NR == 6) ? 9 : DIAL_MAXCHAIN;
   const DevModel& M = *w.M;
   const dial_model_desc& m = M.m;
-  const int lane = w.lane, nb = m.nbody, nv = m.nv;
+  const int lane = w.lane, nb = SH::nbody(M), nv = SH::nv(M);
   float* xpos = SM(xpos); float* xquat = SM(xquat); float* xmat = SM(xmat); float* xipos = SM(xipos);
   float* cinert = SM(cinert); float* cdof = SM(cdof); float* cdofdot = SM(cdofdot);
   float* cvel = SM(cvel); float* cacc = SM(cacc); float* cfrc = SM(cfrc);
@@ -1862,7 +1924,7 @@
   }
   V3 pos = v3(0, 0, 0);
   Q4 quat; quat.w = 1.f; quat.x = quat.y = quat.z = 0.f;
-  for (int lv = 1; lv <= M.maxdepth; ++lv) {
+  for (int lv = 1; lv <= SH::maxdepth(M); ++lv) {
     if (depth == lv) {
       if (jtype == JNT_FREE) {
         const int qa = m.jnt_qposadr[jid];
@@ -1898,7 +1960,7 @@
 
   const int myroot = isbody ? M.body_rootidx[b] : -1;
   V3 com = v3(0, 0, 0);
-  for (int r = 0; r < M.nroot; ++r) {
+  for (int r = 0; r < SH::nroot(M); ++r) {
     float mass = (myroot == r) ? m.body_mass[b] : 0.f;
     float sx = mass * xip.x, sy = mass * xip.y, sz = mass * xip.z;
     warp_sum3(sx, sy, sz);
@@ -1951,7 +2013,7 @@
   syncwarp();
 
   float mycv[6] = {0.f, 0.f, 0.f, 0.f, 0.f, 0.f}, myca[6] = {0.f, 0.f, 0.f, 0.f, 0.f, 0.f};
-  for (int lv = 1; lv <= M.maxdepth; ++lv) {
+  for (int lv = 1; lv <= SH::maxdepth(M); ++lv) {
     if (depth == lv) {
       int p = m.body_parentid[b];
       float cv[6], ca[6];
@@ -2022,18 +2084,18 @@
     const float* src = comp < 10 ? cinert + comp : cfrc + (comp - 10);
     const int stride = comp < 10 ? CIS : 6;
     float* dst = comp < 10 ? crb + comp : cfs + (comp - 10);
-    if (NL > 0 && M.sb_on) {
-      for (int l = half; l < M.star_nchain; l += 2) {
+    if (NL > 0 && SH::sb_on(M)) {
+      for (int l = half; l < SH::nchain(M); l += 2) {
         const int top = M.sb_top[l];
         float acc = 0.f;
-        for (int k = M.sb_len[l] - 1; k >= 0; --k) { acc += src[(top + k) * stride]; dst[(top + k) * stride] = acc; }
+        for (int k = SH::sb_len(M, l) - 1; k >= 0; --k) { acc += src[(top + k) * stride]; dst[(top + k) * stride] = acc; }
       }
       syncwarp();
       if (half == 0) {
         float below = 0.f;
-        for (int r = 0; r < M.sb_nroot; ++r) {
+        for (int r = 0; r < SH::sb_nroot(M); ++r) {
           float acc = src[M.sb_root[r] * stride] + below;
-          for (int l = 0; l < M.star_nchain; ++l)
+          for (int l = 0; l < SH::nchain(M); ++l)
             if (M.sb_att[l] == r) acc += dst[M.sb_top[l] * stride];
           dst[M.sb_root[r] * stride] = acc;
           below = acc;
@@ -2053,7 +2115,7 @@
   }
   syncwarp();
 
-  collide(w);
+  collide<SH>(w);
   syncwarp();
 
   Solver S;
@@ -2164,7 +2226,7 @@
   if (isdof) {
     V3 ca_ = v3(mycdof[0], mycdof[1], mycdof[2]), cl_ = v3(mycdof[3], mycdof[4], mycdof[5]);
     V3 rc = ld3(rcom + 3 * M.body_rootidx[m.dof_bodyid[d]]);
-    for (int c = 0; c < m.ncon; ++c) {
+    for (int c = 0; c < SH::ncon(M); ++c) {
       if (!((w.s_conmask >> c) & 1u)) continue;
       const int k = M.con_pair[c];
       float e0 = 0.f, e1 = 0.f, e2 = 0.f, e3 = 0.f;
@@ -2196,8 +2258,8 @@
     }
   }
   float ejv, dummy;
-  star_mul_MJ<NL, NR, false, true>(w, Mr, Mc, myqvel, dummy, ejv);
-  if (lane < M.nedge) {
+  star_mul_MJ<NL, NR, false, true, SH>(w, Mr, Mc, myqvel, dummy, ejv);
+  if (lane < SH::nedge(M)) {
     int c = lane >> 2;
     int k = M.con_pair[c];
     float pos = cdist[c] - (m.pair_margin[k] - m.pair_gap[k]);
@@ -2224,13 +2286,13 @@
   int it = 0;
   bool done;
   {
-    float x = star_solve2<NL, NR>(w, Rr, Rc, g);
+    float x = star_solve2<NL, NR, SH>(w, Rr, Rc, g);
     S.qas = x;
-    if (M.nedge == 0 && M.nlimited == 0) { S.qacc = x; done = true; }
+    if (SH::nedge(M) == 0 && M.nlimited == 0) { S.qacc = x; done = true; }
     else {
       float Maw, eJw, eJs;
-      star_mul_MJ<NL, NR, true, true>(w, Mr, Mc, mywarm, Maw, eJw);
-      star_mul_MJ<NL, NR, false, true>(w, Mr, Mc, S.qas, dummy, eJs);
+      star_mul_MJ<NL, NR, true, true, SH>(w, Mr, Mc, mywarm, Maw, eJw);
+      star_mul_MJ<NL, NR, false, true, SH>(w, Mr, Mc, S.qas, dummy, eJs);
       eJw -= S.e_aref; eJs -= S.e_aref;
       float lJw = S.l_sign * mywarm - S.l_aref;
       float gw = (Maw - S.qfs) * (mywarm - S.qas);
@@ -2246,9 +2308,9 @@
       S.l_Jaref = usewarm ? lJw : lJs;
       S.cost = INFINITY;
       S.prev_cost = 0.f;
-      star_update_constraint<NL, NR>(w, S);
+      star_update_constraint<NL, NR, SH>(w, S);
       done = false;
-      if (m.iterations != 1) {
+      if (SH::iterations(M) != 1) {
         float improvement = (S.prev_cost - S.cost) / scale;
         float gradient = sqrtf(S.gradnorm2) / scale;
         done = (improvement < m.tolerance) || (gradient < m.tolerance);
@@ -2256,18 +2318,18 @@
     }
   }
   while (!done) {
-    star_build_H<NL, NR>(w, S, Mr, Mc, Rr, Rc);
-    float x = star_solve2<NL, NR>(w, Rr, Rc, S.grad);
+    star_build_H<NL, NR, SH>(w, S, Mr, Mc, Rr, Rc);
+    float x = star_solve2<NL, NR, SH>(w, Rr, Rc, S.grad);
     S.search = -x;
     float mv, e_jv;
-    star_mul_MJ<NL, NR, true, true>(w, Mr, Mc, S.search, mv, e_jv);
-    linesearch_core(w, S, mv, e_jv);
+    star_mul_MJ<NL, NR, true, true, SH>(w, Mr, Mc, S.search, mv, e_jv);
+    linesearch_core<SH>(w, S, mv, e_jv);
     ++it;
-    star_update_constraint<NL, NR>(w, S);
-    done = it >= m.iterations;
+    star_update_constraint<NL, NR, SH>(w, S);
+    done = it >= SH::iterations(M);
     float improvement = (S.prev_cost - S.cost) / scale;
     float gradient = sqrtf(S.gradnorm2) / scale;
-    if (m.iterations != 1) done = done || (improvement < m.tolerance) || (gradient < m.tolerance);
+    if (SH::iterations(M) != 1) done = done || (improvement < m.tolerance) || (gradient < m.tolerance);
   }
   qacc = S.qacc;
   qacc_int = qacc;
@@ -2436,24 +2498,26 @@
 #include DIAL_CUSTOM_REWARD_FILE
 #endif
 
+template <class SH = ShapeRT>
 DEV void reward_partials(WarpCtx& w, const dial_task& T, int step, int stage, float& p0, float& p1) {
   const DevModel& M = *w.M;
   const dial_plan_desc& c = w.P->c;
   const dial_model_desc& m = M.m;
   const float stepf = (float)step;
   const int f = w.lane;
+  const int env = SH::env_id(c);
   p0 = 0.f; p1 = 0.f;
-  if (c.env_id == DIAL_ENV_GO2_WALK || c.env_id == DIAL_ENV_H1_WALK || c.env_id == DIAL_ENV_H1_LOCO) {
-    if (f < c.nfeet) {
+  if (env == DIAL_ENV_GO2_WALK || env == DIAL_ENV_H1_WALK || env == DIAL_ENV_H1_LOCO) {
+    if (f < SH::nfeet(c)) {
       float zt = foot_step(T.gait_duty, T.gait_cadence, T.gait_amplitude, T.gait_phase[f], stepf * c.dt);
       float z;
-      if (c.env_id == DIAL_ENV_GO2_WALK) {
+      if (env == DIAL_ENV_GO2_WALK) {
         int sid = c.feet_site[f], sb = m.site_bodyid[sid];
         const float* X = SM(xmat) + 9 * sb;
         z = SM(xpos)[3 * sb + 2] + X[6] * m.site_pos[sid][0] + X[7] * m.site_pos[sid][1] + X[8] * m.site_pos[sid][2];
         float e = (zt - z) / 0.05f;
         p0 = -e * e;
-      } else if (c.env_id == DIAL_ENV_H1_WALK) {
+      } else if (env == DIAL_ENV_H1_WALK) {
         z = fminf(SM(cdist)[2 * f], SM(cdist)[2 * f + 1]);
         p0 = -(zt - z) * (zt - z);
       } else {
@@ -2461,7 +2525,7 @@
         p0 = -(zt - z) * (zt - z);
       }
     }
-  } else if (c.env_id == DIAL_ENV_GO2_SEQJUMP) {
+  } else if (env == DIAL_ENV_GO2_SEQJUMP) {
     if (f < 4) {
       const int i = f;
       float dist = SM(cdist)[i];
@@ -2482,14 +2546,16 @@
   p0 += shfl_xor(p0, 2); p1 += shfl_xor(p1, 2);
 }
 
+template <class SH = ShapeRT>
 DEV float reward_lane0(WarpCtx& w, const dial_task& T, int step, int& stage, float part0, float part1) {
   const DevModel& M = *w.M;
   const dial_plan_desc& c = w.P->c;
   const dial_model_desc& m = M.m;
   const float stepf = (float)step;
+  const int env = SH::env_id(c);
   float rew = 0.f;
 #ifdef DIAL_CUSTOM_REWARD_FILE
-  if (c.env_id == DIAL_ENV_CUSTOM) {
+  if (env == DIAL_ENV_CUSTOM) {
     dial_reward_ctx x;
     x.step = step; x.dt = c.dt;
     x.nq = m.nq; x.nv = m.nv; x.nu = m.nu; x.nbody = m.nbody; x.ncon = m.ncon; x.nsite = m.nsite; x.n_user = T.n_user;
@@ -2506,16 +2572,16 @@
   V3 up = qrot(rot0, v3(0, 0, 1));
   float r_upright = -(up.x * up.x + up.y * up.y + (up.z - 1.f) * (up.z - 1.f));
   BaseKin bk = base_kin(w, c.torso_body);
-  if (c.env_id == DIAL_ENV_ALLEGRO) {
+  if (env == DIAL_ENV_ALLEGRO) {
     const int ob = c.torso_body;
     V3 wv = ld3(SM(cvel) + 6 * ob) * (3.14159265358979f / 180.f);
     V3 dw = wv - ld3(T.ang_cmd);
     V3 dp = ld3(SM(xpos) + 3 * ob) - ld3(T.pos_tar);
     float rj = 0.f;
-    for (int a = 0; a < m.nu; ++a) { float e = SM(qpos)[7 + a] - c.joint_offset[a]; rj -= e * e; }
+    for (int a = 0; a < SH::nu(M); ++a) { float e = SM(qpos)[7 + a] - c.joint_offset[a]; rj -= e * e; }
     return -dot(dw, dw) - 5.f * dot(dp, dp) + 0.1f * rj;
   }
-  if (c.env_id == DIAL_ENV_GO2_WALK || c.env_id == DIAL_ENV_H1_WALK || c.env_id == DIAL_ENV_H1_LOCO) {
+  if (env == DIAL_ENV_GO2_WALK || env == DIAL_ENV_H1_WALK || env == DIAL_ENV_H1_LOCO) {
     float ramp = stepf * c.dt / c.ramp_up_time;
     const float* vel_cmd = step == T.cmd_step ? T.cmd_vel : T.vel_cmd;
     const float* ang_cmd = step == T.cmd_step ? T.cmd_ang : T.ang_cmd;
@@ -2529,22 +2595,22 @@
     float r_vel = -((bk.vb.x - vtx) * (bk.vb.x - vtx) + (bk.vb.y - vty) * (bk.vb.y - vty));
     float r_ang = -(bk.ab.z - atz) * (bk.ab.z - atz);
     float r_h = -(bk.pos.z - T.pos_tar[2]) * (bk.pos.z - T.pos_tar[2]);
-    if (c.env_id == DIAL_ENV_GO2_WALK) {
+    if (env == DIAL_ENV_GO2_WALK) {
       rew = 0.1f * r_gaits + 0.5f * r_upright + 0.3f * r_yaw + r_vel + r_ang + r_h;
-    } else if (c.env_id == DIAL_ENV_H1_LOCO) {
+    } else if (env == DIAL_ENV_H1_LOCO) {
       float atx = fminf(ang_cmd[0] * ramp, ang_cmd[0]), aty = fminf(ang_cmd[1] * ramp, ang_cmd[1]);
       float r_ang3 = -((bk.ab.x - atx) * (bk.ab.x - atx) + (bk.ab.y - aty) * (bk.ab.y - aty) + (bk.ab.z - atz) * (bk.ab.z - atz));
       float r_level = 0.f;
-      for (int f = 0; f < c.nfeet; ++f) {
+      for (int f = 0; f < SH::nfeet(c); ++f) {
         const float* X = SM(xmat) + 9 * m.site_bodyid[c.feet_site[f]];
         r_level -= X[2] * X[2] + X[5] * X[5] + (X[8] - 1.f) * (X[8] - 1.f);
       }
       float r_energy = 0.f;
-      for (int a = 0; a < m.nu; ++a) { float e = SM(ctrl)[a] / c.joint_torque_range[a][1] * SM(qvel)[6 + a] / 160.f; r_energy -= e * e; }
+      for (int a = 0; a < SH::nu(M); ++a) { float e = SM(ctrl)[a] / c.joint_torque_range[a][1] * SM(qvel)[6 + a] / 160.f; r_energy -= e * e; }
       rew = 10.f * r_gaits + 0.5f * r_upright + 0.5f * r_yaw + r_vel + r_ang3 + 0.5f * r_h + 0.02f * r_level + 0.01f * r_energy;
     } else {
       float r_energy = 0.f;
-      for (int a = 0; a < m.nu; ++a) { float e = SM(ctrl)[a] / c.joint_torque_range[a][1]; r_energy -= e * e; }
+      for (int a = 0; a < SH::nu(M); ++a) { float e = SM(ctrl)[a] / c.joint_torque_range[a][1]; r_energy -= e * e; }
       rew = 5.f * r_gaits + 0.5f * r_upright + 0.1f * r_yaw + r_vel + r_ang + 0.5f * r_h + 0.01f * r_energy;
     }
   } else {
@@ -2560,7 +2626,7 @@
   return rew;
 }
 
-template <int NL, int NR>
+template <int NL, int NR, class SH = ShapeRT>
 DEV void rollout_warp(const DevModel* Mp, const DevPlan* Pp, float* slab, const RolloutArgs& A,
                       int row, int lane) {
   WarpCtx w;
@@ -2571,7 +2637,7 @@
   const DevModel& M = *Mp;
   const dial_model_desc& m = M.m;
   const dial_plan_desc& c = Pp->c;
-  const int nq = m.nq, nv = m.nv, nu = m.nu, nb = m.nbody;
+  const int nq = SH::nq(M), nv = SH::nv(M), nu = SH::nu(M), nb = SH::nbody(M);
   const int inst = A.rows_per_inst > 0 ? row / A.rows_per_inst : 0;
   const int lrow = row - inst * A.rows_per_inst;
   w.nch = 0; w.ndesc = 0; w.mylevel = -1; w.parent = -1;
@@ -2594,11 +2660,11 @@
       w.s_pos = M.s_pos[lane]; w.s_chain = M.s_chain[lane]; w.s_depth = M.s_depth[lane];
       if (w.s_chain >= 0) { w.s_cb = SD::NRP + w.s_chain * SD::CS; w.s_col = SD::NRP + w.s_depth; w.s_top = M.s_top[w.s_chain]; }
       else w.s_col = w.s_depth;
-      for (int c = 0; c < m.ncon; ++c)
+      for (int c = 0; c < SH::ncon(M); ++c)
         if (w.s_chain < 0 || M.s_con_chain[c] == w.s_chain) w.s_conmask |= 1u << c;
     }
-    if (lane < M.nedge) { const int cc = M.s_con_chain[lane >> 2]; if (cc >= 0) w.e_cb = SD::NRP + cc * SD::CS; }
-    const int nz = 2 * M.s_npos * SD::RS + M.nedge * SD::RS + M.s_npos + 8;
+    if (lane < SH::nedge(M)) { const int cc = M.s_con_chain[lane >> 2]; if (cc >= 0) w.e_cb = SD::NRP + cc * SD::CS; }
+    const int nz = 2 * M.s_npos * SD::RS + SH::nedge(M) * SD::RS + M.s_npos + 8;
     for (int i = lane; i < nz; i += 32) SM(Ms)[i] = 0.f;
     for (int i = lane; i < 32; i += 32) SM(frow)[i] = 0.f;
   }
@@ -2645,7 +2711,7 @@
   float rsum = 0.f;
   const bool fwd_only = A.mode == 2;
   const int H = fwd_only ? 1 : A.H;
-  const int nfr = fwd_only ? 1 : c.n_frames;
+  const int nfr = fwd_only ? 1 : SH::n_frames(c);
   for (int t = 0; t < H; ++t) {
     if (A.lockstep && (A.sync_every <= 1 || t % A.sync_every == 0)) cta_sync();
     if (lane < nu && fwd_only) SM(ctrl)[lane] = 0.f;
@@ -2670,12 +2736,12 @@
       SM(ctrl)[lane] = ctrl;
     }
     syncwarp();
-    for (int f = 0; f < nfr; ++f) physics_step<NL, NR>(w, !fwd_only);
+    for (int f = 0; f < nfr; ++f) physics_step<NL, NR, SH>(w, !fwd_only);
     if (fwd_only) break;
     float rew = 0.f, part0, part1;
     const dial_task& T = A.tasks ? A.tasks[A.task_rows > 0 ? row / A.task_rows : 0] : plan_task(c);
-    reward_partials(w, T, step, stage, part0, part1);
-    if (lane == 0) rew = reward_lane0(w, T, step, stage, part0, part1);
+    reward_partials<SH>(w, T, step, stage, part0, part1);
+    if (lane == 0) rew = reward_lane0<SH>(w, T, step, stage, part0, part1);
     stage = shfl_i(stage, 0);
     step += 1;
     rsum += rew;
diff --git a/dial_mpc_b200/csrc/dial_kernels.cu b/dial_mpc_b200/csrc/dial_kernels.cu
--- a/dial_mpc_b200/csrc/dial_kernels.cu
+++ b/dial_mpc_b200/csrc/dial_kernels.cu
@@ -34,6 +34,18 @@
 #endif
 #if DIAL_HAS_VARIANT(4)
 DIAL_DECL_LAUNCH(4)
+#endif
+#ifndef DIAL_ONLY_VARIANT
+typedef cudaError_t (*dial_launch_fn)(const DevModel*, const DevPlan*, const RolloutArgs&, int, int, size_t, cudaStream_t);
+#define DIAL_DECL_SHAPE(s) \
+  cudaError_t dial_launch_rollout_##s(const DevModel*, const DevPlan*, const RolloutArgs&, int, int, size_t, cudaStream_t); \
+  bool dial_shape_matches_##s(const DevModel&, const dial_plan_desc&);
+DIAL_DECL_SHAPE(go2)
+static const struct {
+  const char* name;
+  dial_launch_fn launch;
+  bool (*matches)(const DevModel&, const dial_plan_desc&);
+} kShapes[] = {{"go2", dial_launch_rollout_go2, dial_shape_matches_go2}};
 #endif
 
 template <typename T, int K>
@@ -446,6 +458,7 @@
   DevModel* dM = nullptr;
   DevPlan* dP = nullptr;
   int variant = 0;
+  int shape = 0;
   int n_inst = 1;
   int num_sms = 132;
   size_t smem_bytes = 0;
@@ -520,6 +533,9 @@
     if (e != cudaSuccess) return e;
   }
   p->launches++;
+#ifndef DIAL_ONLY_VARIANT
+  if (p->shape > 0) return kShapes[p->shape - 1].launch(p->dM, p->dP, A, grid, wpc, smem, st);
+#endif
   switch (p->variant) {
 #if DIAL_HAS_VARIANT(1)
     case 1: return dial_launch_rollout_v1(p->dM, p->dP, A, grid, wpc, smem, st);
@@ -612,6 +628,11 @@
     }
   }
   p->n_inst = c.n_inst > 1 ? c.n_inst : 1;
+#ifndef DIAL_ONLY_VARIANT
+  if (p->variant == 1 && !getenv("DIAL_FORCE_GENERIC_SHAPE"))
+    for (int s = 0; s < (int)(sizeof(kShapes) / sizeof(kShapes[0])); ++s)
+      if (kShapes[s].matches(p->hM, p->hP.c)) { p->shape = s + 1; break; }
+#endif
   auto bad = [&](cudaError_t e, const char* what) {
     g_err = std::string(what) + ": " + cudaGetErrorString(e);
     dial_plan_destroy(p);
@@ -1100,6 +1121,15 @@
   return v;
 }
 
+extern "C" const char* dial_plan_rollout_kernel(const dial_plan* p) {
+  static const char* const generic[] = {"v0", "v1", "v2", "v3", "v4"};
+  if (!p) return "";
+#ifndef DIAL_ONLY_VARIANT
+  if (p->shape > 0) return kShapes[p->shape - 1].name;
+#endif
+  return p->variant >= 0 && p->variant <= 4 ? generic[p->variant] : "";
+}
+
 extern "C" const char* dial_custom_reward_id(void) {
 #if defined(DIAL_CUSTOM_REWARD_FILE) && defined(DIAL_CUSTOM_REWARD_ID)
   return DIAL_STR(DIAL_CUSTOM_REWARD_ID);
diff --git a/dial_mpc_b200/csrc/dial_rollout_variant.cu b/dial_mpc_b200/csrc/dial_rollout_variant.cu
--- a/dial_mpc_b200/csrc/dial_rollout_variant.cu
+++ b/dial_mpc_b200/csrc/dial_rollout_variant.cu
@@ -43,7 +43,7 @@
 static_assert(sizeof(DevModel) % 16 == 0, "DevModel must be a multiple of 16 bytes for cp.async.bulk");
 static_assert(sizeof(DevPlan) % 16 == 0, "DevPlan must be a multiple of 16 bytes for cp.async.bulk");
 
-template <int NL, int NR>
+template <int NL, int NR, class SH = ShapeRT>
 __global__ void __launch_bounds__(DIAL_MAXTHREADS, 1) rollout_kernel(const DevModel* __restrict__ gM,
                                                          const DevPlan* __restrict__ gP,
                                                          const RolloutArgs A) {
@@ -80,7 +80,7 @@
     active = A.lockstep != 0;
     row = A.nrows - 1;
   }
-  if (active) rollout_warp<NL, NR>(sM, sP, slab, A, row, lane);
+  if (active) rollout_warp<NL, NR, SH>(sM, sP, slab, A, row, lane);
 #ifndef DIAL_NO_XCH
   if (A.xch_world > 1) {
     __syncthreads();
@@ -103,17 +103,28 @@
 #define DIAL_CAT2(a, b) a##b
 #define DIAL_CAT(a, b) DIAL_CAT2(a, b)
 
-cudaError_t DIAL_CAT(dial_launch_rollout_v, DIAL_VARIANT)(const DevModel* dM, const DevPlan* dP, const RolloutArgs& A,
-                                                          int grid, int wpc, size_t smem, cudaStream_t st) {
+#ifdef DIAL_SHAPE_NAME
+#define DIAL_V_SHAPE ShapeFixed
+#define DIAL_V_LAUNCHER DIAL_CAT(dial_launch_rollout_, DIAL_SHAPE_NAME)
+bool DIAL_CAT(dial_shape_matches_, DIAL_SHAPE_NAME)(const DevModel& M, const dial_plan_desc& c) {
+  return shape_matches<ShapeFixed>(M, c);
+}
+#else
+#define DIAL_V_SHAPE ShapeRT
+#define DIAL_V_LAUNCHER DIAL_CAT(dial_launch_rollout_v, DIAL_VARIANT)
+#endif
+
+cudaError_t DIAL_V_LAUNCHER(const DevModel* dM, const DevPlan* dP, const RolloutArgs& A,
+                            int grid, int wpc, size_t smem, cudaStream_t st) {
   static size_t configured[64] = {0};
   int dev = 0;
   cudaError_t e = cudaGetDevice(&dev);
   if (e != cudaSuccess) return e;
   if (dev < 0 || dev >= 64 || smem > configured[dev]) {
-    e = cudaFuncSetAttribute(rollout_kernel<DIAL_V_NL, DIAL_V_NR>, cudaFuncAttributeMaxDynamicSharedMemorySize, (int)smem);
+    e = cudaFuncSetAttribute(rollout_kernel<DIAL_V_NL, DIAL_V_NR, DIAL_V_SHAPE>, cudaFuncAttributeMaxDynamicSharedMemorySize, (int)smem);
     if (e != cudaSuccess) return e;
     if (dev >= 0 && dev < 64) configured[dev] = smem;
   }
-  rollout_kernel<DIAL_V_NL, DIAL_V_NR><<<grid, wpc * 32, smem, st>>>(dM, dP, A);
+  rollout_kernel<DIAL_V_NL, DIAL_V_NR, DIAL_V_SHAPE><<<grid, wpc * 32, smem, st>>>(dM, dP, A);
   return cudaGetLastError();
 }
diff --git a/dial_mpc_b200/modelc/shape.py b/dial_mpc_b200/modelc/shape.py
--- /dev/null
+++ b/dial_mpc_b200/modelc/shape.py
@@ -0,0 +1,48 @@
+from __future__ import annotations
+
+from typing import List, Optional
+
+SHAPES = (("go2", "unitree_go2_walk"),)
+
+
+def structure_defines(md) -> Optional[List[str]]:
+    nb, nv = md.nbody, md.nv
+    depth = [md.body_depth[b] for b in range(1, nb)]
+    roots = {md.body_rootid[b] for b in range(1, nb)}
+    nchild = [0] * nv
+    for i in range(nv):
+        if md.dof_parentid[i] >= 0:
+            nchild[md.dof_parentid[i]] += 1
+    inchain, lens = [False] * nv, []
+    for i in range(nv):
+        if nchild[i]:
+            continue
+        n, j = 0, i
+        while j >= 0 and nchild[j] <= 1:
+            inchain[j] = True
+            n += 1
+            j = md.dof_parentid[j]
+        lens.append(n)
+    root_dofs = [i for i in range(nv) if not inchain[i]]
+    root_bodies = []
+    for d in reversed(root_dofs):
+        b = md.dof_bodyid[d]
+        if not root_bodies or root_bodies[-1] != b:
+            root_bodies.append(b)
+    kinds = {md.pair_kind[k] for k in range(md.npair) if md.pair_ncon[k] > 0}
+    if not lens or len(set(lens)) != 1 or len(kinds) != 1 or not root_dofs:
+        return None
+    vals = dict(NBODY=nb, NQ=md.nq, NV=nv, NU=md.nu, MAXDEPTH=max(depth), NROOT=len(roots), NCHAIN=len(lens),
+                CHAINLEN=lens[0], SB_NROOT=len(root_bodies), PAIR_KIND=kinds.pop(), ITERATIONS=md.iterations,
+                LS_ITERATIONS=md.ls_iterations)
+    return [f"DIAL_SHAPE_{k}={int(v)}" for k, v in vals.items()]
+
+
+def env_structure_defines(env_name: str) -> List[str]:
+    import dial_mpc_b200.envs as E
+    from dial_mpc_b200 import _capi
+    env = E.get_environment(env_name, config=E.get_config(env_name)())
+    d = structure_defines(_capi.fill_model_desc(env.sys.model))
+    if d is None:
+        raise ValueError(f"{env_name}: the model has no fixed structure to specialise on")
+    return d
diff --git a/include/dial_b200.h b/include/dial_b200.h
--- a/include/dial_b200.h
+++ b/include/dial_b200.h
@@ -8,7 +8,7 @@
 extern "C" {
 #endif
 
-#define DIAL_ABI_VERSION 11
+#define DIAL_ABI_VERSION 12
 
 #define DIAL_MAXB 24
 #define DIAL_MAXV 28
@@ -201,6 +201,8 @@
 
 int dial_solver_variant(const dial_model_desc* model);
 
+const char* dial_plan_rollout_kernel(const dial_plan* plan);
+
 const char* dial_custom_reward_id(void);
 
 int dial_fp32_peak(int iters, float* tflops_out);
```

Result: faster. 72.74 million (median of 6 runs) (+7.9%).
